# antoyang/FrozenBiLM

Hardware: AMD Instinct MI355X
Metric: video-text samples/sec (MLM fwd+bwd) DeBERTa-XL+adapters (higher is better)
Workload: dtype bf16; 1 GPU; DeBERTa-v2-XLarge(24L)+adapters ds8/8, B=32/GPU, T=10x1024, L=256 (S=266), MLM fwd+bwd+allreduce+clip+Adam, dropout 0.1 live, seeded random weights; global_batch=32, seq_len=266, parallelism=dp1, dead_layer23_encoder_pass=skipped (output unused, SURVEY fact 6); FLOPs still counted

## Files before the change

### frozenbilm_amd/build.py

```python
from __future__ import annotations

import concurrent.futures as cf
import os
import shutil
import subprocess
import sys

HERE = os.path.dirname(os.path.abspath(__file__))
CSRC = os.path.join(HERE, "csrc")
DEBUG = os.environ.get("FBL_DEBUG_BUILD", "0") == "1"
OBJ = os.path.join(HERE, "csrc", "build_dbg" if DEBUG else "build")
LIB = os.path.join(HERE, "libfbl_dbg.so" if DEBUG else "libfbl.so")
ARCH = "gfx950"
FLAGS = ["--offload-arch=" + ARCH, "-O3", "-std=c++17", "-fPIC", "-fno-gpu-rdc", "-Wno-unused-result"]
if DEBUG:
    FLAGS.append("-DFBL_DEBUG_SWITCHES")
    FLAGS += os.environ.get("FBL_DEBUG_EXTRA_FLAGS", "").split()
    if os.environ.get("FBL_DEBUG_LIB_NAME"):
        LIB = os.path.join(HERE, os.environ["FBL_DEBUG_LIB_NAME"])
        OBJ = os.path.join(HERE, "csrc", "build_dbg_" + os.path.splitext(os.environ["FBL_DEBUG_LIB_NAME"])[0])


def _hipcc() -> str:
    for cand in (os.environ.get("HIPCC"), shutil.which("hipcc"), "/opt/rocm/bin/hipcc"):
        if cand and os.path.exists(cand):
            return cand
    raise RuntimeError("hipcc not found (need ROCm >= 7.0 with gfx950 support)")


def sources():
    return sorted(os.path.join(CSRC, f) for f in os.listdir(CSRC) if f.endswith(".hip"))


def _deps_mtime() -> float:
    hdrs = [os.path.join(CSRC, f) for f in os.listdir(CSRC) if f.endswith(".h")]
    hdrs += [os.path.join(os.path.dirname(HERE), "include", h) for h in ("fbl.h", "fbl_mha.h", "fbl_qrows.h", "fbl_live.h", "fbl_predict.h", "fbl_groups.h", "fbl_lora.h", "fbl_ema.h", "fbl_prompt.h", "fbl_rows.h", "fbl_prompt_layers.h")]
    return max(os.path.getmtime(h) for h in hdrs)


def _compile(src: str, force: bool) -> str:
    obj = os.path.join(OBJ, os.path.basename(src)[:-4] + ".o")
    if not force and os.path.exists(obj) and os.path.getmtime(obj) > max(os.path.getmtime(src), _deps_mtime()):
        return obj
    cmd = [_hipcc(), *FLAGS, "-Rpass-analysis=kernel-resource-usage", "-c", src, "-o", obj]
    r = subprocess.run(cmd, capture_output=True, text=True)
    if r.returncode != 0:
        raise RuntimeError(f"hipcc failed for {src}:\n{r.stdout}\n{r.stderr}")
    bad, name = [], "?"
    for line in r.stderr.splitlines():
        if "Function Name:" in line:
            name = line.split("Function Name:")[1].split("[")[0].strip()
        elif "ScratchSize [bytes/lane]:" in line:
            n = int(line.split("ScratchSize [bytes/lane]:")[1].split("[")[0])
            if n > 64:
                bad.append(f"{name}: {n} bytes/lane")
            elif n > 0:
                print(f"[frozenbilm_amd.build] note: {name} spills {n} bytes/lane")
    if bad and os.environ.get("FBL_ALLOW_SCRATCH", "0") != "1":
        os.remove(obj)
        raise RuntimeError(f"{os.path.basename(src)}: kernels using scratch memory (set FBL_ALLOW_SCRATCH=1 to build anyway):\n  "
                           + "\n  ".join(bad))
    return obj


def build_lib(force: bool = False, verbose: bool = True) -> str:
    os.makedirs(OBJ, exist_ok=True)
    srcs = sources()
    with cf.ThreadPoolExecutor(max_workers=min(8, len(srcs))) as ex:
        objs = list(ex.map(lambda s: _compile(s, force), srcs))
    if force or not os.path.exists(LIB) or any(os.path.getmtime(o) > os.path.getmtime(LIB) for o in objs):
        cmd = [_hipcc(), "--offload-arch=" + ARCH, "-shared", "-fPIC", "-o", LIB, *objs]
        r = subprocess.run(cmd, capture_output=True, text=True)
        if r.returncode != 0:
            raise RuntimeError(f"link failed:\n{r.stdout}\n{r.stderr}")
        if verbose:
            print(f"[frozenbilm_amd.build] linked {LIB} from {len(objs)} objects")
    elif verbose:
        print(f"[frozenbilm_amd.build] {LIB} up to date")
    return LIB


if __name__ == "__main__":
    build_lib(force="--force" in sys.argv)
```

### frozenbilm_amd/csrc/adapter_dw.hip

```cpp
#include "fbl_common.h"
#include "../../include/fbl.h"

namespace {

constexpr int ADW_MAX_OUT = FBL_ADW_MAX_ADAPTERS;
constexpr int ADW_MAX_SEG = FBL_ADW_MAX_SEGMENTS;

struct AdwSeg { const bf16* dy; const bf16* z; const bf16* dz; const bf16* x; };
struct AdwArgs {
  AdwSeg seg[ADW_MAX_SEG];
  float* dWu[ADW_MAX_OUT]; float* dWd[ADW_MAX_OUT]; float* dbd[ADW_MAX_OUT];
  int seg_first[ADW_MAX_OUT + 1];
  int ld_dy[ADW_MAX_OUT], ld_z[ADW_MAX_OUT], ld_dz[ADW_MAX_OUT], ld_x[ADW_MAX_OUT];
  int N, H, A, tiles_h, n_out;
};

constexpr int WI = 2;
constexpr int WT = WI * 32;
constexpr int ADW_LDW = WT + 16;

template <int NT, int WHICH>
__device__ __forceinline__ void adw_tile(const AdwArgs& g, bf16* sW, bf16* sS, const int th, const int o) {
  constexpr int AP = NT * 32;
  constexpr int LDS_ = AP + 16;
  constexpr int NCH = AP / 8;
  constexpr int SPT = (64 * NCH) / 256;
  constexpr int WCH = WT / 8, WPT = (64 * WCH) / 256;
  const int tid = threadIdx.x, lane = tid & 63;
  const int wave = __builtin_amdgcn_readfirstlane(tid >> 6);
  const int wm = wave >> 1, wn = wave & 1;
  const int h0 = th * WT;
  const long ldw = WHICH ? g.ld_x[o] : g.ld_dy[o], lds = WHICH ? g.ld_dz[o] : g.ld_z[o];
  const int nk = (g.N + 63) / 64;
  const int s0 = g.seg_first[o], s1 = g.seg_first[o + 1];
  const int total = (s1 - s0) * nk;
  const int frow = lane & 15, fg = lane >> 4;

  f32x4 acc[NT][WI];
#pragma unroll
  for (int j = 0; j < NT; ++j)
#pragma unroll
    for (int i = 0; i < WI; ++i) acc[j][i] = (f32x4){0.f, 0.f, 0.f, 0.f};

  bf16x8 rw[WPT], rs[SPT];
  int gW[WPT], lW[WPT], rW[WPT], gS[SPT], lS[SPT], rS[SPT];
#pragma unroll
  for (int t = 0; t < WPT; ++t) {
    const int id = tid + t * 256;
    const int r = id / WCH, ch = id % WCH;
    const int c = min(h0 + ch * 8, g.H - 8);
    rW[t] = r;
    gW[t] = (int)(r * ldw + c);
    lW[t] = r * ADW_LDW + ch * 8;
  }
#pragma unroll
  for (int t = 0; t < SPT; ++t) {
    const int id = tid + t * 256;
    const int r = id / NCH, ch = id % NCH;
    rS[t] = r;
    gS[t] = (int)(r * lds + ch * 8);
    lS[t] = r * LDS_ + ch * 8;
  }
  const bf16x8 zero8 = (bf16x8){0, 0, 0, 0, 0, 0, 0, 0};
  const bool ragged = (g.N & 63) != 0;
  int sg_n = s0, kt_n = 0;
  auto load_tile = [&]() {
    const bf16* W = (WHICH ? g.seg[sg_n].x : g.seg[sg_n].dy) + (long)kt_n * 64 * ldw;
    const bf16* S = (WHICH ? g.seg[sg_n].dz : g.seg[sg_n].z) + (long)kt_n * 64 * lds;
    if (ragged && kt_n == nk - 1) {
      const int left = g.N - kt_n * 64;
#pragma unroll
      for (int t = 0; t < WPT; ++t) rw[t] = *(const bf16x8*)(W + gW[t] - (long)max(rW[t] - (left - 1), 0) * ldw);
#pragma unroll
      for (int t = 0; t < SPT; ++t) rs[t] = rS[t] < left ? *(const bf16x8*)(S + gS[t]) : zero8;
    } else {
#pragma unroll
      for (int t = 0; t < WPT; ++t) rw[t] = *(const bf16x8*)(W + gW[t]);
#pragma unroll
      for (int t = 0; t < SPT; ++t) rs[t] = *(const bf16x8*)(S + gS[t]);
    }
    if (++kt_n == nk) { kt_n = 0; ++sg_n; }
  };
  const bool do_cs = WHICH == 1 && th == 0 && g.dbd[o] != nullptr;
  const bf16x2 ones2 = {(bf16)1.0f, (bf16)1.0f};
  float cs[NT];
#pragma unroll
  for (int j = 0; j < NT; ++j) cs[j] = 0.f;
  const bf16* fW = sW + (fg * 4 + (frow >> 2)) * ADW_LDW + (frow & 3) * 4 + wm * (WI * 16);
  const bf16* fS = sS + (fg * 4 + (frow >> 2)) * LDS_ + (frow & 3) * 4 + wn * (NT * 16);
  if (total > 0) load_tile();
  for (int it = 0; it < total; ++it) {
#pragma unroll
    for (int t = 0; t < WPT; ++t) *(bf16x8*)(sW + lW[t]) = rw[t];
#pragma unroll
    for (int t = 0; t < SPT; ++t) *(bf16x8*)(sS + lS[t]) = rs[t];
    __syncthreads();
    if (it + 1 < total) load_tile();
#pragma unroll
    for (int s = 0; s < 2; ++s) {
      bf16x8 wf[WI], sf[NT];
#pragma unroll
      for (int i = 0; i < WI; ++i) {
        const bf16* p = fW + s * 32 * ADW_LDW + i * 16;
        union { tr16x4 h[2]; bf16x8 v; } u;
        u.h[0] = lds_tr16(p);
        u.h[1] = lds_tr16(p + 16 * ADW_LDW);
        wf[i] = u.v;
      }
#pragma unroll
      for (int j = 0; j < NT; ++j) {
        const bf16* p = fS + s * 32 * LDS_ + j * 16;
        union { tr16x4 h[2]; bf16x8 v; } u;
        u.h[0] = lds_tr16(p);
        u.h[1] = lds_tr16(p + 16 * LDS_);
        sf[j] = u.v;
      }
      if (WHICH == 1 && do_cs && s == wm) {
#pragma unroll
        for (int j = 0; j < NT; ++j) {
          union { bf16x8 v; bf16x2 p[4]; } u;
          u.v = sf[j];
#pragma unroll
          for (int q = 0; q < 4; ++q) cs[j] = __builtin_amdgcn_fdot2_f32_bf16(u.p[q], ones2, cs[j], false);
        }
      }
#pragma unroll
      for (int j = 0; j < NT; ++j)
#pragma unroll
        for (int i = 0; i < WI; ++i) {
          if (WHICH == 0) acc[j][i] = __builtin_amdgcn_mfma_f32_16x16x32_bf16(sf[j], wf[i], acc[j][i], 0, 0, 0);
          else acc[j][i] = __builtin_amdgcn_mfma_f32_16x16x32_bf16(wf[i], sf[j], acc[j][i], 0, 0, 0);
        }
    }
    __syncthreads();
  }
  const int A = g.A;
  if (WHICH == 0) {
    float* out = g.dWu[o];
    if (!out) return;
#pragma unroll
    for (int i = 0; i < WI; ++i) {
      const int h = h0 + wm * (WI * 16) + i * 16 + frow;
      if (h >= g.H) continue;
#pragma unroll
      for (int j = 0; j < NT; ++j) {
        const int a4 = wn * (NT * 16) + j * 16 + fg * 4;
        float* p = out + (long)h * A + a4;
        if (a4 + 4 <= A && ((uintptr_t)p & 15) == 0) *(f32x4*)p += acc[j][i];
        else
          for (int r = 0; r < 4; ++r)
            if (a4 + r < A) p[r] += acc[j][i][r];
      }
    }
  } else {
    if (do_cs) {
      float* red = (float*)sS;
#pragma unroll
      for (int j = 0; j < NT; ++j) red[(wm * 4 + fg) * AP + wn * (NT * 16) + j * 16 + frow] = cs[j];
      __syncthreads();
      if (tid < A) {
        float t = 0.f;
#pragma unroll
        for (int k = 0; k < 8; ++k) t += red[k * AP + tid];
        g.dbd[o][tid] += t;
      }
    }
    float* out = g.dWd[o];
    if (!out) return;
#pragma unroll
    for (int j = 0; j < NT; ++j) {
      const int a = wn * (NT * 16) + j * 16 + frow;
      if (a >= A) continue;
#pragma unroll
      for (int i = 0; i < WI; ++i) {
        const int h4 = h0 + wm * (WI * 16) + i * 16 + fg * 4;
        float* p = out + (long)a * g.H + h4;
        if (h4 + 4 <= g.H && ((uintptr_t)p & 15) == 0) *(f32x4*)p += acc[j][i];
        else
          for (int r = 0; r < 4; ++r)
            if (h4 + r < g.H) p[r] += acc[j][i][r];
      }
    }
  }
}

template <int NT>
__global__ __launch_bounds__(256, 2) void adapter_dw_kernel(AdwArgs g) {
  __shared__ __attribute__((aligned(16))) bf16 sW[64 * ADW_LDW];
  __shared__ __attribute__((aligned(16))) bf16 sS[64 * (NT * 32 + 16)];
  const int lin = blockIdx.x, xcd = lin & 7, slot = lin >> 3;
  const int p = (slot / g.tiles_h) * 8 + xcd, th = slot % g.tiles_h;
  if (p >= 2 * g.n_out) return;
  const int o = p >> 1;
  if ((p & 1) == 0) adw_tile<NT, 0>(g, sW, sS, th, o);
  else adw_tile<NT, 1>(g, sW, sS, th, o);
}

}

extern "C" int fbl_adapter_bwd_dw(int n_adapters, const int32_t* seg_first, const void* const* dy_bf16, const void* const* z_bf16,
                                  const void* const* dz_bf16, const void* const* x_bf16, const int64_t* ld_dy,
                                  const int64_t* ld_z, const int64_t* ld_dz, const int64_t* ld_x, int N, int H, int A, int Ap,
                                  float* const* dWu, float* const* dWd, float* const* dbd, void* stream) {
  if (n_adapters <= 0 || N <= 0 || H <= 0 || A <= 0) return 0;
  if (n_adapters > ADW_MAX_OUT || !seg_first || seg_first[0] != 0) return FBL_ERR_ARG;
  const int nseg = seg_first[n_adapters];
  if (nseg <= 0 || nseg > ADW_MAX_SEG) return FBL_ERR_ARG;
  if (Ap < A || (Ap % 64) || Ap > 256 || (H % 8)) return FBL_ERR_SHAPE;
  if (!dy_bf16 || !z_bf16 || !dz_bf16 || !x_bf16 || !ld_dy || !ld_z || !ld_dz || !ld_x) return FBL_ERR_ARG;
  AdwArgs g{};
  for (int o = 0; o < n_adapters; ++o) {
    if (seg_first[o + 1] < seg_first[o]) return FBL_ERR_ARG;
    g.seg_first[o] = seg_first[o];
    g.dWu[o] = dWu ? dWu[o] : nullptr;
    g.dWd[o] = dWd ? dWd[o] : nullptr;
    g.dbd[o] = dbd ? dbd[o] : nullptr;
    if ((ld_dy[o] % 8) || (ld_z[o] % 8) || (ld_dz[o] % 8) || (ld_x[o] % 8)) return FBL_ERR_ALIGN;
    if (ld_dy[o] < H || ld_x[o] < H || ld_z[o] < Ap || ld_dz[o] < Ap) return FBL_ERR_ARG;
    if ((ld_dy[o] | ld_x[o] | ld_z[o] | ld_dz[o]) >> 24) return FBL_ERR_ARG;
    g.ld_dy[o] = (int)ld_dy[o]; g.ld_z[o] = (int)ld_z[o]; g.ld_dz[o] = (int)ld_dz[o]; g.ld_x[o] = (int)ld_x[o];
  }
  g.seg_first[n_adapters] = nseg;
  for (int s = 0; s < nseg; ++s) {
    if (!dy_bf16[s] || !z_bf16[s] || !dz_bf16[s] || !x_bf16[s]) return FBL_ERR_ARG;
    g.seg[s] = AdwSeg{(const bf16*)dy_bf16[s], (const bf16*)z_bf16[s], (const bf16*)dz_bf16[s], (const bf16*)x_bf16[s]};
  }
  g.N = N; g.H = H; g.A = A;
  g.tiles_h = (H + WT - 1) / WT;
  g.n_out = n_adapters;
  dim3 grid((unsigned)(((2 * n_adapters + 7) / 8) * 8 * g.tiles_h));
  switch (Ap / 64) {
    case 1: hipLaunchKernelGGL(adapter_dw_kernel<2>, grid, dim3(256), 0, (hipStream_t)stream, g); break;
    case 2: hipLaunchKernelGGL(adapter_dw_kernel<4>, grid, dim3(256), 0, (hipStream_t)stream, g); break;
    case 3: hipLaunchKernelGGL(adapter_dw_kernel<6>, grid, dim3(256), 0, (hipStream_t)stream, g); break;
    default: hipLaunchKernelGGL(adapter_dw_kernel<8>, grid, dim3(256), 0, (hipStream_t)stream, g); break;
  }
  FBL_CHECK_LAUNCH();
  return 0;
}
```

### frozenbilm_amd/csrc/rowops.hip

```cpp
#include "fbl_common.h"
#include "../../include/fbl.h"
#include "../../include/fbl_live.h"
#include "../../include/fbl_groups.h"
#include "../../include/fbl_ema.h"
#include "../../include/fbl_rows.h"

namespace {

template <int VEC>
struct VecF {};
template <>
struct VecF<4> {
  typedef f32x4 T;
};
template <>
struct VecF<2> {
  typedef f32x2 T;
};

template <int VEC>
__device__ __forceinline__ void ldf(const float* p, float* v) {
  if (VEC == 4) {
    f32x4 x = *(const f32x4*)p;
    v[0] = x[0]; v[1] = x[1]; v[2] = x[2]; v[3] = x[3];
  } else if (VEC == 2) {
    f32x2 x = *(const f32x2*)p;
    v[0] = x[0]; v[1] = x[1];
  } else {
    v[0] = p[0];
  }
}
template <int VEC>
__device__ __forceinline__ void stf(float* p, const float* v) {
  if (VEC == 4) *(f32x4*)p = (f32x4){v[0], v[1], v[2], v[3]};
  else if (VEC == 2) *(f32x2*)p = (f32x2){v[0], v[1]};
  else p[0] = v[0];
}
template <int VEC>
__device__ __forceinline__ void stb(bf16* p, const float* v) {
  if (VEC == 4) *(bf16x4*)p = (bf16x4){f2bf(v[0]), f2bf(v[1]), f2bf(v[2]), f2bf(v[3])};
  else if (VEC == 2) *(bf16x2*)p = (bf16x2){f2bf(v[0]), f2bf(v[1])};
  else p[0] = f2bf(v[0]);
}

struct LnFwdArgs {
  const float* y; long ldy; float p_drop; uint64_t seed; const uint64_t* seed_dev;
  const float* r_plain; const float* r_t; const float* r_stats; const float* r_gamma; const float* r_beta;
  const int32_t* r_rowmask;
  const float* gamma; const float* beta; float eps; const int32_t* rowmask;
  float* out_t; float* out_stats; bf16* out_bf16; float* out_f32;
  int N, H;
};

template <int EPL>
__global__ __launch_bounds__(256) void ln_fwd_kernel(LnFwdArgs a) {
  constexpr int VEC = (EPL % 4 == 0) ? 4 : ((EPL % 2 == 0) ? 2 : 1);
  constexpr int NIT = EPL / VEC;
  const int lane = threadIdx.x & 63;
  const int row = blockIdx.x * 4 + (threadIdx.x >> 6);
  if (row >= a.N) return;
  const int H = a.H;
  float v[EPL];
  const uint32_t thr = fbl_drop_thresh(a.p_drop);
  const float inv_keep = a.p_drop > 0.f ? 1.0f / (1.0f - a.p_drop) : 1.0f;
  const uint64_t seed = a.p_drop > 0.f ? fbl_seed(a.seed, a.seed_dev) : 0;
  float rmean = 0.f, rrstd = 0.f, rmask = 1.f;
  if (a.r_t) {
    rmean = a.r_stats[2 * (long)row];
    rrstd = a.r_stats[2 * (long)row + 1];
    if (a.r_rowmask) rmask = (float)a.r_rowmask[row];
  }
#pragma unroll
  for (int it = 0; it < NIT; ++it) {
    const int col = (it * 64 + lane) * VEC;
    float* vv = v + it * VEC;
    if (a.y) {
      ldf<VEC>(a.y + (long)row * a.ldy + col, vv);
      if (a.p_drop > 0.f) {
#pragma unroll
        for (int c = 0; c < VEC; ++c) vv[c] *= fbl_dropout_scale(seed, (uint64_t)row * H + col + c, thr, inv_keep);
      }
    } else {
#pragma unroll
      for (int c = 0; c < VEC; ++c) vv[c] = 0.f;
    }
    if (a.r_plain) {
      float r[VEC];
      ldf<VEC>(a.r_plain + (long)row * H + col, r);
#pragma unroll
      for (int c = 0; c < VEC; ++c) vv[c] += r[c];
    }
    if (a.r_t) {
      float r[VEC], gg[VEC], bb[VEC];
      ldf<VEC>(a.r_t + (long)row * H + col, r);
      ldf<VEC>(a.r_gamma + col, gg);
      ldf<VEC>(a.r_beta + col, bb);
#pragma unroll
      for (int c = 0; c < VEC; ++c) vv[c] += ((r[c] - rmean) * rrstd * gg[c] + bb[c]) * rmask;
    }
    if (a.out_t) stf<VEC>(a.out_t + (long)row * H + col, vv);
  }
  float s = 0.f;
#pragma unroll
  for (int e = 0; e < EPL; ++e) s += v[e];
  const float mean = wave_sum(s) / (float)H;
  float q = 0.f;
#pragma unroll
  for (int e = 0; e < EPL; ++e) {
    const float d = v[e] - mean;
    q += d * d;
  }
  const float var = wave_sum(q) / (float)H;
  const float rstd = rsqrtf(var + a.eps);
  if (lane == 0 && a.out_stats) {
    a.out_stats[2 * (long)row] = mean;
    a.out_stats[2 * (long)row + 1] = rstd;
  }
  const float om = a.rowmask ? (float)a.rowmask[row] : 1.0f;
#pragma unroll
  for (int it = 0; it < NIT; ++it) {
    const int col = (it * 64 + lane) * VEC;
    float gg[VEC], bb[VEC], o[VEC];
    ldf<VEC>(a.gamma + col, gg);
    ldf<VEC>(a.beta + col, bb);
#pragma unroll
    for (int c = 0; c < VEC; ++c) o[c] = ((v[it * VEC + c] - mean) * rstd * gg[c] + bb[c]) * om;
    if (a.out_bf16) stb<VEC>(a.out_bf16 + (long)row * H + col, o);
    if (a.out_f32) stf<VEC>(a.out_f32 + (long)row * H + col, o);
  }
}

struct LnMatArgs {
  const float* t; const float* stats; const float* gamma; const float* beta; const int32_t* rowmask;
  const float* add_bcast; int S; float* out_f32; bf16* out_bf16; int N, H;
};
template <int EPL>
__global__ __launch_bounds__(256) void ln_mat_kernel(LnMatArgs a) {
  constexpr int VEC = (EPL % 4 == 0) ? 4 : ((EPL % 2 == 0) ? 2 : 1);
  constexpr int NIT = EPL / VEC;
  const int lane = threadIdx.x & 63;
  const int row = blockIdx.x * 4 + (threadIdx.x >> 6);
  if (row >= a.N) return;
  const int H = a.H;
  const float mean = a.stats[2 * (long)row], rstd = a.stats[2 * (long)row + 1];
  const float om = a.rowmask ? (float)a.rowmask[row] : 1.0f;
#pragma unroll
  for (int it = 0; it < NIT; ++it) {
    const int col = (it * 64 + lane) * VEC;
    float x[VEC], gg[VEC], bb[VEC], o[VEC];
    ldf<VEC>(a.t + (long)row * H + col, x);
    ldf<VEC>(a.gamma + col, gg);
    ldf<VEC>(a.beta + col, bb);
#pragma unroll
    for (int c = 0; c < VEC; ++c) o[c] = ((x[c] - mean) * rstd * gg[c] + bb[c]) * om;
    if (a.add_bcast) {
      float p[VEC];
      ldf<VEC>(a.add_bcast + (long)(row % a.S) * H + col, p);
#pragma unroll
      for (int c = 0; c < VEC; ++c) o[c] += p[c];
    }
    if (a.out_f32) stf<VEC>(a.out_f32 + (long)row * H + col, o);
    if (a.out_bf16) stb<VEC>(a.out_bf16 + (long)row * H + col, o);
  }
}

constexpr int LNB_BLOCKS = 768;
struct LnBwdArgs {
  const float* dout; const int32_t* rowmask; const float* t; const float* stats; const float* gamma;
  float p_drop; uint64_t seed; const uint64_t* seed_dev; float* out_dt; bf16* out_dy_bf16; float* out_dy_f32; float* ws; int N, H;
  long ld_dyb;
  const int32_t* inv; bf16* out_dy_pad;
};
template <int EPL, bool ROWS = false>
__global__ __launch_bounds__(256) void ln_bwd_kernel(LnBwdArgs a) {
  constexpr int VEC = (EPL % 4 == 0) ? 4 : ((EPL % 2 == 0) ? 2 : 1);
  constexpr int NIT = EPL / VEC;
  __shared__ float red[4 * 64 * EPL];
  const int lane = threadIdx.x & 63, wave = threadIdx.x >> 6;
  const int H = a.H;
  float dg[EPL], db[EPL], dys[EPL], gam[EPL];
#pragma unroll
  for (int e = 0; e < EPL; ++e) dg[e] = db[e] = dys[e] = 0.f;
#pragma unroll
  for (int it = 0; it < NIT; ++it) ldf<VEC>(a.gamma + (it * 64 + lane) * VEC, gam + it * VEC);
  const uint32_t thr = fbl_drop_thresh(a.p_drop);
  const float inv_keep = a.p_drop > 0.f ? 1.0f / (1.0f - a.p_drop) : 1.0f;
  const uint64_t seed = a.p_drop > 0.f ? fbl_seed(a.seed, a.seed_dev) : 0;
  for (int row = blockIdx.x * 4 + wave; row < a.N; row += gridDim.x * 4) {
    long crow = row;
    if (ROWS) {
      const int cr = a.inv[row];
      if (cr < 0) {
        const float z[VEC] = {};
#pragma unroll
        for (int it = 0; it < NIT; ++it) stb<VEC>(a.out_dy_pad + (long)row * H + (it * 64 + lane) * VEC, z);
        continue;
      }
      crow = cr;
    }
    const float mean = a.stats[2 * (long)row], rstd = a.stats[2 * (long)row + 1];
    const float om = a.rowmask ? (float)a.rowmask[row] : 1.0f;
    float g[EPL], xh[EPL];
    float s1 = 0.f, s2 = 0.f;
#pragma unroll
    for (int it = 0; it < NIT; ++it) {
      const int col = (it * 64 + lane) * VEC;
      float d[VEC], x[VEC];
      ldf<VEC>(a.dout + crow * H + col, d);
      ldf<VEC>(a.t + (long)row * H + col, x);
#pragma unroll
      for (int c = 0; c < VEC; ++c) {
        const int e = it * VEC + c;
        const float dd = d[c] * om;
        xh[e] = (x[c] - mean) * rstd;
        dg[e] += dd * xh[e];
        db[e] += dd;
        g[e] = dd * gam[e];
        s1 += g[e];
        s2 += g[e] * xh[e];
      }
    }
    s1 = wave_sum(s1) / (float)H;
    s2 = wave_sum(s2) / (float)H;
#pragma unroll
    for (int it = 0; it < NIT; ++it) {
      const int col = (it * 64 + lane) * VEC;
      float dt[VEC], dy[VEC];
#pragma unroll
      for (int c = 0; c < VEC; ++c) {
        const int e = it * VEC + c;
        dt[c] = rstd * (g[e] - s1 - xh[e] * s2);
        dy[c] = dt[c];
        if (a.p_drop > 0.f) dy[c] *= fbl_dropout_scale(seed, (uint64_t)row * H + col + c, thr, inv_keep);
        dys[e] += dy[c];
      }
      if (a.out_dt) stf<VEC>(a.out_dt + crow * H + col, dt);
      if (a.out_dy_bf16) stb<VEC>(a.out_dy_bf16 + crow * a.ld_dyb + col, dy);
      if (a.out_dy_f32) stf<VEC>(a.out_dy_f32 + crow * H + col, dy);
      if (ROWS) stb<VEC>(a.out_dy_pad + (long)row * H + col, dy);
    }
  }
#pragma unroll
  for (int which = 0; which < 3; ++which) {
    const float* src = which == 0 ? dg : (which == 1 ? db : dys);
    if (which) __syncthreads();
#pragma unroll
    for (int it = 0; it < NIT; ++it) {
      const int col = (it * 64 + lane) * VEC;
#pragma unroll
      for (int c = 0; c < VEC; ++c) red[wave * H + col + c] = src[it * VEC + c];
    }
    __syncthreads();
    for (int i = threadIdx.x; i < H; i += 256) {
      float s_ = 0.f;
#pragma unroll
      for (int w = 0; w < 4; ++w) s_ += red[w * H + i];
      a.ws[(long)blockIdx.x * 3 * H + which * H + i] = s_;
    }
  }
}
template <int EPL, bool ROWS = false>
__global__ __launch_bounds__(256, 3) void ln_bwd2_kernel(LnBwdArgs a) {
  static_assert(EPL % 2 == 0, "two waves share a row");
  constexpr int EW = EPL / 2;
  constexpr int VEC = (EW % 4 == 0) ? 4 : ((EW % 2 == 0) ? 2 : 1);
  constexpr int NIT = EW / VEC;
  __shared__ float red[2 * 64 * EPL];
  __shared__ float xch[2][2][2][2];
  const int lane = threadIdx.x & 63, wave = threadIdx.x >> 6;
  const int slot = wave >> 1, half = wave & 1;
  const int H = a.H;
  const int c0 = half * (H / 2);
  float dg[EW], db[EW], dys[EW], gam[EW];
#pragma unroll
  for (int e = 0; e < EW; ++e) dg[e] = db[e] = dys[e] = 0.f;
#pragma unroll
  for (int it = 0; it < NIT; ++it) ldf<VEC>(a.gamma + c0 + (it * 64 + lane) * VEC, gam + it * VEC);
  const uint32_t thr = fbl_drop_thresh(a.p_drop);
  const float inv_keep = a.p_drop > 0.f ? 1.0f / (1.0f - a.p_drop) : 1.0f;
  const uint64_t seed = a.p_drop > 0.f ? fbl_seed(a.seed, a.seed_dev) : 0;
  int par = 0;
  for (int base = blockIdx.x * 2; base < a.N; base += gridDim.x * 2, par ^= 1) {
    const int row = base + slot;
    bool live = row < a.N;
    const int rr = live ? row : a.N - 1;
    long crow = row;
    bool pad_zero = false;
    if (ROWS) {
      const int cr = a.inv[rr];
      pad_zero = live && cr < 0;
      live = live && cr >= 0;
      crow = cr;
    }
    float g[EW], xh[EW];
    float s1 = 0.f, s2 = 0.f, rstd = 0.f;
    if (!ROWS || live) {
      const long lr = ROWS ? crow : (long)rr;
      const float mean = a.stats[2 * (long)rr];
      rstd = a.stats[2 * (long)rr + 1];
      const float om = live ? (a.rowmask ? (float)a.rowmask[rr] : 1.0f) : 0.f;
#pragma unroll
      for (int it = 0; it < NIT; ++it) {
        const int col = c0 + (it * 64 + lane) * VEC;
        float d[VEC], x[VEC];
        ldf<VEC>(a.dout + lr * H + col, d);
        ldf<VEC>(a.t + (long)rr * H + col, x);
#pragma unroll
        for (int c = 0; c < VEC; ++c) {
          const int e = it * VEC + c;
          const float dd = d[c] * om;
          xh[e] = (x[c] - mean) * rstd;
          dg[e] += dd * xh[e];
          db[e] += dd;
          g[e] = dd * gam[e];
          s1 += g[e];
          s2 += g[e] * xh[e];
        }
      }
      s1 = wave_sum(s1);
      s2 = wave_sum(s2);
    }
    if (lane == 0) {
      xch[par][slot][half][0] = s1;
      xch[par][slot][half][1] = s2;
    }
    __syncthreads();
    s1 = (xch[par][slot][0][0] + xch[par][slot][1][0]) / (float)H;
    s2 = (xch[par][slot][0][1] + xch[par][slot][1][1]) / (float)H;
    if (live) {
#pragma unroll
      for (int it = 0; it < NIT; ++it) {
        const int col = c0 + (it * 64 + lane) * VEC;
        float dt[VEC], dy[VEC];
#pragma unroll
        for (int c = 0; c < VEC; ++c) {
          const int e = it * VEC + c;
          dt[c] = rstd * (g[e] - s1 - xh[e] * s2);
          dy[c] = dt[c];
          if (a.p_drop > 0.f) dy[c] *= fbl_dropout_scale(seed, (uint64_t)row * H + col + c, thr, inv_keep);
          dys[e] += dy[c];
        }
        if (a.out_dt) stf<VEC>(a.out_dt + crow * H + col, dt);
        if (a.out_dy_bf16) stb<VEC>(a.out_dy_bf16 + crow * a.ld_dyb + col, dy);
        if (a.out_dy_f32) stf<VEC>(a.out_dy_f32 + crow * H + col, dy);
        if (ROWS) stb<VEC>(a.out_dy_pad + (long)row * H + col, dy);
      }
    } else if (ROWS && pad_zero) {
      const float z[VEC] = {};
#pragma unroll
      for (int it = 0; it < NIT; ++it) stb<VEC>(a.out_dy_pad + (long)row * H + c0 + (it * 64 + lane) * VEC, z);
    }
  }
#pragma unroll
  for (int which = 0; which < 3; ++which) {
    const float* src = which == 0 ? dg : (which == 1 ? db : dys);
    __syncthreads();
#pragma unroll
    for (int it = 0; it < NIT; ++it) {
      const int col = c0 + (it * 64 + lane) * VEC;
#pragma unroll
      for (int c = 0; c < VEC; ++c) red[slot * H + col + c] = src[it * VEC + c];
    }
    __syncthreads();
    for (int i = threadIdx.x; i < H; i += 256) a.ws[(long)blockIdx.x * 3 * H + which * H + i] = red[i] + red[H + i];
  }
}

__device__ __forceinline__ float fold16(const float* ws, int nblk, int ncols, int col) {
  __shared__ float red[16][17];
  const int tx = threadIdx.x & 15, ty = threadIdx.x >> 4;
  float s = 0.f;
  if (col < ncols)
    for (int b = ty; b < nblk; b += 16) s += ws[(long)b * ncols + col];
  red[ty][tx] = s;
  __syncthreads();
  if (ty == 0) {
#pragma unroll
    for (int k = 1; k < 16; ++k) s += red[k][tx];
  }
  return s;
}
__global__ __launch_bounds__(256) void ln_bwd_fold_kernel(const float* ws, int nblk, int H, float* dgamma, float* dbeta,
                                                          float* dysum) {
  __shared__ f32x4 red[4][8];
  const int tx = threadIdx.x & 7, ty = threadIdx.x >> 3;
  const int lane = threadIdx.x & 63, wave = threadIdx.x >> 6;
  const int col = blockIdx.x * 32 + tx * 4;
  const int ncols = 3 * H;
  f32x4 s = {0.f, 0.f, 0.f, 0.f};
  if (col < ncols) {
    const float* p = ws + col;
    int b = ty;
    for (; b + 224 < nblk; b += 256) {
      f32x4 v[8];
#pragma unroll
      for (int u = 0; u < 8; ++u) v[u] = *(const f32x4*)(p + (long)(b + 32 * u) * ncols);
      s += ((v[0] + v[1]) + (v[2] + v[3])) + ((v[4] + v[5]) + (v[6] + v[7]));
    }
    for (; b < nblk; b += 32) s += *(const f32x4*)(p + (long)b * ncols);
  }
#pragma unroll
  for (int o = 8; o < 64; o <<= 1) {
#pragma unroll
    for (int r = 0; r < 4; ++r) s[r] += __shfl_xor(s[r], o, 64);
  }
  if (lane < 8) red[wave][lane] = s;
  __syncthreads();
  if (threadIdx.x < 8 && col < ncols) {
    s = (red[0][tx] + red[1][tx]) + (red[2][tx] + red[3][tx]);
    float* dst = col < H ? dgamma : (col < 2 * H ? dbeta : dysum);
    if (dst) {
      float* q = dst + (col % H);
#pragma unroll
      for (int r = 0; r < 4; ++r) q[r] += s[r];
    }
  }
}

__global__ void embed_gather_kernel(const int64_t* ids, const float* E, const float* vproj, int B, int T, int L, int H,
                                    float* out) {
  const int S = T + L;
  const int row = blockIdx.x;
  const int b = row / S, s = row % S;
  const float* src = (s < T) ? vproj + ((long)b * T + s) * H : E + ids[(long)b * L + (s - T)] * (long)H;
  float* dst = out + (long)row * H;
  for (int c = threadIdx.x * 4; c < H; c += blockDim.x * 4) *(f32x4*)(dst + c) = *(const f32x4*)(src + c);
}

__global__ void video_stage_kernel(const _Float16* feats, const int64_t* row_off, const int32_t* n_rows, int T, int F,
                                   float* out, int64_t* video_len, int64_t* video_mask) {
  const int b = blockIdx.x / T, j = blockIdx.x % T;
  const int n = n_rows[b];
  const int len = n < T ? n : T;
  if (threadIdx.x == 0) {
    if (j == 0 && video_len) video_len[b] = len;
    if (video_mask) video_mask[(long)b * T + j] = j < len ? 1 : 0;
  }
  float* dst = out + ((long)b * T + j) * F;
  if (j >= len) {
    for (int c = threadIdx.x * 4; c < F; c += blockDim.x * 4) *(f32x4*)(dst + c) = (f32x4){0.f, 0.f, 0.f, 0.f};
    return;
  }
  const long r = n > T ? ((long)j * n) / T : j;
  const _Float16* src = feats + (row_off[b] + r) * (long)F;
  typedef __attribute__((ext_vector_type(8))) _Float16 f16x8;
  for (int c = threadIdx.x * 8; c < F; c += blockDim.x * 8) {
    const f16x8 h = *(const f16x8*)(src + c);
    *(f32x4*)(dst + c) = (f32x4){(float)h[0], (float)h[1], (float)h[2], (float)h[3]};
    *(f32x4*)(dst + c + 4) = (f32x4){(float)h[4], (float)h[5], (float)h[6], (float)h[7]};
  }
}

__global__ void mask_tokens_kernel(int64_t* ids, int64_t* labels, long n, const int64_t* special, int n_special, float p,
                                   int64_t mask_id, int64_t vocab, uint64_t seed) {
  const long i = (long)blockIdx.x * blockDim.x + threadIdx.x;
  if (i >= n) return;
  const int64_t id = ids[i];
  bool sp = false;
  for (int k = 0; k < n_special; ++k) sp |= (special[k] == id);
  const float inv = 1.0f / 4294967296.0f;
  const bool pick = !sp && (float)fbl_hash(seed, 4ull * i) * inv < p;
  labels[i] = pick ? id : -100;
  if (!pick) return;
  if ((float)fbl_hash(seed, 4ull * i + 1) * inv < 0.8f) ids[i] = mask_id;
  else if ((float)fbl_hash(seed, 4ull * i + 2) * inv < 0.5f) ids[i] = (int64_t)(fbl_hash(seed, 4ull * i + 3) % (uint64_t)vocab);
}

__global__ void im2col3_kernel(const bf16* x, bf16* out, int B, int S, int H) {
  const int row = blockIdx.x;
  const int s = row % S;
  const int chunks = 3 * H / 8;
  for (int i = threadIdx.x; i < chunks; i += blockDim.x) {
    const int k = (i * 8) / H, c = (i * 8) % H;
    const int ss = s + k - 1;
    bf16x8 v = {0, 0, 0, 0, 0, 0, 0, 0};
    if (ss >= 0 && ss < S) v = *(const bf16x8*)(x + ((long)row + k - 1) * H + c);
    *(bf16x8*)(out + (long)row * 3 * H + i * 8) = v;
  }
}
__global__ void col2im3_kernel(const float* dcol, float* dx, int B, int S, int H, int accumulate) {
  const int row = blockIdx.x;
  const int s = row % S;
  for (int c = threadIdx.x * 4; c < H; c += blockDim.x * 4) {
    f32x4 acc = accumulate ? *(const f32x4*)(dx + (long)row * H + c) : (f32x4){0.f, 0.f, 0.f, 0.f};
#pragma unroll
    for (int k = 0; k < 3; ++k) {
      const int ss = s - k + 1;
      if (ss >= 0 && ss < S) acc += *(const f32x4*)(dcol + ((long)row - k + 1) * 3 * H + k * H + c);
    }
    *(f32x4*)(dx + (long)row * H + c) = acc;
  }
}

__global__ void dropout_gelu_fwd_kernel(const float* c, float p, uint64_t seed0, const uint64_t* seed_dev, float* out, long n) {
  const uint64_t seed = p > 0.f ? fbl_seed(seed0, seed_dev) : 0;
  const uint32_t thr = fbl_drop_thresh(p);
  const float ik = p > 0.f ? 1.f / (1.f - p) : 1.f;
  for (long i = (long)blockIdx.x * blockDim.x + threadIdx.x; i < n; i += (long)gridDim.x * blockDim.x) {
// ... 539 lines not shown
    const int h = (int)(eh % nh);
    const long e = eh / nh;
    const f32x4 a = *(const f32x4*)(src + q * 64 + c8 * 8), b = *(const f32x4*)(src + q * 64 + c8 * 8 + 4);
    *(bf16x8*)(dst + (e * rows + r) * ld_dst + h * 64 + c8 * 8) =
        (bf16x8){f2bf(a[0]), f2bf(a[1]), f2bf(a[2]), f2bf(a[3]), f2bf(b[0]), f2bf(b[1]), f2bf(b[2]), f2bf(b[3])};
  }
}

inline int grid1d(long n, int block = 256, int cap = 256 * 16) {
  long b = (n + block - 1) / block;
  return (int)(b < 1 ? 1 : (b > cap ? cap : b));
}

}

#define FBL_EPL_DISPATCH(H, KERNEL, GRID, ARGS, STREAM)                                              \
  switch ((H) / 64) {                                                                                \
    case 1: hipLaunchKernelGGL(KERNEL<1>, GRID, dim3(256), 0, STREAM, ARGS); break;                  \
    case 2: hipLaunchKernelGGL(KERNEL<2>, GRID, dim3(256), 0, STREAM, ARGS); break;                  \
    case 4: hipLaunchKernelGGL(KERNEL<4>, GRID, dim3(256), 0, STREAM, ARGS); break;                  \
    case 8: hipLaunchKernelGGL(KERNEL<8>, GRID, dim3(256), 0, STREAM, ARGS); break;                  \
    case 12: hipLaunchKernelGGL(KERNEL<12>, GRID, dim3(256), 0, STREAM, ARGS); break;                \
    case 16: hipLaunchKernelGGL(KERNEL<16>, GRID, dim3(256), 0, STREAM, ARGS); break;                \
    case 24: hipLaunchKernelGGL(KERNEL<24>, GRID, dim3(256), 0, STREAM, ARGS); break;                \
    case 32: hipLaunchKernelGGL(KERNEL<32>, GRID, dim3(256), 0, STREAM, ARGS); break;                \
    default: return FBL_ERR_SHAPE;                                                                   \
  }

extern "C" int fbl_abi_version(void) { return 9; }

extern "C" int fbl_embed_gather(const int64_t* ids, const float* E, const float* vproj, int B, int T, int L, int H,
                                float* out_t, void* stream) {
  if (H % 4) return FBL_ERR_SHAPE;
  if (T > 0 && !vproj) return FBL_ERR_ARG;
  if (B * (T + L) <= 0) return 0;
  hipLaunchKernelGGL(embed_gather_kernel, dim3(B * (T + L)), dim3(128), 0, (hipStream_t)stream, ids, E, vproj, B, T, L,
                     H, out_t);
  FBL_CHECK_LAUNCH();
  return 0;
}

extern "C" int fbl_video_stage_f16(const void* feats_f16, const int64_t* row_off, const int32_t* n_rows, int B, int T, int F,
                                   float* out_f32, int64_t* video_len, int64_t* video_mask, void* stream) {
  if (F % 8 || ((uintptr_t)feats_f16 & 15) || ((uintptr_t)out_f32 & 15)) return FBL_ERR_ALIGN;
  if (B <= 0 || T <= 0) return 0;
  hipLaunchKernelGGL(video_stage_kernel, dim3(B * T), dim3(128), 0, (hipStream_t)stream, (const _Float16*)feats_f16, row_off,
                     n_rows, T, F, out_f32, video_len, video_mask);
  FBL_CHECK_LAUNCH();
  return 0;
}

extern "C" int fbl_mask_tokens(int64_t* ids, int64_t* labels, int64_t n, const int64_t* special_ids, int n_special,
                               float mlm_probability, int64_t mask_token_id, int64_t vocab_size, uint64_t seed,
                               void* stream) {
  if (n <= 0) return 0;
  if (vocab_size <= 0 || mlm_probability < 0.f || mlm_probability > 1.f || n_special < 0) return FBL_ERR_ARG;
  hipLaunchKernelGGL(mask_tokens_kernel, dim3((unsigned)((n + 255) / 256)), dim3(256), 0, (hipStream_t)stream, ids, labels,
                     (long)n, special_ids, n_special, mlm_probability, mask_token_id, vocab_size, seed);
  FBL_CHECK_LAUNCH();
  return 0;
}

extern "C" int fbl_ln_fwd(const float* y, int64_t ldy, float p_drop, uint64_t seed, const uint64_t* seed_dev, const float* r_plain,
                          const float* r_t, const float* r_stats, const float* r_gamma, const float* r_beta,
                          const int32_t* r_rowmask, const float* gamma, const float* beta, float eps,
                          const int32_t* rowmask, float* out_t, float* out_stats, void* out_bf16, float* out_f32, int N,
                          int H, void* stream) {
  if (H % 64 || H > 2048) return FBL_ERR_SHAPE;
  if (r_t && (!r_stats || !r_gamma || !r_beta)) return FBL_ERR_ARG;
  if (N <= 0) return 0;
  LnFwdArgs a{y, ldy, p_drop, seed, seed_dev, r_plain, r_t, r_stats, r_gamma, r_beta, r_rowmask, gamma, beta, eps, rowmask,
              out_t, out_stats, (bf16*)out_bf16, out_f32, N, H};
  dim3 grid((N + 3) / 4);
  FBL_EPL_DISPATCH(H, ln_fwd_kernel, grid, a, (hipStream_t)stream);
  FBL_CHECK_LAUNCH();
  return 0;
}

extern "C" int fbl_ln_materialize(const float* t, const float* stats, const float* gamma, const float* beta,
                                  const int32_t* rowmask, const float* add_bcast, int S, float* out_f32, void* out_bf16,
                                  int N, int H, void* stream) {
  if (H % 64 || H > 2048) return FBL_ERR_SHAPE;
  if (N <= 0) return 0;
  LnMatArgs a{t, stats, gamma, beta, rowmask, add_bcast, S > 0 ? S : 1, out_f32, (bf16*)out_bf16, N, H};
  dim3 grid((N + 3) / 4);
  FBL_EPL_DISPATCH(H, ln_mat_kernel, grid, a, (hipStream_t)stream);
  FBL_CHECK_LAUNCH();
  return 0;
}

extern "C" int64_t fbl_ln_bwd_ws_floats(int H) { return (int64_t)LNB_BLOCKS * 3 * H; }
template <bool ROWS>
static int ln_bwd_launch(const LnBwdArgs& a, float* dgamma, float* dbeta, float* dysum, hipStream_t stream) {
  const int N = a.N, H = a.H;
  int nblk;
  if ((H / 64) % 2 == 0) {
    nblk = (N + 1) / 2;
    if (nblk > LNB_BLOCKS) nblk = LNB_BLOCKS;
    dim3 grid(nblk);
    switch (H / 64) {
      case 2: hipLaunchKernelGGL((ln_bwd2_kernel<2, ROWS>), grid, dim3(256), 0, stream, a); break;
      case 4: hipLaunchKernelGGL((ln_bwd2_kernel<4, ROWS>), grid, dim3(256), 0, stream, a); break;
      case 8: hipLaunchKernelGGL((ln_bwd2_kernel<8, ROWS>), grid, dim3(256), 0, stream, a); break;
      case 12: hipLaunchKernelGGL((ln_bwd2_kernel<12, ROWS>), grid, dim3(256), 0, stream, a); break;
      case 16: hipLaunchKernelGGL((ln_bwd2_kernel<16, ROWS>), grid, dim3(256), 0, stream, a); break;
      case 24: hipLaunchKernelGGL((ln_bwd2_kernel<24, ROWS>), grid, dim3(256), 0, stream, a); break;
      case 32: hipLaunchKernelGGL((ln_bwd2_kernel<32, ROWS>), grid, dim3(256), 0, stream, a); break;
      default: return FBL_ERR_SHAPE;
    }
  } else {
    nblk = (N + 3) / 4;
    if (nblk > LNB_BLOCKS) nblk = LNB_BLOCKS;
    dim3 grid(nblk);
    switch (H / 64) {
      case 1: hipLaunchKernelGGL((ln_bwd_kernel<1, ROWS>), grid, dim3(256), 0, stream, a); break;
      default: return FBL_ERR_SHAPE;
    }
  }
  FBL_CHECK_LAUNCH();
  if (dgamma || dbeta || dysum) {
    hipLaunchKernelGGL(ln_bwd_fold_kernel, dim3((3 * H + 31) / 32), dim3(256), 0, stream, a.ws, nblk, H, dgamma, dbeta, dysum);
    FBL_CHECK_LAUNCH();
  }
  return 0;
}

extern "C" int fbl_ln_bwd(const float* dout, const int32_t* rowmask, const float* t, const float* stats,
                          const float* gamma, float p_drop, uint64_t seed, const uint64_t* seed_dev, float* out_dt, void* out_dy_bf16,
                          float* out_dy_f32, float* dgamma, float* dbeta, float* dysum, float* ws, int N, int H,
                          int64_t ld_dy_bf16, void* stream) {
  if (H % 64 || H > 2048) return FBL_ERR_SHAPE;
  if (N <= 0) return 0;
  if (ld_dy_bf16 == 0) ld_dy_bf16 = H;
  if (ld_dy_bf16 < H || (ld_dy_bf16 % 8)) return FBL_ERR_ALIGN;
  LnBwdArgs a{dout, rowmask, t, stats, gamma, p_drop, seed, seed_dev, out_dt, (bf16*)out_dy_bf16, out_dy_f32, ws, N, H, ld_dy_bf16,
              nullptr, nullptr};
  return ln_bwd_launch<false>(a, dgamma, dbeta, dysum, (hipStream_t)stream);
}

extern "C" int fbl_ln_bwd_rows(const float* dout, const int32_t* inv, const int32_t* rowmask, const float* t, const float* stats,
                               const float* gamma, float p_drop, uint64_t seed, const uint64_t* seed_dev, float* out_dt,
                               void* out_dy_bf16, int64_t ld_dy_bf16, void* out_dy_pad_bf16, float* dgamma, float* dbeta,
                               float* dysum, float* ws, int N_pad, int H, void* stream) {
  if (H % 64 || H > 2048) return FBL_ERR_SHAPE;
  if (!dout || !inv || !t || !stats || !gamma || !ws || !out_dy_pad_bf16) return FBL_ERR_ARG;
  if (N_pad <= 0) return 0;
  if (ld_dy_bf16 == 0) ld_dy_bf16 = H;
  if (ld_dy_bf16 < H || (ld_dy_bf16 % 8)) return FBL_ERR_ALIGN;
  LnBwdArgs a{dout, rowmask, t, stats, gamma, p_drop, seed, seed_dev, out_dt, (bf16*)out_dy_bf16, nullptr, ws, N_pad, H, ld_dy_bf16,
              inv, (bf16*)out_dy_pad_bf16};
  return ln_bwd_launch<true>(a, dgamma, dbeta, dysum, (hipStream_t)stream);
}

extern "C" int fbl_im2col3(const void* x_bf16, void* out_bf16, int B, int S, int H, void* stream) {
  if (H % 8) return FBL_ERR_SHAPE;
  if (B * S <= 0) return 0;
  hipLaunchKernelGGL(im2col3_kernel, dim3(B * S), dim3(256), 0, (hipStream_t)stream, (const bf16*)x_bf16,
                     (bf16*)out_bf16, B, S, H);
  FBL_CHECK_LAUNCH();
  return 0;
}
extern "C" int fbl_col2im3(const float* dcol, float* dx, int B, int S, int H, int accumulate, void* stream) {
  if (H % 4) return FBL_ERR_SHAPE;
  if (B * S <= 0) return 0;
  hipLaunchKernelGGL(col2im3_kernel, dim3(B * S), dim3(256), 0, (hipStream_t)stream, dcol, dx, B, S, H, accumulate);
  FBL_CHECK_LAUNCH();
  return 0;
}

extern "C" int fbl_dropout_gelu_fwd(const float* c, float p_drop, uint64_t seed, const uint64_t* seed_dev, float* out_f32,
                                    int64_t n, void* stream) {
  if (n <= 0) return 0;
  hipLaunchKernelGGL(dropout_gelu_fwd_kernel, dim3(grid1d(n)), dim3(256), 0, (hipStream_t)stream, c, p_drop, seed, seed_dev,
                     out_f32, (long)n);
  FBL_CHECK_LAUNCH();
  return 0;
}
extern "C" int fbl_dropout_gelu_bwd(const float* dy, const float* c, float p_drop, uint64_t seed, const uint64_t* seed_dev,
                                    void* out_bf16, float* out_f32, int64_t n, void* stream) {
  if (n <= 0) return 0;
  hipLaunchKernelGGL(dropout_gelu_bwd_kernel, dim3(grid1d(n)), dim3(256), 0, (hipStream_t)stream, dy, c, p_drop, seed, seed_dev,
                     (bf16*)out_bf16, out_f32, (long)n);
  FBL_CHECK_LAUNCH();
  return 0;
}

extern "C" int fbl_transpose_to_bf16(const void* in, int in_is_bf16, int64_t ld_in, int rows, int cols, void* out_bf16,
                                     int64_t rows_pad, void* stream) {
  if (rows_pad < rows) return FBL_ERR_ARG;
  if (rows_pad <= 0 || cols <= 0) return 0;
  dim3 grid((unsigned)((rows_pad + 63) / 64), (cols + 63) / 64);
  if (in_is_bf16)
    hipLaunchKernelGGL(transpose_kernel<true>, grid, dim3(256), 0, (hipStream_t)stream, in, (long)ld_in, rows, cols,
                       (bf16*)out_bf16, (long)rows_pad);
  else
    hipLaunchKernelGGL(transpose_kernel<false>, grid, dim3(256), 0, (hipStream_t)stream, in, (long)ld_in, rows, cols,
                       (bf16*)out_bf16, (long)rows_pad);
  FBL_CHECK_LAUNCH();
  return 0;
}

extern "C" int fbl_transpose_batched_bf16(const void* src_bf16, const int64_t* src_off, void* dst_bf16,
                                          const int64_t* dst_off, int count, int rows, int cols, void* stream) {
  if (count <= 0 || rows <= 0 || cols <= 0) return 0;
  hipLaunchKernelGGL(transpose_batched_kernel, dim3((rows + 63) / 64, (cols + 63) / 64, count), dim3(256), 0,
                     (hipStream_t)stream, (const bf16*)src_bf16, src_off, (bf16*)dst_bf16, dst_off, rows, cols);
  FBL_CHECK_LAUNCH();
  return 0;
}

extern "C" int64_t fbl_colsum_ws_floats(int cols) { return (int64_t)CS_BLOCKS * cols; }
extern "C" int fbl_colsum(const void* in, int in_is_bf16, int64_t ld_in, int rows, int cols, float* out, float* ws,
                          void* stream) {
  if (rows <= 0 || cols <= 0) return 0;
  int nblk = rows < CS_BLOCKS ? rows : CS_BLOCKS;
  dim3 grid(nblk, (cols + 255) / 256);
  if (in_is_bf16)
    hipLaunchKernelGGL(colsum_kernel<true>, grid, dim3(256), 0, (hipStream_t)stream, in, (long)ld_in, rows, cols, ws);
  else
    hipLaunchKernelGGL(colsum_kernel<false>, grid, dim3(256), 0, (hipStream_t)stream, in, (long)ld_in, rows, cols, ws);
  FBL_CHECK_LAUNCH();
  hipLaunchKernelGGL(colsum_fold_kernel, dim3((cols + 15) / 16), dim3(256), 0, (hipStream_t)stream, ws, nblk, cols,
                     out);
  FBL_CHECK_LAUNCH();
  return 0;
}

extern "C" int fbl_head_transpose(const void* v_bf16, int64_t ldv, void* vt_bf16, int B, int S, int Sp, int nh,
                                  int64_t out_sh, int64_t out_sb, int64_t out_sd, void* stream) {
  if (Sp < S || Sp % 64) return FBL_ERR_SHAPE;
  if (ldv % 8 || out_sh % 8 || out_sb % 8 || out_sd % 8 || ((uintptr_t)v_bf16 & 15) || ((uintptr_t)vt_bf16 & 15)) return FBL_ERR_ALIGN;
  if (B * S <= 0) return 0;
  hipLaunchKernelGGL(head_transpose_kernel, dim3(Sp / 64, nh, B), dim3(256), 0, (hipStream_t)stream,
                     (const bf16*)v_bf16, (long)ldv, (bf16*)vt_bf16, B, S, Sp, nh, (long)out_sh, (long)out_sb,
                     (long)out_sd);
  FBL_CHECK_LAUNCH();
  return 0;
}

extern "C" int fbl_ce_fwd(const float* logits, int64_t ldv, const int64_t* labels, int N, int V, float* row_lse,
                          float* loss_sum_cnt, void* stream) {
  if (N <= 0) return 0;
  hipLaunchKernelGGL(ce_fwd_kernel, dim3(N), dim3(256), 0, (hipStream_t)stream, logits, (long)ldv, labels, N, V,
                     row_lse, loss_sum_cnt);
  FBL_CHECK_LAUNCH();
  hipLaunchKernelGGL(ce_fold_kernel, dim3(1), dim3(256), 0, (hipStream_t)stream, logits, (long)ldv, labels, N, row_lse,
                     loss_sum_cnt);
  FBL_CHECK_LAUNCH();
  return 0;
}
extern "C" int fbl_ce_bwd_rows(const float* logits, int64_t ldv, const int64_t* labels, const int32_t* rows, int R,
                               int V, int Vp, const float* row_lse, const float* loss_sum_cnt, float gscale,
                               const float* gscale_dev, void* dlogits_bf16, void* stream) {
  if (R <= 0) return 0;
  if (Vp < V) return FBL_ERR_ARG;
  hipLaunchKernelGGL(ce_bwd_rows_kernel, dim3(R), dim3(256), 0, (hipStream_t)stream, logits, (long)ldv, labels, rows, V,
                     Vp, row_lse, loss_sum_cnt, gscale, gscale_dev, (bf16*)dlogits_bf16);
  FBL_CHECK_LAUNCH();
  return 0;
}

extern "C" int fbl_gather_rows_bf16(const void* in, int64_t ld, const int32_t* rows, int R, int cols, void* out,
                                    void* stream) {
  if (R <= 0) return 0;
  if (cols % 8 || ld % 8) return FBL_ERR_ALIGN;
  hipLaunchKernelGGL(gather_rows_bf16_kernel, dim3(R), dim3(128), 0, (hipStream_t)stream, (const bf16*)in, (long)ld,
                     rows, cols, (bf16*)out);
  FBL_CHECK_LAUNCH();
  return 0;
}
extern "C" int fbl_scatter_rows_f32(const float* in, const int32_t* rows, int R, int cols, float* out, int64_t ld,
                                    void* stream) {
  if (R <= 0) return 0;
  hipLaunchKernelGGL(scatter_rows_f32_kernel, dim3(R), dim3(256), 0, (hipStream_t)stream, in, rows, cols, out,
                     (long)ld);
  FBL_CHECK_LAUNCH();
  return 0;
}

extern "C" int64_t fbl_sumsq_ws_floats(void) { return SUMSQ_BLOCKS; }
extern "C" int fbl_sumsq(const float* x, int64_t n, float* out_sumsq, float* ws, void* stream) {
  if (n <= 0) return 0;
  if (!ws || !out_sumsq) return FBL_ERR_ARG;
  const int nblk = grid1d(n, 256, SUMSQ_BLOCKS);
  hipLaunchKernelGGL(sumsq_kernel, dim3(nblk), dim3(256), 0, (hipStream_t)stream, x, (long)n, ws);
  FBL_CHECK_LAUNCH();
  hipLaunchKernelGGL(sumsq_fold_kernel, dim3(1), dim3(256), 0, (hipStream_t)stream, (const float*)ws, nblk, out_sumsq);
  FBL_CHECK_LAUNCH();
  return 0;
}
extern "C" int fbl_adam_flat(float* p, const float* g, float* m, float* v, int64_t n, float lr, float beta1,
                             float beta2, float eps, float weight_decay, int step, const float* sumsq, float max_norm,
                             float grad_scale, void* stream) {
  if (n <= 0) return 0;
  const float bc1 = 1.0f - powf(beta1, (float)step);
  const float bc2 = 1.0f - powf(beta2, (float)step);
  hipLaunchKernelGGL(adam_flat_kernel, dim3(grid1d(n)), dim3(256), 0, (hipStream_t)stream, p, g, m, v, (long)n, lr,
                     beta1, beta2, eps, weight_decay, bc1, bc2, sumsq, max_norm, grad_scale);
  FBL_CHECK_LAUNCH();
  return 0;
}

static inline bool live_aligned(const void* a) { return ((uintptr_t)a & 15) == 0; }
extern "C" int fbl_sumsq_live(const float* x, int64_t n, const int64_t* ranges, float* out_sumsq, float* ws, void* stream) {
  if (n <= 0) return 0;
  if (!x || !ranges || !ws || !out_sumsq) return FBL_ERR_ARG;
// ... 138 lines not shown
```

### frozenbilm_amd/engine.py

```python
from __future__ import annotations

import dataclasses
from dataclasses import dataclass, field
from typing import Dict, List, Optional

import numpy as np
import torch

from . import lib as L
from .predict import check_topk, of_call as predictions_of_call
from .live_set import REL_LN, LiveSetMixin, flat_layout, stage_plan
from .attn_bwd import ATTN_SCALE, _relidx_range, disent_attn_bwd, pos_chain_buffers, pos_table_grads_batched
from .model.deberta import PROMPT_NAME, layer_prompt_name
from .model.relpos import rel_index_vector

BF16, F32 = torch.bfloat16, torch.float32


def _ru(x: int, m: int) -> int:
    return (x + m - 1) // m * m


def check_logit_rows(logit_rows: torch.Tensor, n_grid: int) -> None:
    r = logit_rows.reshape(-1)
    if r.numel() == 0:
        return
    s = torch.sort(r.long()).values
    dup = (s[1:] == s[:-1]).any() if s.numel() > 1 else torch.zeros((), dtype=torch.bool, device=s.device)
    lo, hi, dup = torch.stack([s[0], s[-1], dup.long()]).tolist()
    if lo < 0 or hi >= n_grid:
        raise ValueError(f"logit_rows must index the [B, S] token grid: 0 <= row < {n_grid} (got {lo} .. {hi})")
    if dup:
        raise ValueError("logit_rows holds an index more than once: with gradients every requested row must be distinct")


@dataclass
class NormRef:
    t: torch.Tensor
    stats: torch.Tensor
    gamma: torch.Tensor
    beta: torch.Tensor
    rowmask: Optional[torch.Tensor] = None

    def as_args(self):
        return (self.t, self.stats, self.gamma, self.beta, self.rowmask)


@dataclass
class Stream:
    bf16: torch.Tensor
    norm: Optional[NormRef] = None
    plain: Optional[torch.Tensor] = None
    full: Optional[torch.Tensor] = None


@dataclass
class Packing:
    row0: torch.Tensor
    sel: torch.Tensor
    inv: torch.Tensor
    pos: torch.Tensor
    n: int
    sel32: Optional[torch.Tensor] = None
    inv32: Optional[torch.Tensor] = None


@dataclass
class MergedPack:
    A: int
    WT: torch.Tensor
    WM: torch.Tensor
    bM: torch.Tensor
    b16: torch.Tensor
    WF: Optional[torch.Tensor]
    groups: list


@dataclass
class AdapterSite:
    name: str
    A: int
    Ap: int
    down: torch.Tensor
    up: torch.Tensor
    bd: torch.Tensor
    bu: torch.Tensor
    merged: bool
    grouped: bool
    WM: Optional[torch.Tensor] = None
    bM: Optional[torch.Tensor] = None
    WF: Optional[torch.Tensor] = None
    upT: Optional[torch.Tensor] = None
    downT: Optional[torch.Tensor] = None


@dataclass
class LoraSite:
    name: str
    li: int
    t: int
    idx: int


class Engine(LiveSetMixin):
    def __init__(self, model):
        self.m = model
        cfg = model.config
        self.cfg = cfg
        self.H, self.I, self.V = cfg.hidden_size, cfg.intermediate_size, cfg.vocab_size
        self.nh = cfg.num_attention_heads
        self.nL = cfg.num_hidden_layers
        self.span2 = 2 * cfg.att_span
        self.lin_span = min(cfg.position_buckets // 2, cfg.att_span) if cfg.position_buckets > 0 else 0
        self.F = model.features_dim
        self.Fp = _ru(self.F, 64) if self.F else 0
        self.A1 = self.H // model.ds_factor_attn if model.ds_factor_attn else 0
        self.A2 = self.H // model.ds_factor_ff if model.ds_factor_ff else 0
        self.Vp = _ru(self.V, 64)
        dev = model.device
        if dev.type != "cuda":
            raise RuntimeError("frozenbilm_amd runs on MI355X only: move the model to a cuda (HIP) device; "
                               "there is no CPU fallback")
        L.load()
        self.dev = dev
        o = dict(getattr(model, "engine_options", None) or {})
        unknown = set(o) - {"eager_logits", "dw_group", "attn_save_p"}
        if unknown:
            raise ValueError(f"unknown engine_options: {sorted(unknown)}")
        self.eager_logits = bool(o.get("eager_logits", False))
        self.attn_save_p = bool(o.get("attn_save_p", True))
        self.dw_group = max(1, min(L.ADW_MAX_ADAPTERS, int(o.get("dw_group", 16))))
        self.n_prompt = int(getattr(model, "n_prompt", 0))
        self.prompt_depth = int(getattr(model, "prompt_depth", 1))
        self._build_flat()
        self._pack_frozen()
        self._build_trainable_operands()
        self._build_lora()
        self._compose_ev = None
        self._relidx: Dict[int, torch.Tensor] = {}
        self._pos_cache: Dict[int, torch.Tensor] = {}
        self._no_pos_cache = False
        self.reducer = None
        self._dyz_pool: Dict[tuple, list] = {}
        self._dyz_shape = None
        self._dyz_compact = None
        self.params_version = 0
        self._ops_version = None
        self.skip_dead_layer = True
        self._ln_ws = L.ln_bwd_ws(self.H, dev)
        self._cs_ws = L.colsum_ws(max(self.H, self.I), dev)
        self.sk_ws = torch.empty(48 << 20, dtype=F32, device=dev)
        self.side = torch.cuda.Stream(device=dev)
        self.side_ws = torch.empty(8 << 20, dtype=F32, device=dev)
        self.side_cs_ws = L.colsum_ws(max(self.H, self.I), dev)
        if L._AUX.get(dev.index if dev.index is not None else torch.cuda.current_device()) is None:
            L.set_aux_stream(torch.cuda.Stream(device=dev), dev)
        L.exclude_from_aux(self.side)

    def _build_flat(self):
        from .model.deberta import flat_order

        m = self.m
        named = dict(m.named_parameters())
        train_names = m.trainable_names()
        order = flat_order(self.cfg, train_names)
        offs, total = flat_layout(order, {n: named[n].numel() for n in order})
        self.flat = torch.zeros(total, dtype=F32, device=self.dev)
        from .parallel import SCALAR_SLOT

        self.flat_grad_full = torch.zeros(SCALAR_SLOT + total, dtype=F32, device=self.dev)
        self.flat_grad = self.flat_grad_full[SCALAR_SLOT:]
        self.flat_bf16 = torch.zeros(total, dtype=BF16, device=self.dev)
        self.offsets, self.order = offs, order
        self._adT_offs = {}
        self.G: Dict[str, torch.Tensor] = {}
        self.Pb: Dict[str, torch.Tensor] = {}
        for n in order:
            p = named[n]
            o, k = offs[n], p.numel()
            view = self.flat[o:o + k].view(p.shape)
            view.copy_(p.data)
            p.data = view
            self.G[n] = self.flat_grad[o:o + k].view(p.shape)
            self.Pb[n] = self.flat_bf16[o:o + k].view(p.shape)
        self.P = {n: p.data for n, p in named.items()}
        self.named = named
        self.bucket_ends: Dict[str, int] = {}
        for n in order:
            key = self._bucket_key(n)
            self.bucket_ends[key] = offs[n] + _ru(named[n].numel(), 8)
        self._plans: Dict[tuple, object] = {}
        self._init_live()

    def plan(self, grad_in=()):
        key = (self.live_version, bool(grad_in))
        pl = self._plans.get(key)
        if pl is None:
            pl = self._plans[key] = stage_plan(self.nL, bool(self.cfg.conv_kernel_size), self.live_order, grad_in)
        return pl

    def _bucket_key(self, name: str) -> str:
        if name.startswith("lm_predictions."):
            return "head"
        if name.startswith("deberta.encoder.layer."):
            return "layer" + name.split(".")[3]
        if name.startswith("deberta.encoder.conv."):
            return "conv"
        if name.startswith("deberta.encoder.LayerNorm"):
            return "relln"
        return "emb"

    def attach_grads(self):
        fresh = all(self.named[n].grad is None for n in self.live_order)
        if fresh:
            L.zero_(self.flat_grad)
        for n in self.live_order:
            p = self.named[n]
# ... 27 lines not shown
                Wi=bf(P[p + ".intermediate.dense.weight"]), WiT=bf(P[p + ".intermediate.dense.weight"].t()),
                bi=P[p + ".intermediate.dense.bias"].float().contiguous(),
                Wd=bf(P[p + ".output.dense.weight"]), WdT=self.WdT_rev[j],
                bd=P[p + ".output.dense.bias"].float().contiguous(),
            )
            self.Lw.append(d)
        order = [nL - 1, nL - 1] + list(range(nL - 2, -1, -1)) + [nL - 1]
        self.WposT_exec = torch.empty(len(order), H, 2 * H, dtype=BF16, device=dev)
        for e, li in enumerate(order):
            self.WposT_exec[e].copy_(self.Lw[li]["WqkvT"][:, : 2 * H])
        if self.cfg.conv_kernel_size:
            w = P["deberta.encoder.conv.conv.weight"]
            W2 = w.permute(0, 2, 1).reshape(H, 3 * H)
            self.Wc, self.WcT = bf(W2), bf(W2.t())
            self.bc = P["deberta.encoder.conv.conv.bias"].float().contiguous()
        hd = "lm_predictions.lm_head."
        self.Wh, self.WhT = bf(P[hd + "dense.weight"]), bf(P[hd + "dense.weight"].t())
        self.bh = P[hd + "dense.bias"].float().contiguous()
        E = P["deberta.embeddings.word_embeddings.weight"]
        self.E32 = E.float().contiguous()
        self.Eb = bf(E)
        self.ETb = torch.zeros(H, self.Vp, dtype=BF16, device=self.dev)
        self.ETb[:, : self.V] = E.t().to(BF16)
        self.head_bias = P[hd + "bias"].float().contiguous()
        self.rel_emb = P["deberta.encoder.rel_embeddings.weight"].float().contiguous()
        self.pos_emb = P["deberta.embeddings.position_embeddings.weight"].float().contiguous()
        if self.m.n_ans:
            T = P["answer_embeddings.weight"]
            self.n_ans = T.shape[0]
            self.Ansb = bf(T)
            self.ans_bias = P["answer_bias"].float().contiguous()

    def _build_trainable_operands(self):
        H, nL, dev = self.H, self.nL, self.dev
        self.sites = [[None, None] for _ in range(nL)]
        self.packs: List[MergedPack] = []
        for k, (blk, A, K, WT, wkey, bkey) in enumerate(((".attention.output.adapter", self.A1, H, self.WoT_rev, "Wo", "bo"),
                                                         (".output.adapter", self.A2, self.I, self.WdT_rev, "Wd", "bd"))):
            if not A:
                continue
            Ap = _ru(A, 64)
            merged = A % 64 == 0 and H % 64 == 0
            names = [f"deberta.encoder.layer.{i}{blk}" for i in range(nL)]
            pack = None
            if merged:
                WF = torch.zeros(nL, H, _ru(H + A, 128), dtype=BF16, device=dev) if k == 0 else None
                ow = [self.offsets[n + ".down.weight"] for n in names]
                ob = [self.offsets[n + ".down.bias"] for n in names]
                if nL >= 3 and len({ow[i - 1] - ow[i] for i in range(2, nL)}) == 1 and \
                        len({ob[i - 1] - ob[i] for i in range(2, nL)}) == 1 and ow[nL - 2] - ow[nL - 1] == ob[nL - 2] - ob[nL - 1] > 0:
                    groups = [(nL - 1, 1, ow[0], ob[0], A * H), (0, nL - 1, ow[nL - 1], ob[nL - 1], ow[nL - 2] - ow[nL - 1])]
                else:
                    groups = [(nL - 1 - i, 1, ow[i], ob[i], A * H) for i in range(nL)]
                pack = MergedPack(A=A, WT=WT, WM=torch.zeros(nL, H + A, K, dtype=BF16, device=dev),
                                  bM=torch.zeros(nL, H + A, dtype=F32, device=dev),
                                  b16=torch.zeros(nL, 1, H, dtype=BF16, device=dev), WF=WF, groups=groups)
                self.packs.append(pack)
            for i, n in enumerate(names):
                j = nL - 1 - i
                up = self.Pb[n + ".up.weight"] if Ap == A else torch.zeros(H, Ap, dtype=BF16, device=dev)
                site = AdapterSite(name=n, A=A, Ap=Ap, down=self.Pb[n + ".down.weight"], up=up, bd=self.P[n + ".down.bias"],
                                   bu=self.P[n + ".up.bias"], merged=merged, grouped=Ap <= 256 and H % 8 == 0)
                if merged:
                    pack.WM[j, :H].copy_(self.Lw[i][wkey])
                    pack.bM[j, :H].copy_(self.Lw[i][bkey])
                    pack.b16[j, 0].copy_(self.Lw[i][bkey])
                    site.WM, site.bM = pack.WM[j], pack.bM[j]
                    if pack.WF is not None:
                        pack.WF[j, :, :H].copy_(WT[j])
                        site.WF = pack.WF[j]
                self.sites[i][k] = site
        self.all_sites = [a for pair in self.sites for a in pair if a is not None]
        if self.F:
            wv = self.Pb["deberta.embeddings.linear_video.weight"]
            self.Wv = wv if self.Fp == self.F else torch.zeros(H, self.Fp, dtype=BF16, device=dev)

    def _build_lora(self):
        from .model.deberta import LORA_TARGETS

        m, H = self.m, self.H
        self.lora_r = int(getattr(m, "lora_rank", 0) or 0)
        self.lora_sites: Dict[tuple, LoraSite] = {}
        self.lora_composes = 0
        self._lora_ops = None
        self._lora_idx = None
        self._lora_names = set()
        self._lora_pos = False
        if not self.lora_r:
            return
        self.lora_s = float(m.lora_scale)
        recs = []
        for i in range(self.nL):
            for tname in m.lora_targets:
                t = LORA_TARGETS.index(tname)
                nm = f"deberta.encoder.layer.{i}.attention.self.{tname}"
                self.lora_sites[(i, t)] = LoraSite(name=nm, li=i, t=t, idx=len(recs))
                recs.append(dict(W=self.P[nm + ".weight"], A=self.P[nm + ".lora_A.weight"], B=self.P[nm + ".lora_B.weight"],
                                 scale=self.lora_s, dst=self.Lw[i]["Wqkv"][t * H:(t + 1) * H],
                                 dstT=self.Lw[i]["WqkvT"][:, t * H:(t + 1) * H]))
        self._lora_recs = recs
        self._lora_table = L.LoraTable(recs, self.dev)
        self._lora_names = {s.name for s in self.lora_sites.values()}
        self._lora_pos = any(t < 2 for (_, t) in self.lora_sites)
        self._lora_Aop = torch.zeros(len(recs), 64, H, dtype=BF16, device=self.dev)
        self._lora_BTop = torch.zeros(len(recs), 64, H, dtype=BF16, device=self.dev)

    def _compose_lora(self):
        L.lora_compose(self._lora_table)
        self.lora_composes += 1
        if self._lora_pos:
            H, nL = self.H, self.nL
            for e, li in enumerate([nL - 1, nL - 1] + list(range(nL - 2, -1, -1)) + [nL - 1]):
                self.WposT_exec[e].copy_(self.Lw[li]["WqkvT"][:, : 2 * H])

    def merge_lora(self):
        L.lora_compose(L.LoraTable([dict(r, dst32=r["W"]) for r in self._lora_recs], self.dev))
        for r in self._lora_recs:
            r["B"].zero_()
        self.invalidate_operands()

    def _lora_bwd_operands(self):
        if self._lora_ops is None:
            r, H, dev = self.lora_r, self.H, self.dev
            if self._lora_idx is None:
                i64 = lambda v: torch.tensor(v, dtype=torch.int64, device=dev)
                sites = sorted(self.lora_sites.values(), key=lambda s: s.idx)
                oA = i64([self.offsets[s.name + ".lora_A.weight"] for s in sites])
                oB = i64([self.offsets[s.name + ".lora_B.weight"] for s in sites])
                rowmajor = torch.arange(r * H, device=dev)
                transposed = (torch.arange(H, device=dev)[None, :] * r + torch.arange(r, device=dev)[:, None]).reshape(-1)
                self._lora_idx = ((oA[:, None] + rowmajor[None]).reshape(-1), (oB[:, None] + transposed[None]).reshape(-1))
            ns = len(self.lora_sites)
            self._lora_Aop[:, :r].copy_(self.flat_bf16.index_select(0, self._lora_idx[0]).view(ns, r, H))
            self._lora_BTop[:, :r].copy_(self.flat_bf16.index_select(0, self._lora_idx[1]).view(ns, r, H))
            self._lora_ops = (self._lora_Aop, self._lora_BTop)
        return self._lora_ops

    def _lora_products(self, site: LoraSite, dy, x):
        Aop, BTop = self._lora_bwd_operands()
        n = dy.shape[0]
        u = torch.empty(n, 64, dtype=BF16, device=self.dev)
        v = torch.empty(n, 64, dtype=BF16, device=self.dev)
        L.gemm(x, Aop[site.idx], alpha=self.lora_s, out_bf16=u)
        L.gemm(dy, BTop[site.idx], alpha=self.lora_s, out_bf16=v)
        return (dy, u, v, x)

    def _lora_live(self, site: Optional[LoraSite]) -> bool:
        return site is not None and any((site.name + k) in self.Gl for k in (".lora_A.weight", ".lora_B.weight"))

    def _lora_bwd(self, run, li: int, t: int, dy, x):
        site = self.lora_sites.get((li, t))
        if not self._lora_live(site):
            return
        run.dw_pending.append((self.lora_r, site.name, self._lora_products(site, dy, x), run.dw_count, None))
        run.dw_count += 1

    def _dw_outputs(self, nm: str, Gl):
        if nm in getattr(self, "_lora_names", ()):
            return Gl.get(nm + ".lora_B.weight"), Gl.get(nm + ".lora_A.weight"), None
        return Gl.get(nm + ".up.weight"), Gl.get(nm + ".down.weight"), Gl.get(nm + ".down.bias")

    def _lora_pos_bwd(self, run, pc, dpb):
        H, nL = self.H, self.nL
        order = [nL - 1, nL - 1] + list(range(nL - 2, -1, -1)) + [nL - 1]
        segs: Dict[str, list] = {}
        for e in range(dpb.shape[0]):
            sites = [self.lora_sites.get((order[e], t)) for t in (0, 1)]
            if not any(self._lora_live(s) for s in sites):
                continue
            if run.p_hid > 0:
                xe = torch.empty(self.span2, H, dtype=BF16, device=self.dev)
                L.dropout_f32(run.R32, run.p_hid, pc.seeds[e], out_bf16=xe)
            else:
                xe = run.Rb
            x = xe[pc.rmin:pc.rmin + pc.rcnt]
            for t, site in enumerate(sites):
                if self._lora_live(site):
                    segs.setdefault(site.name, []).append(self._lora_products(site, dpb[e][:, t * H:(t + 1) * H], x))
        groups, nseg = [], 0
        for nm, sg in list(segs.items()) + [(None, None)]:
            if groups and (nm is None or len(groups) == L.ADW_MAX_ADAPTERS or nseg + len(sg) > L.ADW_MAX_SEGMENTS):
                L.adapter_bwd_dw(groups, A=self.lora_r)
                groups, nseg = [], 0
            if nm is not None:
                groups.append((sg, *self._dw_outputs(nm, self.Gl)))
                nseg += len(sg)

    def relidx(self, S: int) -> torch.Tensor:
        if S not in self._relidx:
            v = rel_index_vector(S, self.cfg.position_buckets, self.cfg.max_rel, self.cfg.att_span)
            self._relidx[S] = torch.from_numpy(np.ascontiguousarray(v)).to(self.dev)
        return self._relidx[S]

    def _refresh_if_stale(self, need_grad: bool):
        frozen = getattr(self.m, "_weights_frozen", 0) > 0
        ver = (self.params_version, tuple(self.named[n]._version for n in self.order)) if (frozen and not need_grad) else None
        if ver is None or ver != self._ops_version:
            self.refresh_trainable_operands()
            self._ops_version = ver

    def seed_word_value(self) -> int:
        return (self.m.dropout_seed_base() * 0x9E3779B1) & 0x7FFFFFFFFFFFFFFF

    def prepare_inference(self):
        self._refresh_if_stale(False)
        if self._compose_ev is not None:
            torch.cuda.current_stream().wait_event(self._compose_ev[1])
            self._compose_ev = None

    def invalidate_operands(self):
        self._ops_version = None
        self.params_version += 1

    def refresh_trainable_operands(self):
        self._pos_cache.clear()
        L.cast_bf16(self.flat, self.flat_bf16)
        for a in self.all_sites:
            if a.Ap != a.A:
                a.up[:, :a.A] = self.Pb[a.name + ".up.weight"]
            a.upT = a.downT = None
        if self.packs:
            self.side.wait_stream(torch.cuda.current_stream())
            with torch.cuda.stream(self.side):
                self._compose_ev = self._compose_adapter_down()
        if self.F and self.Fp != self.F:
            self.Wv[:, : self.F] = self.Pb["deberta.embeddings.linear_video.weight"]
        if self.lora_r:
            self._lora_ops = None
            self._compose_lora()

    def _compose_adapter_down(self):
        H = self.H

        def run_group(pk: MergedPack, grp):
            A, (j0, nb, o_w, o_b, st) = pk.A, grp
            wd3 = torch.as_strided(self.flat_bf16, (nb, A, H), (st, H, 1), o_w)
            L.gemm(wd3, pk.WT[j0:j0 + nb], out_bf16=pk.WM[j0:j0 + nb, H:H + A, :])
            if pk.WF is not None:
                L.gemm(pk.WT[j0:j0 + nb], wd3, out_bf16=pk.WF[j0:j0 + nb, :, H:H + A])
            bd3 = torch.as_strided(self.flat, (nb, A, 1), (st, 1, 1), o_b)
            bo3 = torch.as_strided(pk.bM, (nb, A, 1), (pk.bM.stride(0), 1, 1), pk.bM[j0, H:].storage_offset())
            L.gemm(wd3, pk.b16[j0:j0 + nb], aux=bd3, aux_kind=L.AUX_ADD_F32, out_f32=bo3)

        for pk in self.packs:
            run_group(pk, pk.groups[0])
        ev0 = torch.cuda.Event()
        ev0.record()
        for pk in self.packs:
            for grp in pk.groups[1:]:
                run_group(pk, grp)
        ev1 = torch.cuda.Event()
        ev1.record()
        return ev0, ev1

    def _adapter_bwd_operands(self, site: AdapterSite):
        if site.upT is None:
            H = self.H
            groups = {}
            for a in self.all_sites:
                groups.setdefault((a.A, a.Ap), []).append(a)
            for (A, Ap), sites in groups.items():
                upT_all = torch.empty(len(sites), A, H, dtype=BF16, device=self.dev)
                for i, a in enumerate(sites):
                    a.upT = upT_all[i]
                cache = self._adT_offs.get((A, Ap))
                if cache is None:
                    i64 = lambda v: torch.tensor(v, dtype=torch.int64, device=self.dev)
                    cache = dict(up_src=i64([self.offsets[a.name + ".up.weight"] for a in sites]),
                                 dn_src=i64([self.offsets[a.name + ".down.weight"] for a in sites]),
                                 dst=i64([i * A * H for i in range(len(sites))]))
                    self._adT_offs[(A, Ap)] = cache
                L.transpose_batched_bf16(self.flat_bf16, cache["up_src"], upT_all, cache["dst"], H, A)
                if Ap == A:
                    dnT_all = torch.empty(len(sites), H, A, dtype=BF16, device=self.dev)
                    L.transpose_batched_bf16(self.flat_bf16, cache["dn_src"], dnT_all, cache["dst"], A, H)
                    for i, a in enumerate(sites):
                        a.downT = dnT_all[i]
                else:
                    for a in sites:
                        a.downT = torch.zeros(H, Ap, dtype=BF16, device=self.dev)
                        a.downT[:, :A].copy_(a.down.t())
        return site.upT, site.downT

    def run(self, input_ids, attention_mask, video, video_mask, labels, mlm, want_hidden, logit_rows=None, want_attn=False,
            inputs_embeds=None):
        m = self.m
        train = m.training
        k_pred = check_topk(getattr(m, "predict_topk", 0))
        text = input_ids if inputs_embeds is None else inputs_embeds
        if text.device != self.dev:
            raise RuntimeError(f"inputs must be on {self.dev}")
        B, Lt = text.shape[:2]
        if attention_mask is None:
            attention_mask = (torch.ones_like(input_ids) if inputs_embeds is None
                              else torch.ones(B, Lt, dtype=torch.long, device=self.dev))
        use_video = bool(self.F) and video is not None
        grad_on = torch.is_grad_enabled()
        grad_in = []
        if grad_on and use_video and video.requires_grad:
            grad_in.append(("video", video))
        if grad_on and inputs_embeds is not None and inputs_embeds.requires_grad:
            grad_in.append(("embeds", inputs_embeds))
        need_grad = grad_on and (self.update_live() or bool(grad_in))
        T = video.shape[1] if use_video else 0
        Pn = self.n_prompt
        S = T + Pn + Lt
        if S > self.cfg.max_position_embeddings:
            raise RuntimeError(
                f"sequence of {S} positions (video {T} + " + (f"prompt {Pn} + " if Pn else "") + f"text {Lt}) exceeds "
                f"max_position_embeddings={self.cfg.max_position_embeddings} (the reference fails the same way, "
                "model/deberta.py:1020-1021,1392)")
        front = []
        if use_video:
            if video_mask is None:
                video_mask = torch.ones(video.shape[:2], device=self.dev, dtype=attention_mask.dtype)
            front.append(video_mask.to(attention_mask.dtype))
        if Pn:
            front.append(torch.ones(B, Pn, device=self.dev, dtype=attention_mask.dtype))
        mask = torch.cat([*front, attention_mask], 1) if front else attention_mask
        mask = mask.to(torch.int32).contiguous()
        full_labels = None
        if labels is not None:
            if T + Pn:
                full_labels = torch.cat([torch.full((B, T + Pn), -100, dtype=torch.long, device=self.dev), labels], 1)
            else:
                full_labels = labels
            full_labels = full_labels.contiguous().view(-1)
            rows_labelled = torch.nonzero(full_labels != -100).view(-1)
        bwd_rows = self._backward_rows(m, need_grad, tuple(k for k, _ in grad_in), mask, full_labels, logit_rows, want_hidden, want_attn,
                                        B, S, T)
        if logit_rows is not None:
            if full_labels is not None:
                raise RuntimeError("logit_rows cannot be combined with labels (the loss of a labelled call lives on its own rows)")
            if need_grad:
                check_logit_rows(logit_rows, B * S)
        pk = None
        if (getattr(m, "packed_rows", False) and not want_attn and (full_labels is not None or logit_rows is not None)
                and not torch.cuda.is_current_stream_capturing()):
            pk = self._make_packing(mask, full_labels, logit_rows, B, S, T)
        if train:
            m.step_seed += 1
        run = Run(B=B, S=S, T=T, P=Pn, Lt=Lt, train=train, save=need_grad, seed_base=self.seed_word_value() if train else 0,
                  p_hid=self.cfg.hidden_dropout_prob if train else 0.0,
                  p_att=self.cfg.attention_probs_dropout_prob if train else 0.0,
                  p_ad=m.adapter_dropout if train else 0.0, mask=mask.view(-1), pk=pk, N=pk.n if pk is not None else B * S,
                  want_attn=bool(want_attn), labels=full_labels, rows=rows_labelled if full_labels is not None else None,
                  bwd_rows=bwd_rows)
        if want_attn and train and run.p_att > 0:
            raise NotImplementedError("output_attentions=True is served in eval mode (the probabilities of a training forward "
                                      "carry the attention dropout mask, which the fused kernel regenerates instead of storing)")
        if (getattr(m, "decoder_rows", False) and not self.lora_r and not want_attn and not want_hidden and not self.eager_logits
                and (full_labels is not None or logit_rows is not None) and not torch.cuda.is_current_stream_capturing()):
            run.dec_grid = (rows_labelled if full_labels is not None else logit_rows.to(self.dev).long().view(-1))
        if pk is not None and full_labels is not None:
            run.label_rows = rows_labelled
            run.rows = pk.inv[rows_labelled]
        self._refresh_if_stale(need_grad)
        use_ans = bool(m.n_ans) and not mlm
        if logit_rows is not None:
            run.logit_rows = logit_rows.to(self.dev).to(torch.int32).contiguous().view(-1)
            if pk is not None:
                run.logit_rows = pk.inv[run.logit_rows.long()].to(torch.int32)
        run.embeds = inputs_embeds
        run.video_dtype = video.dtype if use_video else None
        run.grad_in = tuple(k for k, _ in grad_in)
        if need_grad:
            run.plan, run.live_version = self.plan(run.grad_in), self.live_version
        run.hid_grad = bool(want_hidden) and need_grad
        with L.seed_word(run.seed_word):
            logits, loss_t = self._forward(run, input_ids.contiguous() if inputs_embeds is None else None, video, use_ans,
                                           want_hidden or want_attn)
        Vout = self.n_ans if use_ans else self.V
        if logit_rows is not None:
            res = {"logits": logits[:, :Vout], "loss": None, "run": run}
        else:
            res = {"logits": logits.view(B, S, -1)[:, :, :Vout] if logits is not None else None, "loss": None, "run": run}
        if k_pred:
            res["predictions"] = predictions_of_call(run, logits, k_pred, rows_labelled if full_labels is not None else None,
                                                     logit_rows)
        if want_hidden:
            res["hidden_states"] = run.hidden_out
        if want_attn:
            res["attentions"] = tuple(run.attn_out)
        if need_grad and res["logits"] is not None:
            lt = loss_t if loss_t is not None else torch.zeros((), dtype=F32, device=self.dev)
            hid = res["hidden_states"] if run.hid_grad else ()
            outs = _StepFn.apply(self, run, lt, res["logits"], len(hid), *hid, *[t for _, t in grad_in],
                                 *[self.named[n] for n in self.order])
            loss_o, res["logits"] = outs[:2]
            res["loss"] = loss_o if full_labels is not None else None
            if hid:
                res["hidden_states"] = tuple(outs[2:])
        elif full_labels is not None:
            res["loss"] = loss_t
        return res

    COMPACT_BWD_MIN_DROPPED = 0.37

    def _backward_rows(self, m, need_grad, grad_in, mask, full_labels, logit_rows, want_hidden, want_attn, B, S, T) -> Optional[Packing]:
        force = getattr(m, "compact_backward", None)
        if (force is False or not need_grad or full_labels is None or logit_rows is not None or want_hidden or want_attn
                or torch.cuda.is_current_stream_capturing() or getattr(m, "packed_rows", False) or getattr(m, "decoder_rows", False)
                or self.lora_r or self.n_prompt or self.reducer is not None or not self.attn_save_p):
            return None
        plan = self.plan(grad_in)
        if plan is not None and plan.lowest != 0:
            return None
        pk = self._make_packing(mask, full_labels, None, B, S, T)
        if pk is None or (force is not True and 1.0 - pk.n / (B * S) < self.COMPACT_BWD_MIN_DROPPED):
            return None
        pk.sel32, pk.inv32 = pk.sel.to(torch.int32), pk.inv.to(torch.int32)
        return pk

    def _make_packing(self, mask, full_labels, logit_rows, B, S, T) -> Optional[Packing]:
        dev = self.dev
        keep = mask.view(B, S) != 0
        if full_labels is not None:
            keep = keep | (full_labels.view(B, S) != -100)
        if logit_rows is not None:
            want = torch.zeros(B * S, dtype=torch.bool, device=dev)
            want[logit_rows.to(dev).long().view(-1)] = True
            keep = keep | want.view(B, S)
        pos1 = torch.arange(1, S + 1, device=dev, dtype=torch.int32)
        plen_h = [max(int(v), T, 1) for v in (keep.to(torch.int32) * pos1).amax(1).tolist()]
        n = sum(plen_h)
        if n >= B * S:
            return None
        offs = [0]
        for v in plen_h:
            offs.append(offs[-1] + v)
        row0 = torch.tensor(offs, dtype=torch.int32, device=dev)
        b_of = torch.repeat_interleave(torch.arange(B, device=dev), torch.tensor(plen_h, device=dev), output_size=n)
        pos = torch.arange(n, device=dev) - row0[:-1].long()[b_of]
        sel = b_of * S + pos
        inv = torch.full((B * S,), -1, dtype=torch.int64, device=dev)
        inv[sel] = torch.arange(n, device=dev)
        return Packing(row0=row0, sel=sel, inv=inv, pos=pos, n=n)

    def _ln(self, run, name, *, y, resid: Optional[Stream], N, p_drop=0.0, rowmask=None, want_f32=False, tail=0):
        H = self.H
        g, b = self.P[name + ".weight"], self.P[name + ".bias"]
        t = torch.empty(N, H, dtype=F32, device=self.dev)
        stats = torch.empty(N, 2, dtype=F32, device=self.dev)
        full = torch.empty(N + tail, H, dtype=BF16, device=self.dev)
        ob = full[:N]
        of = torch.empty(N, H, dtype=F32, device=self.dev) if want_f32 else None
        seed = run.next_seed() if p_drop > 0 else 0
        r_norm = resid.norm.as_args() if resid is not None and resid.norm is not None else None
        r_plain = resid.plain if resid is not None and r_norm is None else None
        L.ln_fwd(y=y, p_drop=p_drop, seed=seed, r_plain=r_plain, r_norm=r_norm,
                 gamma=g, beta=b, eps=self.cfg.layer_norm_eps, rowmask=rowmask, out_t=t, out_stats=stats, out_bf16=ob,
                 out_f32=of, N=N, H=H)
        return Stream(bf16=ob, norm=NormRef(t, stats, g, b, rowmask), plain=of, full=full if tail else None), seed

    def _adapter_fwd(self, run, site: AdapterSite, x_f32, x_bf16, N):
        A, Ap = site.A, site.Ap
        z = torch.zeros(N, Ap, dtype=BF16, device=self.dev) if Ap != A else torch.empty(N, Ap, dtype=BF16, device=self.dev)
        seed = run.next_seed() if run.p_ad > 0 else 0
        L.adapter_down_fwd(x_bf16, site.down, site.bd, z, A=A, p_drop=run.p_ad, seed=seed)
        y = torch.empty(N, self.H, dtype=F32, device=self.dev)
        L.gemm(z, site.up, bias=site.bu, aux=x_f32, aux_kind=L.AUX_ADD_F32, out_f32=y)
        return y, z, seed

    def _dense_adapter_ln(self, run, li, x_bf16, W, bias, site: Optional[AdapterSite], N, ln_name, resid: Stream, tail=0):
        H, dev = self.H, self.dev
        ob = torch.empty(N, H, dtype=BF16, device=dev)
        if site is None or not site.merged:
            y = torch.empty(N, H, dtype=F32, device=dev)
            L.gemm(x_bf16, W, bias=bias, out_f32=y, out_bf16=ob)
            z, seed_ad = None, 0
            if site is not None:
                y, z, seed_ad = self._adapter_fwd(run, site, y, ob, N)
            out, seed_ln = self._ln(run, ln_name, y=y, resid=resid, N=N, p_drop=run.p_hid, tail=tail)
            return out, ob, z, seed_ad, seed_ln
        if self._compose_ev is not None:
            torch.cuda.current_stream().wait_event(self._compose_ev[0 if li == 0 else 1])
        A = site.A
        z = torch.empty(N, A, dtype=BF16, device=dev)
        seed_ad = run.next_seed() if run.p_ad > 0 else 0
        L.dense_adapter_down_fwd(x_bf16, site.WM, site.bM, H, z, y_bf16=ob, p_drop=run.p_ad, seed=seed_ad)
        g, b = self.P[ln_name + ".weight"], self.P[ln_name + ".bias"]
        t = torch.empty(N, H, dtype=F32, device=dev)
        stats = torch.empty(N, 2, dtype=F32, device=dev)
        full = torch.empty(N + tail, H, dtype=BF16, device=dev)
        seed_ln = run.next_seed() if run.p_hid > 0 else 0
        r_norm = resid.norm.as_args() if resid.norm is not None else None
        L.adapter_up_resid_fwd(z, site.up, site.bu, ob, t, A=A, p_drop=run.p_hid, seed=seed_ln,
                               r_plain=resid.plain if r_norm is None else None, r_norm=r_norm)
        L.ln_fwd(y=t, gamma=g, beta=b, eps=self.cfg.layer_norm_eps, out_stats=stats, out_bf16=full[:N], N=N, H=H)
        return (Stream(bf16=full[:N], norm=NormRef(t, stats, g, b, None), full=full if tail else None), ob, z, seed_ad,
                seed_ln)

    def _pos_proj_cached(self, li: int, W, Rb: torch.Tensor) -> torch.Tensor:
        c = self._pos_cache.get(li)
        if c is None:
            c = torch.empty(self.span2, 2 * self.H, dtype=BF16, device=self.dev)
            L.gemm(Rb, W["Wqkv"][: 2 * self.H], bias=W["bqkv"][: 2 * self.H], out_bf16=c)
            self._pos_cache[li] = c
        return c

    def _pos_cache_allowed(self, run) -> bool:
        return not run.save and run.p_hid == 0 and getattr(self.m, "_weights_frozen", 0) > 0 and not self._no_pos_cache

    def _layer_fwd(self, run, li: int, kv: Stream, q: Optional[Stream], Rb: torch.Tensor):
        W = self.Lw[li]
        B, S, H, nh = run.B, run.S, self.H, self.nh
        N = run.N
        Sp = _ru(S, 64)
        dev = self.dev
        sv = LayerSave(li=li, emd=q is not None)
        P_ = self.span2
        if run.p_hid > 0:
            sv.seed_pos = run.next_seed()

        def put_r(full):
            if run.p_hid > 0:
                L.dropout_f32(run.R32, run.p_hid, sv.seed_pos, out_bf16=full[N:])
            else:
                full[N:].copy_(Rb)

        infer = not run.save and run.p_hid == 0
        pqk_c = self._pos_proj_cached(li, W, Rb) if self._pos_cache_allowed(run) else None
        reuse = infer and q is not None and run.emd_qkv is not None
        if reuse:
            qkv = run.emd_qkv
            if pqk_c is None:
                put_r(q.full)
            L.gemm(q.full if pqk_c is None else q.bf16, W["Wqkv"][:H], bias=W["bqkv"][:H], out_bf16=qkv[:, :H])
        else:
            rows_in = N if pqk_c is not None else N + P_
            qkv = torch.empty(rows_in, 3 * H, dtype=BF16, device=dev)
            kin = kv.full[:rows_in]
            if pqk_c is None:
                put_r(kv.full)
            if q is None:
                L.gemm(kin, W["Wqkv"], bias=W["bqkv"], out_bf16=qkv)
            else:
                if pqk_c is None:
                    put_r(q.full)
                L.gemm(q.full[:rows_in], W["Wqkv"][:H], bias=W["bqkv"][:H], out_bf16=qkv[:, :H])
                L.gemm(kin, W["Wqkv"][H:], bias=W["bqkv"][H:], out_bf16=qkv[:, H:])
                if infer:
                    run.emd_qkv = qkv
        if pqk_c is not None:
            pq, pk = pqk_c[:, :H], pqk_c[:, H:]
        else:
            pq, pk = qkv[N:, :H], qkv[N:, H:2 * H]
        ctx = torch.empty(N, H, dtype=BF16, device=dev)
        lse = torch.empty(B, nh, S, dtype=F32, device=dev)
        sv.seed_att = run.next_seed() if run.p_att > 0 else 0
        psave = msave = None
        if run.save and self.attn_save_p:
            psave = torch.empty(B, nh, Sp, Sp, dtype=BF16, device=dev)
            msave = torch.empty(B, nh, Sp // 64, S, dtype=F32, device=dev)
        L.disent_attn_fwd(qkv[:N, :H], qkv[:N, H:2 * H], qkv[:N, 2 * H:], pk, pq, self.relidx(S), run.mask_i32,
                          ATTN_SCALE, ctx, lse, B, S, Sp, nh, self.span2, p_drop=run.p_att, seed=sv.seed_att, klen=run.klen,
                          border=run.border, lin=self.lin_span, row0=run.row0, psave=psave, msave=msave)
        sv.psave, sv.msave = psave, msave
        if run.want_attn and q is None:
            probs = torch.empty(B, nh, S, S, dtype=F32, device=dev)
            L.disent_attn_probs(qkv[:N, :H], qkv[:N, H:2 * H], pk, pq, self.relidx(S), run.mask_i32, lse,
                                ATTN_SCALE, probs, B, S, nh)
            run.attn_out.append(probs)
        if run.save:
            sv.qkv, sv.pqk, sv.ctx, sv.lse = qkv[:N], qkv[N:, : 2 * H], ctx, lse
            if self.lora_r:
                sv.xkv, sv.xq = kv.bf16, (q.bf16 if q is not None else None)
        return self._layer_tail(run, li, sv, ctx, q if q is not None else kv, N, tail=self.span2)

    def _layer_tail(self, run, li: int, sv: "LayerSave", ctx, resid: Stream, N: int, tail=0) -> Stream:
        W, (a1, a2) = self.Lw[li], self.sites[li]
        p = f"deberta.encoder.layer.{li}"
        a, ob, z1, sv.seed_ad1, sv.seed_ln1 = self._dense_adapter_ln(
            run, li, ctx, W["Wo"], W["bo"], a1, N, p + ".attention.output.LayerNorm", resid=resid)
        h = torch.empty(N, self.I, dtype=BF16, device=self.dev)
        hpre = torch.empty(N, self.I, dtype=BF16, device=self.dev) if run.save else None
        L.gemm(a.bf16, W["Wi"], bias=W["bi"], act=L.ACT_GELU_GRAD if run.save else L.ACT_GELU, out_bf16=h, out_pre=hpre)
        out, fb, z2, sv.seed_ad2, sv.seed_ln2 = self._dense_adapter_ln(
            run, li, h, W["Wd"], W["bd"], a2, N, p + ".output.LayerNorm", resid=Stream(bf16=a.bf16, norm=a.norm), tail=tail)
        if run.save:
            sv.ob, sv.z1, sv.ln1 = ob, z1, a.norm
            sv.hpre, sv.fb, sv.z2, sv.ln2 = hpre, fb, z2, out.norm
            run.layers.append(sv)
        return out

    @staticmethod
    def _stage_runs(run, stage: str) -> bool:
        return run.plan is None or run.plan.runs(stage)

    def _skip_tail_seeds(self, run, li: int):
# ... 157 lines not shown
            run.logits_c = lc
        run.logits = torch.empty(run.B * run.S, run.ldv, dtype=F32, device=self.dev)
        run.logits_pending = True
        return run.loss_acc[0] / run.loss_acc[1]

    def _decoder_rows_fwd(self, run, kv: Stream, Rb, use_ans):
        from .row_plan import plan_query_rows

        H, nh, dev = self.H, self.nh, self.dev
        B, S, N = run.B, run.S, run.N
        li = self.nL - 1
        W = self.Lw[li]
        pk = run.pk
        pl = plan_query_rows(run.dec_grid, B, S, inv=pk.inv if pk is not None else None)
        run.dec_plan = pl
        R = pl.R
        Sp = _ru(S, 64)
        q = None
        if R:
            n_ = kv.norm
            if n_ is not None:
                qc32 = torch.empty(R, H, dtype=F32, device=dev)
                rm = n_.rowmask.index_select(0, pl.krows) if n_.rowmask is not None else None
                L.ln_materialize(n_.t.index_select(0, pl.krows), n_.stats.index_select(0, pl.krows), n_.gamma, n_.beta, rowmask=rm,
                                 out_f32=qc32)
            else:
                qc32 = kv.plain.index_select(0, pl.krows)
            qc32.add_(self.pos_emb.index_select(0, pl.rpos.long()))
            q = Stream(bf16=qc32.to(BF16), plain=qc32)
            kvp = torch.empty(N, 2 * H, dtype=BF16, device=dev)
            L.gemm(kv.bf16, W["Wqkv"][H:], bias=W["bqkv"][H:], out_bf16=kvp)
        keep = run.save
        run.save = keep and self._stage_runs(run, "decoder")
        for _ in range(2):
            sv = LayerSave(li=li, emd=True)
            if run.p_hid > 0:
                sv.seed_pos = run.next_seed()
            sv.seed_att = run.next_seed() if run.p_att > 0 else 0
            if not R:
                self._skip_tail_seeds(run, li)
                continue
            if run.p_hid > 0:
                Rd = torch.empty(self.span2, H, dtype=BF16, device=dev)
                L.dropout_f32(run.R32, run.p_hid, sv.seed_pos, out_bf16=Rd)
            else:
                Rd = Rb
            if self._pos_cache_allowed(run):
                pqk = self._pos_proj_cached(li, W, Rb)
            else:
                pqk = torch.empty(self.span2, 2 * H, dtype=BF16, device=dev)
                L.gemm(Rd, W["Wqkv"][: 2 * H], bias=W["bqkv"][: 2 * H], out_bf16=pqk)
            qp = torch.empty(R, H, dtype=BF16, device=dev)
            L.gemm(q.bf16, W["Wqkv"][:H], bias=W["bqkv"][:H], out_bf16=qp)
            ctx = torch.empty(R, H, dtype=BF16, device=dev)
            lse = torch.empty(nh, R, dtype=F32, device=dev)
            L.disent_attn_fwd_qrows(qp, pl.rseg, pl.rpos, kvp[:, :H], kvp[:, H:], pqk[:, H:], pqk[:, :H], self.relidx(S), run.mask_i32,
                                    run.klen, ATTN_SCALE, ctx, lse, B, S, Sp, nh, self.span2, p_drop=run.p_att, seed=sv.seed_att,
                                    row0=run.row0)
            if run.save:
                sv.qc, sv.kvp, sv.pqk, sv.ctx, sv.lse = qp, kvp, pqk, ctx, lse
            q = self._layer_tail(run, li, sv, ctx, q, R)
        run.save = keep
        Vout, table, bias, ldv = self._head_tables(run, use_ans)
        hin = q.bf16 if R else torch.empty(0, H, dtype=BF16, device=dev)
        hp, hl = self._head_stage(run, hin, R)
        run.head_pre, run.head_norm, run.head_ln_bf16 = hp, hl.norm, hl.bf16
        lc = torch.empty(R, ldv, dtype=F32, device=dev)
        if R:
            L.gemm(hl.bf16, table, bias=bias, out_f32=lc, N=Vout)
        if run.labels is None:
            run.logits = lc.index_select(0, pl.back)
            return run.logits, None
        run.rows_i32 = run.rows.to(torch.int32)
        loss_t = self._labelled_loss(run, lc, run.labels[pl.grid]) if R else self._labelled_loss(run, None, None)
        return run.logits, loss_t

    def fill_logits(self, run):
        if run.logits_pending:
            run.logits_pending = False
            if run.dec_plan is not None:
                run.logits.zero_()
                if run.dec_plan.R:
                    run.logits.index_copy_(0, run.dec_plan.grid, run.logits_c)
                return
            hin_all = run.head_in_all
            if hin_all is not None:
                _, hl = self._head_stage(run, hin_all, hin_all.shape[0])
                run.head_ln_bf16, run.head_in_all = hl.bf16, None
            pk = run.pk
            if pk is None:
                L.gemm(run.head_ln_bf16, run.head_table, bias=run.head_bias, out_f32=run.logits, N=run.Vout)
            else:
                run.logits.zero_()
                for r0 in range(0, pk.n, 1024):
                    r1 = min(pk.n, r0 + 1024)
                    slab = torch.empty(r1 - r0, run.logits.shape[1], dtype=F32, device=self.dev)
                    L.gemm(run.head_ln_bf16[r0:r1], run.head_table, bias=run.head_bias, out_f32=slab, N=run.Vout)
                    run.logits.index_copy_(0, pk.sel[r0:r1], slab)

    def _head_stage(self, run, hin, N):
        hp = torch.empty(N, self.H, dtype=F32, device=self.dev)
        L.gemm(hin, self.Wh, bias=self.bh, out_f32=hp)
        hg = torch.empty(N, self.H, dtype=F32, device=self.dev)
        L.dropout_gelu_fwd(hp, 0.0, 0, hg)
        hl, _ = self._ln(run, "lm_predictions.lm_head.LayerNorm", y=hg, resid=None, N=N)
        return hp, hl

    def _materialize(self, s: Stream, add=None, S=1, out_f32=None, out_bf16=None):
        N, H = s.bf16.shape
        if s.plain is not None and add is None and out_bf16 is None:
            return s.plain
        if out_f32 is None:
            out_f32 = torch.empty(N, H, dtype=F32, device=self.dev)
        if s.norm is not None:
            n = s.norm
            L.ln_materialize(n.t, n.stats, n.gamma, n.beta, rowmask=n.rowmask, add_bcast=add, S=S, out_f32=out_f32,
                             out_bf16=out_bf16)
        else:
            v = s.plain if add is None else (s.plain.view(-1, S, H) + add[:S]).view(N, H)
            out_f32.copy_(v)
            if out_bf16 is not None:
                out_bf16.copy_(v)
        return out_f32

    def _prompt_overwrite(self, run, i: int, x: Stream) -> Stream:
        N, H = run.N, self.H
        f32 = torch.empty(N, H, dtype=F32, device=self.dev)
        full = torch.empty(N + self.span2, H, dtype=BF16, device=self.dev)
        self._materialize(x, out_f32=f32, out_bf16=full[:N])
        L.prompt_rows_write(self.P[layer_prompt_name(i)], run.row0, run.B, run.S, run.T, out_f32=f32, out_bf16=full[:N])
        return Stream(bf16=full[:N], plain=f32, full=full)

    def _conv_fwd(self, run, emb: Stream, l0: Stream) -> Stream:
        B, S, H, dev = run.B, run.S, self.H, self.dev
        N = run.N
        pk = run.pk
        if pk is None:
            col = torch.empty(N, 3 * H, dtype=BF16, device=dev)
            L.im2col3(emb.bf16, col, B, S, H)
        else:
            grid = torch.zeros(B * S, H, dtype=BF16, device=dev).index_copy_(0, pk.sel, emb.bf16)
            colg = torch.empty(B * S, 3 * H, dtype=BF16, device=dev)
            L.im2col3(grid, colg, B, S, H)
            col = colg.index_select(0, pk.sel)
        c = torch.empty(N, H, dtype=F32, device=dev)
        L.gemm(col, self.Wc, bias=self.bc, rowscale=run.mask_f, out_f32=c)
        y = torch.empty(N, H, dtype=F32, device=dev)
        run.seed_conv = run.next_seed() if run.p_hid > 0 else 0
        L.dropout_gelu_fwd(c, run.p_hid, run.seed_conv, y)
        out, _ = self._ln(run, "deberta.encoder.conv.LayerNorm", y=y, resid=l0, N=N, rowmask=run.rowmask, tail=self.span2)
        run.conv_c, run.conv_norm = c, out.norm
        return out

    def _ln_bwd(self, name, dout, norm: NormRef, p_drop, seed, want_dy_bf16=True, dysum=None, tail=0, dy_out=None, cb=None):
        N, H = dout.shape
        if cb is not None:
            dt = torch.empty(N, H, dtype=F32, device=self.dev)
            dyb = dy_out if dy_out is not None else torch.empty(N, H, dtype=BF16, device=self.dev)
            dy_pad = torch.empty(norm.t.shape[0], H, dtype=BF16, device=self.dev)
            L.ln_bwd_rows(dout, cb.inv32, norm.t, norm.stats, norm.gamma, rowmask=norm.rowmask, p_drop=p_drop, seed=seed, out_dt=dt,
                          out_dy_bf16=dyb, out_dy_pad=dy_pad, dgamma=self.Gl.get(name + ".weight"), dbeta=self.Gl.get(name + ".bias"),
                          dysum=dysum, ws=self._ln_ws)
            return dt, dyb, dy_pad
        dt_full = torch.empty(N + tail, H, dtype=F32, device=self.dev)
        dt = dt_full[:N]
        if tail:
            dt_full[N:].zero_()
        dyb = dy_out if dy_out is not None else (torch.empty(N, H, dtype=BF16, device=self.dev) if want_dy_bf16 else None)
        L.ln_bwd(dout, norm.t, norm.stats, norm.gamma, rowmask=norm.rowmask, p_drop=p_drop, seed=seed, out_dt=dt,
                 out_dy_bf16=dyb, dgamma=self.Gl.get(name + ".weight"), dbeta=self.Gl.get(name + ".bias"), dysum=dysum,
                 ws=self._ln_ws)
        if tail:
            return dt, dyb, dt_full
        return dt, dyb

    def _adapter_bwd(self, run, site: AdapterSite, dyb, z, xin_b, seed, dz_out=None, pooled=None, pad=None):
        N, H = dyb.shape
        A, Ap = site.A, site.Ap
        dev = self.dev
        upT, downT = self._adapter_bwd_operands(site)
        if dz_out is not None:
            dz = dz_out
        else:
            dz = torch.zeros(N, Ap, dtype=BF16, device=dev) if Ap != A else torch.empty(N, Ap, dtype=BF16, device=dev)
        inv_keep = 1.0 / (1.0 - run.p_ad) if run.p_ad > 0 else 1.0
        L.gemm(dyb, upT, alpha=inv_keep, aux=z, aux_kind=L.AUX_MUL_POS_BF16, out_bf16=dz, N=A)
        dx = None
        if dz_out is None:
            dx = torch.empty(N, H, dtype=BF16, device=dev)
            L.gemm(dz, downT, aux=dyb, aux_kind=L.AUX_ADD_BF16, out_bf16=dx)
        nm = site.name
        gwu, gwd, gbd = (self.Gl.get(nm + k) for k in (".up.weight", ".down.weight", ".down.bias"))
        if gwu is None and gwd is None and gbd is None:
            return dx
        if pad is not None:
            dz_c, (dyb, z) = dz, pad
            dz = torch.empty(dyb.shape[0], dz_c.shape[1], dtype=BF16, device=dev)
            L.scatter_rows_zero_bf16(dz_c, run.cb.inv32, dz)
        sk = max(2, min(16, dyb.shape[0] // 512))

        if site.grouped:
            run.dw_pending.append((A, nm, (dyb, z, dz, xin_b), run.dw_count, pooled))
            run.dw_count += 1
            return dx

        self.side.wait_stream(torch.cuda.current_stream())
        with torch.cuda.stream(self.side):
            if gwu is not None:
                L.gemm_tn_acc(dyb, z, gwu, self.side_ws, N=A, splitk=sk)
            if gwd is not None:
                L.gemm_tn_acc(dz, xin_b, gwd, self.side_ws, M=A, splitk=sk)
            if gbd is not None:
                L.colsum(dz, gbd, self.side_cs_ws, cols=A)
        if not torch.cuda.is_current_stream_capturing():
            for t in (dyb, z, dz, xin_b):
                t.record_stream(self.side)
        else:
            run._pos_keep.extend((dyb, z, dz, xin_b))
        run.side_used = True
        if self.reducer is not None:
            run.dw_event = torch.cuda.Event()
            run.dw_event.record(self.side)
        return dx

    def _dw_flush(self, run, red=None, force=False):
        pend = run.dw_pending
        while pend and (force or len({rec[1] for rec in pend}) >= self.dw_group):
            take, names, rest = {}, set(), []
            for rec in pend:
                A, nm, seg = rec[:3]
                if nm in names or len(names) >= min(self.dw_group, L.ADW_MAX_ADAPTERS):
                    rest.append(rec)
                else:
                    names.add(nm)
                    take.setdefault((A, getattr(seg[0], "shape", (None,))[0]), []).append((nm, seg))
            for (A, _rows), recs in take.items():
                Gl = getattr(self, "Gl", None)
                Gl = self.G if Gl is None else Gl
                L.adapter_bwd_dw([([seg], *Engine._dw_outputs(self, nm, Gl)) for nm, seg in recs], A=A)
            kept = {id(r) for r in rest}
            for rec in pend:
                if id(rec) not in kept and rec[4] is not None and tuple(rec[4].shape) == self._dyz_shape:
                    self._dyz_pool.setdefault(self._dyz_shape, []).append(rec[4])
            pend[:] = rest
        if red is not None:
            parked = {self._bucket_key(rec[1] + ".up.weight") for rec in pend}
            still = []
            for key in run.dw_ready_keys:
                if key in parked:
                    still.append(key)
                elif not (getattr(run, "lora_pos_wait", False) and key.startswith("layer")):
                    red.ready(key)
            run.dw_ready_keys[:] = still

    def _layer_bwd(self, run, sv: "LayerSave", dout: torch.Tensor):
        li = sv.li
        W, (a1, a2) = self.Lw[li], self.sites[li]
        H, I, dev = self.H, self.I, self.dev
        N = dout.shape[0]
        p = f"deberta.encoder.layer.{li}"
        cb = run.cb
        if cb is not None:
            return self._layer_bwd_compact(run, sv, dout, cb)
        dt2, dy2 = self._ln_bwd(p + ".output.LayerNorm", dout, sv.ln2, run.p_hid, sv.seed_ln2,
                                dysum=self.Gl.get(a2.name + ".up.bias") if a2 is not None else None)
        df = dy2
        if a2 is not None:
            df = self._adapter_bwd(run, a2, dy2, sv.z2, sv.fb, sv.seed_ad2)
        dh = torch.empty(N, I, dtype=BF16, device=dev)
        L.gemm(df, W["WdT"], aux=sv.hpre, aux_kind=L.AUX_MUL_BF16, out_bf16=dh)
        da = torch.empty(N, H, dtype=F32, device=dev)
        L.gemm(dh, W["WiT"], aux=dt2, aux_kind=L.AUX_ADD_F32, out_f32=da)
        del dh
        dctx = torch.empty(N, H, dtype=BF16, device=dev)
        if a1 is not None and a1.merged:
            A1, Kf = a1.A, a1.WF.shape[1]
            pooled = None
            can_pool = not torch.cuda.is_current_stream_capturing() and a1.grouped and sv.kvp is None
            if can_pool and self._dyz_shape != (N, Kf):
                self._dyz_pool.clear()
                self._dyz_shape = (N, Kf)
            free = self._dyz_pool.get((N, Kf)) if can_pool else None
            if free:
                dyz = pooled = free.pop()
            elif can_pool:
                dyz = pooled = torch.zeros(N, Kf, dtype=BF16, device=dev)
            else:
                dyz = torch.empty(N, Kf, dtype=BF16, device=dev)
                if Kf > H + A1:
                    dyz[:, H + A1:].zero_()
            dt1, dy1 = self._ln_bwd(p + ".attention.output.LayerNorm", da, sv.ln1, run.p_hid, sv.seed_ln1,
                                    dysum=self.Gl.get(a1.name + ".up.bias"), dy_out=dyz[:, :H])
            self._adapter_bwd(run, a1, dy1, sv.z1, sv.ob, sv.seed_ad1, dz_out=dyz[:, H:H + A1], pooled=pooled)
            L.gemm(dyz, a1.WF, out_bf16=dctx)
            if pooled is not None and not any((a1.name + k) in self.Gl for k in (".up.weight", ".down.weight", ".down.bias")):
                self._dyz_pool.setdefault(self._dyz_shape, []).append(pooled)
        else:
            dt1, dy1 = self._ln_bwd(p + ".attention.output.LayerNorm", da, sv.ln1, run.p_hid, sv.seed_ln1,
                                    dysum=self.Gl.get(a1.name + ".up.bias") if a1 is not None else None)
            do = dy1
            if a1 is not None:
                do = self._adapter_bwd(run, a1, dy1, sv.z1, sv.ob, sv.seed_ad1)
            L.gemm(do, W["WoT"], out_bf16=dctx)
        if self.reducer is not None:
            self.reducer.window()
        if not sv.emd:
            dqkv = self._attn_bwd(run, sv, dctx)
            for t in range(3 if self.lora_r else 0):
                self._lora_bwd(run, li, t, dqkv[:, t * H:(t + 1) * H], sv.xkv)
            dx = torch.empty(N, H, dtype=F32, device=dev)
            L.gemm(dqkv, W["WqkvT"], aux=dt1, aux_kind=L.AUX_ADD_F32, out_f32=dx)
            return dx, None
        if sv.kvp is not None:
            dq_op, dkv_op = self._attn_bwd_qrows(run, sv, dctx)
        else:
            dqkv = self._attn_bwd(run, sv, dctx)
            dq_op, dkv_op = dqkv[:, :H], dqkv[:, H:]
            for t in range(3 if self.lora_r else 0):
                self._lora_bwd(run, li, t, dqkv[:, t * H:(t + 1) * H], sv.xq if t == 0 else sv.xkv)
        dq = torch.empty(N, H, dtype=F32, device=dev)
        L.gemm(dq_op, W["WqkvT"][:, :H], aux=dt1, aux_kind=L.AUX_ADD_F32, out_f32=dq)
        return dq, dkv_op

    def _layer_bwd_compact(self, run, sv: "LayerSave", dout: torch.Tensor, cb: Packing):
        li = sv.li
        W, (a1, a2) = self.Lw[li], self.sites[li]
        H, I, dev = self.H, self.I, self.dev
        Np = dout.shape[0]
        p = f"deberta.encoder.layer.{li}"
        pairs = [(t, torch.empty(Np, t.shape[1], dtype=t.dtype, device=dev))
                 for t in (sv.qkv, sv.ctx, sv.hpre, sv.z1 if a1 is not None else None, sv.z2 if a2 is not None else None) if t is not None]
        L.gather_rows_multi(pairs, cb.sel32)
        got = {id(src): dst for src, dst in pairs}
        qkv, ctx, hpre = got[id(sv.qkv)], got[id(sv.ctx)], got[id(sv.hpre)]
        dt2, dy2, dy2p = self._ln_bwd(p + ".output.LayerNorm", dout, sv.ln2, run.p_hid, sv.seed_ln2,
                                      dysum=self.Gl.get(a2.name + ".up.bias") if a2 is not None else None, cb=cb)
        df = dy2
        if a2 is not None:
            df = self._adapter_bwd(run, a2, dy2, got[id(sv.z2)], sv.fb, sv.seed_ad2, pad=(dy2p, sv.z2))
        del dy2p
        dh = torch.empty(Np, I, dtype=BF16, device=dev)
        L.gemm(df, W["WdT"], aux=hpre, aux_kind=L.AUX_MUL_BF16, out_bf16=dh)
        da = torch.empty(Np, H, dtype=F32, device=dev)
        L.gemm(dh, W["WiT"], aux=dt2, aux_kind=L.AUX_ADD_F32, out_f32=da)
        del dh, hpre
        dctx = torch.empty(Np, H, dtype=BF16, device=dev)
        if a1 is not None and a1.merged:
            A1, Kf = a1.A, a1.WF.shape[1]
            dyz = self._dyz_compact
            if dyz is None or tuple(dyz.shape) != (Np, Kf):
                dyz = self._dyz_compact = torch.zeros(Np, Kf, dtype=BF16, device=dev)
            dt1, dy1, dy1p = self._ln_bwd(p + ".attention.output.LayerNorm", da, sv.ln1, run.p_hid, sv.seed_ln1,
                                          dysum=self.Gl.get(a1.name + ".up.bias"), dy_out=dyz[:, :H], cb=cb)
            self._adapter_bwd(run, a1, dy1, got[id(sv.z1)], sv.ob, sv.seed_ad1, dz_out=dyz[:, H:H + A1], pad=(dy1p, sv.z1))
            L.gemm(dyz, a1.WF, out_bf16=dctx)
        else:
            dt1, dy1, dy1p = self._ln_bwd(p + ".attention.output.LayerNorm", da, sv.ln1, run.p_hid, sv.seed_ln1,
                                          dysum=self.Gl.get(a1.name + ".up.bias") if a1 is not None else None, cb=cb)
            do = dy1
            if a1 is not None:
                do = self._adapter_bwd(run, a1, dy1, got[id(sv.z1)], sv.ob, sv.seed_ad1, pad=(dy1p, sv.z1))
            L.gemm(do, W["WoT"], out_bf16=dctx)
        del dy1p
        svc = dataclasses.replace(sv, qkv=qkv, ctx=ctx)
        dqkv = self._attn_bwd(run, svc, dctx)
        sv.psave = sv.msave = None
        if not sv.emd:
            dx = torch.empty(Np, H, dtype=F32, device=dev)
            L.gemm(dqkv, W["WqkvT"], aux=dt1, aux_kind=L.AUX_ADD_F32, out_f32=dx)
            return dx, None
        dq = torch.empty(Np, H, dtype=F32, device=dev)
        L.gemm(dqkv[:, :H], W["WqkvT"][:, :H], aux=dt1, aux_kind=L.AUX_ADD_F32, out_f32=dq)
        return dq, dqkv[:, H:]

    def _attn_bwd(self, run, sv, dctx):
        dqkv = torch.empty(dctx.shape[0], 3 * self.H, dtype=BF16, device=self.dev)
        st = disent_attn_bwd(self, run, sv, dctx, dqkv, None, defer_pos=True)
        if run.pos_chain is not None and sv.extra:
            run.pos_extra = (st, sv.seed_pos)
        elif run.pos_chain is not None:
            run.pos_chain.add(st, sv.seed_pos)
        return dqkv

    def _attn_bwd_qrows(self, run, sv, dctx):
        B, S, H, nh, dev = run.B, run.S, self.H, self.nh, self.dev
        pl = run.dec_plan
        R, Sp = pl.R, _ru(S, 64)
        rmin, rcnt = _relidx_range(S, self.cfg)
        dqc = torch.empty(R, H, dtype=BF16, device=dev)
        dkv = torch.empty(run.N, 2 * H, dtype=BF16, device=dev)
        dpk, dpq = run.pos_chain.formed_slot() if run.pos_chain is not None else (None, None)
        ws = torch.empty(L.disent_attn_bwd_qrows_ws_bytes(R, Sp, nh), dtype=torch.uint8, device=dev)
        kvp, pqk = sv.kvp, sv.pqk
        L.disent_attn_bwd_qrows(sv.qc, pl.rseg, pl.rpos, kvp[:, :H], kvp[:, H:], pqk[:, H:], pqk[:, :H], self.relidx(S), run.mask_i32,
                                run.klen, dctx, sv.ctx, sv.lse, ATTN_SCALE, dqc, dkv[:, :H], dkv[:, H:], dpk, dpq,
                                rmin, rcnt, ws, B, S, Sp, nh, self.span2, p_drop=run.p_att, seed=sv.seed_att, row0=run.row0)
        if run.pos_chain is not None:
            run.pos_chain.add_formed(sv.seed_pos)
        return dqc, dkv

    def _dlog_operand(self, g):
        rows, Vout = g.shape
        Vp = _ru(Vout, 64)
        dlog = torch.zeros(rows, Vp, dtype=BF16, device=self.dev) if Vp != Vout else torch.empty(rows, Vp, dtype=BF16, device=self.dev)
        dlog[:, :Vout].copy_(g)
        return dlog

    def _head_bwd(self, run, rows, dlog, dq, all_rows=False, compact=False, to_rows=None):
        H, dev = self.H, self.dev
        R, Vp = dlog.shape
        Vout = run.Vout
        if Vout == self.V:
            tableT = self.ETb
        else:
            tableT = torch.zeros(H, Vp, dtype=BF16, device=dev)
            tableT[:, :Vout] = self.Ansb.t()
        dhl = L.zeros(R, H, dtype=F32, device=dev)
        if R >= 2048:
            L.gemm(dlog, tableT, out_f32=dhl)
        else:
            L.gemm(dlog, tableT, out_f32=dhl, splitk=max(2, min(16, Vp // 8192)), ws=self.sk_ws)
        hn = run.head_norm
        if compact:
            sub, pre = hn, run.head_pre
        else:
            rl = rows.long()
            sub, pre = NormRef(hn.t[rl].contiguous(), hn.stats[rl].contiguous(), hn.gamma, hn.beta), run.head_pre[rl].contiguous()
        dt, _ = self._ln_bwd("lm_predictions.lm_head.LayerNorm", dhl, sub, 0.0, 0, want_dy_bf16=False)
        dpre = torch.empty(R, H, dtype=BF16, device=dev)
        L.dropout_gelu_bwd(dt, pre, 0.0, 0, out_bf16=dpre)
        dqr = torch.empty(R, H, dtype=F32, device=dev)
        L.gemm(dpre, self.WhT, out_f32=dqr)
        if all_rows:
            dq.add_(dqr)
        else:
            L.scatter_rows_f32(dqr, rows if to_rows is None else to_rows, dq)

    def backward(self, run, gloss: Optional[torch.Tensor], glogits: Optional[torch.Tensor] = None, attach: bool = True,
                 ghid=None):
        if not run.save:
            raise RuntimeError("forward was run without gradient bookkeeping")
        with L.seed_word(run.seed_word):
            return self._backward(run, gloss, glogits, attach, ghid)

    def _hid_grad(self, run, ghid, i):
        g = ghid[i] if ghid is not None and i < len(ghid) else None
        if g is None:
            return None
        g = g.reshape(run.B * run.S, self.H).to(F32)
        return g.index_select(0, run.pk.sel) if run.pk is not None else g.contiguous()

    def _backward(self, run, gloss, glogits, attach, ghid=None):
        cfg, H, dev = self.cfg, self.H, self.dev
        B, S, T = run.B, run.S, run.T
        N = run.N
        pk = run.pk
        if run.plan is not None and run.live_version != self.live_version:
            raise RuntimeError("requires_grad of a trainable parameter changed between this step's forward and its backward: "
                               "the forward saved what the live set of ITS time needs; change the flags between steps")
        if attach:
            self.attach_grads()
        reducer = self.reducer
        runs = lambda stage: self._stage_runs(run, stage)
        if ghid is not None and all(g is None for g in ghid):
            ghid = None
        if run.logit_rows is not None and run.logit_rows.numel() == 0 and reducer is None and ghid is None:
            return

        red = _Ready(self, run, reducer) if reducer is not None else None
        run.dw_pending, run.dw_ready_keys, run.dw_count = [], [], 0
        dec = run.dec_plan
        cb = run.cb = run.bwd_rows if (glogits is None and ghid is None and gloss is not None and dec is None and pk is None) else None
        run.bwd_compact = cb is not None
        dq = L.zeros(dec.R if dec is not None else (cb.n if cb is not None else N), H, dtype=F32, device=dev)
        Vout = run.Vout
        Vp = _ru(Vout, 64)
        if gloss is not None and run.labels is not None:
            rows = run.rows_i32
            R = rows.numel()
            if R > 0:
                dlog = torch.empty(R, Vp, dtype=BF16, device=dev)
                gs = gloss.detach().to(F32) if (isinstance(gloss, torch.Tensor) and gloss.is_cuda) else float(gloss)
                ar = torch.arange(R, dtype=torch.int32, device=dev)
                L.ce_bwd_rows(run.logits_c, run.labels_c, ar, Vout, Vp, run.row_lse, run.loss_acc, gs, dlog)
                if dec is not None:
                    self._head_bwd(run, None, dlog, dq, all_rows=True, compact=True)
                else:
                    self._head_bwd(run, rows, dlog, dq, to_rows=cb.inv32[rows.long()] if cb is not None else None)
                del dlog
        if glogits is not None and run.logit_rows is not None:
            rows = run.logit_rows
            R = rows.numel()
            if R > 0:
                gl = glogits.reshape(R, Vout)
                if dec is not None:
                    self._head_bwd(run, None, self._dlog_operand(gl.index_select(0, dec.order)), dq, all_rows=True, compact=True)
                else:
                    self._head_bwd(run, rows, self._dlog_operand(gl), dq, compact=True)
        elif glogits is not None and dec is not None:
            if dec.R:
                gl = glogits.reshape(B * S, Vout).index_select(0, dec.grid)
                self._head_bwd(run, None, self._dlog_operand(gl), dq, all_rows=True, compact=True)
        elif glogits is not None:
            gl = glogits.reshape(B * S, Vout)
            if pk is not None:
                gl = gl.index_select(0, pk.sel)
            self._head_bwd(run, torch.arange(N, dtype=torch.int32, device=dev), self._dlog_operand(gl), dq, all_rows=True)

        def stage_done(key):
            run.dw_ready_keys.append(key)
            self._dw_flush(run, red)

        D = self.prompt_depth

# ... 345 lines not shown
```

### frozenbilm_amd/lib.py

```python
from __future__ import annotations

import ctypes as C
import os
import re
from typing import Optional

import torch

HERE = os.path.dirname(os.path.abspath(__file__))
LIB_PATH = os.environ.get("FBL_LIB") or os.path.join(HERE, "libfbl.so")

ACT_NONE, ACT_GELU, ACT_RELU, ACT_GELU_GRAD = 0, 1, 2, 3
AUX_NONE, AUX_ADD_F32, AUX_ADD_BF16, AUX_MUL_DGELU_BF16, AUX_MUL_POS_BF16, AUX_MUL_BF16 = 0, 1, 2, 3, 4, 5
ABI_VERSION = 9

_CTYPES = {"int": C.c_int, "int64_t": C.c_int64, "float": C.c_float, "uint64_t": C.c_uint64}
_DECL = re.compile(r"(?:^|[;{}])\s*([\w\s*]+?)\s*\b(fbl_\w+)\s*\(([^;()]*)\)\s*(?=;)")


def _ctype(text: str, decl: str):
    if "*" in text:
        return C.c_void_p
    words = [w for w in text.split() if w != "const"]
    if not 1 <= len(words) <= 2 or words[0] not in _CTYPES or not words[-1].isidentifier():
        raise ValueError(f"{decl}: no ctypes mapping for '{text.strip()}'")
    return _CTYPES[words[0]]


def parse_signatures(src: str) -> dict:
    src = re.sub(r"/\*.*?\*/|//[^\n]*", "", src, flags=re.S)
    src = re.sub(r"^[ \t]*#.*$", "", src, flags=re.M)
    out = {}
    for ret, name, params in _DECL.findall(src):
        params = [] if params.strip() in ("", "void") else params.split(",")
        out[name] = (_ctype(ret, name), [_ctype(p, name) for p in params])
    unparsed = set(re.findall(r"\b(fbl_\w+)\s*\(", src)) - set(out)
    if unparsed:
        raise ValueError(f"{', '.join(sorted(unparsed))}: declaration not understood")
    return out


def _header_signatures(header: str) -> dict:
    p = os.path.join(os.path.dirname(HERE), "include", header)
    if not os.path.exists(p):
        raise RuntimeError(f"{p} not found: the binding of libfbl.so takes its argument types from the C headers")
    with open(p) as f:
        return parse_signatures(f.read())


SIGNATURES = _header_signatures("fbl.h")
MHA_SIGNATURES = _header_signatures("fbl_mha.h")
QROWS_SIGNATURES = _header_signatures("fbl_qrows.h")
LIVE_SIGNATURES = _header_signatures("fbl_live.h")
PREDICT_SIGNATURES = _header_signatures("fbl_predict.h")
GROUP_SIGNATURES = _header_signatures("fbl_groups.h")
LORA_SIGNATURES = _header_signatures("fbl_lora.h")
EMA_SIGNATURES = _header_signatures("fbl_ema.h")
PROMPT_SIGNATURES = _header_signatures("fbl_prompt.h")

ROWS_SIGNATURES = _header_signatures("fbl_rows.h")
PROMPT_LAYERS_SIGNATURES = _header_signatures("fbl_prompt_layers.h")

_LIB = None


def load(path: Optional[str] = None):
    global _LIB
    if _LIB is not None and path is None:
        return _LIB
    p = path or LIB_PATH
    if not os.path.exists(p):
        raise RuntimeError(
            f"{p} not found: the FrozenBiLM MI355X path needs its HIP library (python -m frozenbilm_amd.build); "
            "there is no CPU/eager fallback")
    lib = C.CDLL(p)
    for name, (res, args) in (*SIGNATURES.items(), *MHA_SIGNATURES.items(), *QROWS_SIGNATURES.items(),
                              *LIVE_SIGNATURES.items(), *PREDICT_SIGNATURES.items(), *GROUP_SIGNATURES.items(),
                              *LORA_SIGNATURES.items(), *EMA_SIGNATURES.items(), *PROMPT_SIGNATURES.items(),
                              *ROWS_SIGNATURES.items(), *PROMPT_LAYERS_SIGNATURES.items()):
        fn = getattr(lib, name)
        fn.restype = res
        fn.argtypes = args
    ver = lib.fbl_abi_version()
    if ver != ABI_VERSION:
        raise RuntimeError(f"{p} has ABI version {ver}, this binding needs {ABI_VERSION}: rebuild it "
                           "(python -m frozenbilm_amd.build --force)")
    if path is None:
        _LIB = lib
    return lib


def _p(t: Optional[torch.Tensor]):
    return None if t is None else t.data_ptr()


def _stream():
    return torch.cuda.current_stream().cuda_stream


_AUX = {}
_NO_AUX = set()


def exclude_from_aux(stream: "torch.cuda.Stream"):
    _NO_AUX.add(stream.cuda_stream)



def set_aux_stream(stream: Optional["torch.cuda.Stream"], device=None):
    dev = torch.device("cuda", torch.cuda.current_device()) if device is None else torch.device(device)
    idx = dev.index if dev.index is not None else torch.cuda.current_device()
    if stream is None:
        _AUX.pop(idx, None)
    else:
        _AUX[idx] = stream


def _aux_stream():
    st = _AUX.get(torch.cuda.current_device())
    if st is None:
        return None
    h = st.cuda_stream
    cur = torch.cuda.current_stream().cuda_stream
    return None if (h == cur or cur in _NO_AUX) else h


_SEED_WORD = None


class seed_word:

    def __init__(self, t: Optional[torch.Tensor]):
        self.t, self.prev = t, None

    def __enter__(self):
        global _SEED_WORD
        if self.t is not None:
            assert self.t.dtype == torch.int64 and self.t.is_cuda and self.t.numel() >= 1
        self.prev, _SEED_WORD = _SEED_WORD, self.t
        return self

    def __exit__(self, *exc):
        global _SEED_WORD
        _SEED_WORD = self.prev
        return False


def _seed_dev():
    return None if _SEED_WORD is None else _SEED_WORD.data_ptr()


def _chk(code: int, name: str):
    if code != 0:
        raise RuntimeError(f"{name} failed with code {code}")


def _req(t: torch.Tensor, dtype, name: str):
    if t.dtype != dtype:
        raise TypeError(f"{name}: expected {dtype}, got {t.dtype}")
    if not t.is_cuda:
        raise RuntimeError(f"{name}: tensor must live in HBM (cuda device), got {t.device}")


def _rows2d(t: torch.Tensor, name: str):
    if t.dim() != 2 or t.stride(1) != 1:
        raise ValueError(f"{name}: need a 2-D row-major view (stride(1)==1), got shape {tuple(t.shape)} strides {t.stride()}")
    return t.stride(0)


def gemm_plan(M, N, K, batch=1, splitk=1):
    return load().fbl_gemm_plan(int(M), int(N), int(K), int(batch), int(splitk))


GK_NAMES = ("G8_256", "G8_224", "G8_128", "G8_SPLITK", "T2_256", "T2_224", "T2_128", "T2_64_RING", "T2_128_SPLITK")
ENTRY_PLAIN, ENTRY_ADAPTER_DOWN, ENTRY_DENSE_ADAPTER_DOWN, ENTRY_ADAPTER_TAIL = 0, 1, 2, 3
GPQ = dict(out_f32=1, out_bf16=2, out_pre=4, bias=8, rowscale=16, aux=32, dropout=64, ws=128, aux_stream=256, r_norm=512)


def gemm_plan_launches(entry, M, N, K, *, lda=None, ldb=None, ldc=None, ld_aux=0, seg_n=0, act=ACT_NONE, aux_kind=AUX_NONE,
                       opts=(), batch=1, splitk=1, ws_floats=0, n_cu=256):
    flags = 0
    for o in opts:
        flags |= GPQ[o]
    out = (C.c_int32 * 13)()
    code = load().fbl_gemm_plan_launches(int(entry), int(M), int(N), int(K), int(K if lda is None else lda),
                                         int(K if ldb is None else ldb), int(N if ldc is None else ldc), int(ld_aux),
                                         int(seg_n), int(act), int(aux_kind), flags, int(batch), int(splitk), int(ws_floats),
                                         int(n_cu), out)
    if code:
        return code, None
    launches = [(GK_NAMES[out[5 + 4 * i]], out[6 + 4 * i], out[7 + 4 * i], bool(out[8 + 4 * i])) for i in range(out[0])]
    return 0, dict(launches=launches, splitk=out[1], k8_per=out[2], fold=bool(out[3]), big8=bool(out[4]))


def gemm(A, B, *, bias=None, rowscale=None, alpha=1.0, act=ACT_NONE, aux=None, aux_kind=AUX_NONE, out_f32=None,
         out_bf16=None, out_pre=None, splitk=1, M=None, N=None, ws=None):
    _req(A, torch.bfloat16, "A")
    _req(B, torch.bfloat16, "B")
    batch = 1
    sA = sB = sC = sX = 0
    if A.dim() == 3:
        batch = A.shape[0]
        sA, sB = A.stride(0), (B.stride(0) if B.dim() == 3 else 0)
        A2, B2 = A[0], (B[0] if B.dim() == 3 else B)
    else:
        A2, B2 = A, B
    lda, ldb = _rows2d(A2, "A"), _rows2d(B2, "B")
    Mv, K = A2.shape
    Nv = B2.shape[0]
    assert B2.shape[1] == K, (A2.shape, B2.shape)
    M = Mv if M is None else M
    N = Nv if N is None else N
    ldc = None
    for o, dt in ((out_f32, torch.float32), (out_bf16, torch.bfloat16), (out_pre, torch.bfloat16)):
        if o is None:
            continue
        _req(o, dt, "out")
        o2 = o[0] if o.dim() == 3 else o
        l = _rows2d(o2, "out")
        assert o2.shape[0] >= M and o2.shape[1] >= N, (o2.shape, M, N)
        if ldc is None:
            ldc = l
            sC = o.stride(0) if o.dim() == 3 else 0
        assert ldc == l, "all outputs of one GEMM must share the row stride"
    ld_aux = 0
    if aux is not None:
        a2 = aux[0] if aux.dim() == 3 else aux
        ld_aux = _rows2d(a2, "aux")
        sX = aux.stride(0) if aux.dim() == 3 else 0
        _req(aux, torch.float32 if aux_kind == AUX_ADD_F32 else torch.bfloat16, "aux")
    sBias = 0
    if bias is not None:
        _req(bias, torch.float32, "bias")
        if bias.dim() == 2:
            sBias = bias.stride(0)
    if rowscale is not None:
        _req(rowscale, torch.float32, "rowscale")
    code = load().fbl_gemm_bf16_nt(_p(A), lda, _p(B), ldb, M, N, K, _p(bias), _p(rowscale), float(alpha), act, aux_kind,
                                   _p(aux), ld_aux, _p(out_f32), _p(out_bf16), _p(out_pre), ldc or 0, batch, sA, sB, sC,
                                   sX, sBias, splitk, _p(ws), (ws.numel() if ws is not None else 0), _stream(), _aux_stream())
    _chk(code, "fbl_gemm_bf16_nt")


def adapter_down_fwd(x, wd, bias, z, *, A=None, p_drop=0.0, seed=0):
    _req(x, torch.bfloat16, "x"); _req(wd, torch.bfloat16, "wd"); _req(z, torch.bfloat16, "z")
    _req(bias, torch.float32, "bias")
    ldx, ldw, ldz = _rows2d(x, "x"), _rows2d(wd, "wd"), _rows2d(z, "z")
    M, K = x.shape
    A = wd.shape[0] if A is None else A
    assert wd.shape[1] == K and z.shape[0] >= M and z.shape[1] >= A
    _chk(load().fbl_adapter_down_fwd(_p(x), ldx, _p(wd), ldw, M, A, K, _p(bias), float(p_drop), int(seed), _seed_dev(), _p(z), ldz,
                                     _stream()), "fbl_adapter_down_fwd")


def dense_adapter_down_fwd(x, wm, bias_m, N1, z, *, y_f32=None, y_bf16=None, p_drop=0.0, seed=0):
    _req(x, torch.bfloat16, "x"); _req(wm, torch.bfloat16, "wm"); _req(z, torch.bfloat16, "z"); _req(bias_m, torch.float32, "bias")
    ldx, ldw, ldz = _rows2d(x, "x"), _rows2d(wm, "wm"), _rows2d(z, "z")
    M, K = x.shape
    A = wm.shape[0] - N1
    assert wm.shape[1] == K and A > 0 and z.shape[0] >= M and z.shape[1] >= A and bias_m.numel() >= N1 + A
    ldy = None
    for o, dt in ((y_f32, torch.float32), (y_bf16, torch.bfloat16)):
        if o is not None:
            _req(o, dt, "y")
            l = _rows2d(o, "y")
            assert ldy is None or ldy == l
            ldy = l
    _chk(load().fbl_dense_adapter_down_fwd(_p(x), ldx, _p(wm), ldw, M, N1, A, K, _p(bias_m), _p(y_f32), _p(y_bf16), ldy or 0,
                                           float(p_drop), int(seed), _seed_dev(), _p(z), ldz, _stream(), _aux_stream()),
         "fbl_dense_adapter_down_fwd")


def adapter_up_resid_fwd(z, wu, bias_u, x, out_t, *, A=None, p_drop=0.0, seed=0, r_plain=None, r_norm=None):
    _req(z, torch.bfloat16, "z"); _req(wu, torch.bfloat16, "wu"); _req(x, torch.bfloat16, "x"); _req(out_t, torch.float32, "out_t")
    ldz, ldw, ldx, ldt = _rows2d(z, "z"), _rows2d(wu, "wu"), _rows2d(x, "x"), _rows2d(out_t, "out_t")
    M, H = x.shape
    A = wu.shape[1] if A is None else A
    assert wu.shape[0] == H and z.shape[0] >= M and z.shape[1] >= A and out_t.shape[0] >= M and out_t.shape[1] >= H
    if bias_u is not None:
        _req(bias_u, torch.float32, "bias_u")
    if (r_plain is None) == (r_norm is None):
        raise ValueError("exactly one of r_plain / r_norm")
    rs = rg = rb = rm = None
    if r_norm is not None:
        rt, rs, rg, rb, rm = r_norm
        for t in (rt, rs, rg, rb):
            _req(t, torch.float32, "r_norm")
        assert rs.is_contiguous() and rs.numel() >= 2 * M
        if rm is not None:
            _req(rm, torch.int32, "rowmask")
    else:
        rt = r_plain
        _req(rt, torch.float32, "r_plain")
    ld_r = _rows2d(rt, "residual")
    assert rt.shape[0] >= M and rt.shape[1] >= H
    _chk(load().fbl_adapter_up_resid_fwd(_p(z), ldz, _p(wu), ldw, M, H, int(A), _p(bias_u), _p(x), ldx, float(p_drop),
                                         int(seed), _seed_dev(), _p(rt), ld_r, _p(rs), _p(rg), _p(rb), _p(rm), _p(out_t), ldt,
                                         _stream()), "fbl_adapter_up_resid_fwd")


def gemm_tn_acc(A, B, out_f32, ws, *, M=None, N=None, K=None, splitk=8):
    _req(A, torch.bfloat16, "A"); _req(B, torch.bfloat16, "B"); _req(out_f32, torch.float32, "out")
    lda, ldb, ldc = _rows2d(A, "A"), _rows2d(B, "B"), _rows2d(out_f32, "out")
    K = min(A.shape[0], B.shape[0]) if K is None else K
    M = A.shape[1] if M is None else M
    N = B.shape[1] if N is None else N
    assert out_f32.shape[0] >= M and out_f32.shape[1] >= N
    _chk(load().fbl_gemm_bf16_tn_acc(_p(A), lda, _p(B), ldb, M, N, K, _p(out_f32), ldc, splitk, _p(ws), ws.numel(),
                                     _stream()), "fbl_gemm_bf16_tn_acc")


ADW_MAX_ADAPTERS, ADW_MAX_SEGMENTS = 16, 24


def adapter_bwd_dw(groups, *, A):
    segs = [sg for g in groups for sg in g[0]]
    assert 0 < len(groups) <= ADW_MAX_ADAPTERS and 0 < len(segs) <= ADW_MAX_SEGMENTS
    N, H = segs[0][0].shape
    Ap = segs[0][1].shape[1]
    strides = []
    for g in groups:
        lds = None
        for dy, z, dz, x in g[0]:
            for t, n in ((dy, "dy"), (z, "z"), (dz, "dz"), (x, "x")):
                _req(t, torch.bfloat16, n)
            assert dy.shape == (N, H) and x.shape == (N, H) and z.shape == (N, Ap) and dz.shape == (N, Ap) and Ap >= A
            l = (_rows2d(dy, "dy"), _rows2d(z, "z"), _rows2d(dz, "dz"), _rows2d(x, "x"))
            assert lds is None or l == lds, "the segments of an adapter share their row strides"
            lds = l
        strides.append(lds)
    for _, dWu, dWd, dbd in groups:
        for o, shp in ((dWu, (H, A)), (dWd, (A, H)), (dbd, (A,))):
            if o is not None:
                _req(o, torch.float32, "out")
                assert tuple(o.shape) == shp and o.is_contiguous(), (tuple(o.shape), shp)
    first = [0]
    for g in groups:
        first.append(first[-1] + len(g[0]))
    seg_first = (C.c_int32 * len(first))(*first)
    tab = lambda ts: (C.c_void_p * len(ts))(*[_p(t) for t in ts])
    ldt = lambda k: (C.c_int64 * len(strides))(*[st[k] for st in strides])
    _chk(load().fbl_adapter_bwd_dw(len(groups), seg_first, tab([s[0] for s in segs]), tab([s[1] for s in segs]),
                                   tab([s[2] for s in segs]), tab([s[3] for s in segs]), ldt(0), ldt(1), ldt(2), ldt(3),
                                   N, H, int(A), Ap, tab([g[1] for g in groups]), tab([g[2] for g in groups]),
                                   tab([g[3] for g in groups]), _stream()), "fbl_adapter_bwd_dw")


def embed_gather(ids, E, vproj, T, out_t):
    B, L = ids.shape
    H = E.shape[1]
    _req(ids, torch.int64, "ids"); _req(E, torch.float32, "E"); _req(out_t, torch.float32, "out_t")
    assert ids.is_contiguous() and E.is_contiguous() and out_t.is_contiguous()
    if vproj is not None:
        _req(vproj, torch.float32, "vproj")
        assert vproj.is_contiguous()
    _chk(load().fbl_embed_gather(_p(ids), _p(E), _p(vproj), B, T, L, H, _p(out_t), _stream()), "fbl_embed_gather")


PROMPT_MAX = 128


def embed_assemble(ids, E, vproj, prompt, T, L, out_t):
    P, H = prompt.shape
    B = out_t.shape[0]
    _req(prompt, torch.float32, "prompt"); _req(out_t, torch.float32, "out_t")
    assert prompt.is_contiguous() and out_t.is_contiguous() and tuple(out_t.shape) == (B, T + P + L, H), (out_t.shape, T, P, L, H)
    if ids is not None:
        _req(ids, torch.int64, "ids"); _req(E, torch.float32, "E")
        assert ids.is_contiguous() and E.is_contiguous() and tuple(ids.shape) == (B, L) and E.shape[1] == H
    if vproj is not None:
        _req(vproj, torch.float32, "vproj")
        assert vproj.is_contiguous() and vproj.numel() == B * T * H
    _chk(load().fbl_embed_assemble(_p(ids), _p(E) if ids is not None else None, _p(vproj), _p(prompt), B, T, P, L, H, _p(out_t),
                                   _stream()), "fbl_embed_assemble")


def prompt_grad(dt, row0, B, S, T, g):
    P, H = g.shape
    _req(dt, torch.float32, "dt"); _req(g, torch.float32, "g")
    assert dt.is_contiguous() and g.is_contiguous() and dt.dim() == 2 and dt.shape[1] == H
    if row0 is not None:
        _req(row0, torch.int32, "row0")
        assert row0.is_contiguous() and row0.numel() >= B
    else:
        assert dt.shape[0] >= B * S
    _chk(load().fbl_prompt_grad(_p(dt), _p(row0), B, S, T, P, H, _p(g), _stream()), "fbl_prompt_grad")


def _prompt_rows_checks(t, row0, B, S, T, P, H, what):
    assert t.is_contiguous() and t.dim() == 2 and t.shape[1] == H, (what, tuple(t.shape), H)
    if row0 is not None:
        _req(row0, torch.int32, "row0")
        assert row0.is_contiguous() and row0.numel() >= B
    else:
        assert S >= T + P and t.shape[0] >= B * S, (what, tuple(t.shape), B, S, T, P)


def prompt_rows_write(prompt, row0, B, S, T, out_f32=None, out_bf16=None):
    P, H = prompt.shape
    _req(prompt, torch.float32, "prompt")
    assert prompt.is_contiguous() and (out_f32 is not None or out_bf16 is not None)
    if out_f32 is not None:
        _req(out_f32, torch.float32, "out_f32")
        _prompt_rows_checks(out_f32, row0, B, S, T, P, H, "out_f32")
    if out_bf16 is not None:
        _req(out_bf16, torch.bfloat16, "out_bf16")
        _prompt_rows_checks(out_bf16, row0, B, S, T, P, H, "out_bf16")
    _chk(load().fbl_prompt_rows_write(_p(prompt), _p(row0), B, S, T, P, H, _p(out_f32), _p(out_bf16), _stream()),
         "fbl_prompt_rows_write")


def prompt_rows_grad(dx, row0, B, S, T, P, g):
    H = dx.shape[1]
    _req(dx, torch.float32, "dx")
    _prompt_rows_checks(dx, row0, B, S, T, P, H, "dx")
    if g is not None:
        _req(g, torch.float32, "g")
        assert g.is_contiguous() and tuple(g.shape) == (P, H), (tuple(g.shape), P, H)
    _chk(load().fbl_prompt_rows_grad(_p(dx), _p(row0), B, S, T, P, H, _p(g), _stream()), "fbl_prompt_rows_grad")


def ln_fwd(*, y=None, p_drop=0.0, seed=0, r_plain=None, r_norm=None, gamma, beta, eps, rowmask=None, out_t=None,
           out_stats=None, out_bf16=None, out_f32=None, N, H):
    ldy = 0
    if y is not None:
        _req(y, torch.float32, "y")
        ldy = _rows2d(y, "y")
    rt = rs = rg = rb = rm = None
    if r_norm is not None:
        rt, rs, rg, rb, rm = r_norm
    for t in (r_plain, rt, out_t, out_bf16, out_f32):
        if t is not None:
            assert t.is_contiguous()
    _chk(load().fbl_ln_fwd(_p(y), ldy, float(p_drop), int(seed), _seed_dev(), _p(r_plain), _p(rt), _p(rs), _p(rg), _p(rb), _p(rm),
                           _p(gamma), _p(beta), float(eps), _p(rowmask), _p(out_t), _p(out_stats), _p(out_bf16),
                           _p(out_f32), N, H, _stream()), "fbl_ln_fwd")


def ln_materialize(t, stats, gamma, beta, rowmask=None, add_bcast=None, S=1, out_f32=None, out_bf16=None):
    N, H = t.shape
    _chk(load().fbl_ln_materialize(_p(t), _p(stats), _p(gamma), _p(beta), _p(rowmask), _p(add_bcast), S, _p(out_f32),
                                   _p(out_bf16), N, H, _stream()), "fbl_ln_materialize")


def ln_bwd_ws(H, device):
    return torch.empty(load().fbl_ln_bwd_ws_floats(H), dtype=torch.float32, device=device)


def ln_bwd(dout, t, stats, gamma, *, rowmask=None, p_drop=0.0, seed=0, out_dt=None, out_dy_bf16=None, out_dy_f32=None,
           dgamma=None, dbeta=None, dysum=None, ws=None):
    N, H = t.shape
    assert dout.is_contiguous() and t.is_contiguous()
    ld_dyb = _rows2d(out_dy_bf16, "out_dy_bf16") if out_dy_bf16 is not None else 0
    _chk(load().fbl_ln_bwd(_p(dout), _p(rowmask), _p(t), _p(stats), _p(gamma), float(p_drop), int(seed), _seed_dev(), _p(out_dt),
                           _p(out_dy_bf16), _p(out_dy_f32), _p(dgamma), _p(dbeta), _p(dysum), _p(ws), N, H, ld_dyb,
                           _stream()), "fbl_ln_bwd")


def im2col3(x_bf16, out_bf16, B, S, H):
    _chk(load().fbl_im2col3(_p(x_bf16), _p(out_bf16), B, S, H, _stream()), "fbl_im2col3")


def col2im3(dcol, dx, B, S, H, accumulate):
    _chk(load().fbl_col2im3(_p(dcol), _p(dx), B, S, H, int(accumulate), _stream()), "fbl_col2im3")


def dropout_gelu_fwd(c, p_drop, seed, out_f32):
    _chk(load().fbl_dropout_gelu_fwd(_p(c), float(p_drop), int(seed), _seed_dev(), _p(out_f32), c.numel(), _stream()),
         "fbl_dropout_gelu_fwd")


def dropout_gelu_bwd(dy, c, p_drop, seed, out_bf16=None, out_f32=None):
    _chk(load().fbl_dropout_gelu_bwd(_p(dy), _p(c), float(p_drop), int(seed), _seed_dev(), _p(out_bf16), _p(out_f32), c.numel(),
                                     _stream()), "fbl_dropout_gelu_bwd")


def video_stage_f16(feats, row_off, n_rows, T):
    assert feats.dtype == torch.float16 and feats.is_contiguous() and row_off.dtype == torch.int64 and n_rows.dtype == torch.int32
    B, F_ = n_rows.numel(), feats.shape[1]
    video = torch.empty(B, T, F_, dtype=torch.float32, device=feats.device)
    vlen = torch.empty(B, dtype=torch.int64, device=feats.device)
    vmask = torch.empty(B, T, dtype=torch.int64, device=feats.device)
    _chk(load().fbl_video_stage_f16(_p(feats), _p(row_off), _p(n_rows), B, T, F_, _p(video), _p(vlen), _p(vmask), _stream()),
         "fbl_video_stage_f16")
    return video, vlen, vmask


def mask_tokens(ids, labels, special_ids, p, mask_token_id, vocab_size, seed):
    assert ids.dtype == torch.int64 and labels.dtype == torch.int64 and ids.is_contiguous() and labels.is_contiguous()
    assert special_ids.dtype == torch.int64
    _chk(load().fbl_mask_tokens(_p(ids), _p(labels), ids.numel(), _p(special_ids), special_ids.numel(), float(p),
                                int(mask_token_id), int(vocab_size), int(seed), _stream()), "fbl_mask_tokens")


def transpose_batched_bf16(src, src_off, dst, dst_off, rows, cols):
    assert src.dtype == torch.bfloat16 and dst.dtype == torch.bfloat16
    assert src_off.dtype == torch.int64 and dst_off.dtype == torch.int64 and src_off.numel() == dst_off.numel()
    _chk(load().fbl_transpose_batched_bf16(_p(src), _p(src_off), _p(dst), _p(dst_off), src_off.numel(), rows, cols,
# ... 146 lines not shown
                                  _p(PQX), _p(PKX), B, S, Sp, nh, span2, _row0(row0, B, True), _stream()),
         "fbl_attn_bwd_prep")


def attn_rowdot(dO, O, out, B, S, nh):
    ld = _rows2d(dO, "dO")
    assert _rows2d(O, "O") == ld
    _chk(load().fbl_attn_rowdot(_p(dO), _p(O), ld, _p(out), B, S, nh, _stream()), "fbl_attn_rowdot")


def disent_attn_bwd_ds(q, k, v, dO, pk, pq, relidx, mask, lse, Dv, scale, dV, dS, dST, B, S, Sp, nh, span2,
                       p_drop=0.0, seed=0, klen=None, border=None, lin=0, row0=None):
    ldq = _rows2d(q, "q")
    assert _rows2d(k, "k") == ldq and _rows2d(v, "v") == ldq
    ldo, ldp, lddv = _rows2d(dO, "dO"), _rows2d(pk, "pk"), _rows2d(dV, "dV")
    assert _rows2d(pq, "pq") == ldp
    _chk(load().fbl_disent_attn_bwd_ds(_p(q), _p(k), _p(v), ldq, _p(dO), ldo, _p(pk), _p(pq), ldp,
                                       _p(relidx), _p(mask), _p(klen), _p(border), _p(lse), _p(Dv), float(scale), float(p_drop), int(seed), _seed_dev(),
                                       _p(dV), lddv, _p(dS), _p(dST), B, S, Sp, nh, span2, int(lin), _row0(row0, B, klen), _stream()),
         "fbl_disent_attn_bwd_ds")


def disent_attn_bwd_dspk(psave, msave, q, v, dO, pqx, lse, Dv, scale, dK, dV, dS, dST, B, S, Sp, nh, p_drop=0.0, seed=0, klen=None,
                         border=None, row0=None):
    _req(psave, torch.bfloat16, "psave"); _req(msave, torch.float32, "msave"); _req(pqx, torch.bfloat16, "pqx")
    assert psave.is_contiguous() and msave.is_contiguous() and pqx.is_contiguous()
    assert psave.numel() == B * nh * Sp * Sp and msave.numel() == B * nh * (Sp // 64) * S and pqx.numel() == nh * 64 * 2 * Sp
    ldq, ldv, ldo, lddk, lddv = _rows2d(q, "q"), _rows2d(v, "v"), _rows2d(dO, "dO"), _rows2d(dK, "dK"), _rows2d(dV, "dV")
    _chk(load().fbl_disent_attn_bwd_dspk(_p(psave), _p(msave), _p(q), ldq, _p(v), ldv, _p(dO), ldo, _p(pqx), _p(klen), _p(border),
                                         _p(lse), _p(Dv), float(scale), float(p_drop), int(seed), _seed_dev(), _p(dK), lddk,
                                         _p(dV), lddv, _p(dS), _p(dST), B, S, Sp, nh, _row0(row0, B, klen), _stream()),
         "fbl_disent_attn_bwd_dspk")


def disent_attn_bwd_dq(dS, k, pkx, dQ, B, S, Sp, nh, klen=None, border=None, row0=None):
    _req(dS, torch.bfloat16, "dS"); _req(pkx, torch.bfloat16, "pkx")
    assert dS.is_contiguous() and pkx.is_contiguous() and dS.numel() == B * nh * Sp * Sp and pkx.numel() == nh * 2 * Sp * 64
    ldk, lddq = _rows2d(k, "k"), _rows2d(dQ, "dQ")
    _chk(load().fbl_disent_attn_bwd_dq(_p(dS), _p(k), ldk, _p(pkx), _p(klen), _p(border), _p(dQ), lddq, B, S, Sp, nh,
                                       _row0(row0, B, klen), _stream()), "fbl_disent_attn_bwd_dq")


def attn_pos_grad(neg, Xs, Ys, dlo, dcnt, dcnt_max, out, B, S, Sp, nh, rcnt, klen=None, row0=None):
    E = len(Xs)
    assert E == len(Ys) and E > 0
    ldy = _rows2d(Ys[0], "Y")
    for x, y in zip(Xs, Ys):
        _req(x, torch.bfloat16, "X"); _req(y, torch.bfloat16, "Y")
        assert x.is_contiguous() and x.numel() == B * nh * Sp * Sp and _rows2d(y, "Y") == ldy
    _req(dlo, torch.int16, "dlo"); _req(dcnt, torch.int16, "dcnt"); _req(out, torch.float32, "out")
    assert dlo.numel() == rcnt and dcnt.numel() == rcnt and out.is_contiguous() and out.numel() == E * nh * rcnt * 64
    xp = (C.c_void_p * E)(*[x.data_ptr() for x in Xs])
    yp = (C.c_void_p * E)(*[y.data_ptr() for y in Ys])
    _chk(load().fbl_attn_pos_grad(int(neg), xp, yp, ldy, _p(dlo), _p(dcnt), int(dcnt_max), _p(klen), _row0(row0, B, klen), _p(out),
                                  E, B, S, Sp, nh, int(rcnt), _stream()), "fbl_attn_pos_grad")


def disent_attn_bwd_shear(dST, QT, PQT, relidx, dK, B, S, Sp, nh, span2, klen=None, lin=0, border=None, row0=None):
    lddk = _rows2d(dK, "dK")
    sh, sb, sd = head_strides(B, Sp, nh, True)
    _chk(load().fbl_disent_attn_bwd_shear(_p(dST), _p(QT), sh, sb, sd, _p(PQT), _p(relidx), _p(klen), _p(border), _p(dK), lddk,
                                          int(lin), B, S, Sp, nh, span2, _row0(row0, B, klen), _stream()),
         "fbl_disent_attn_bwd_shear")


def ce_fwd(logits, labels, V, row_lse, loss_sum_cnt):
    ldv = _rows2d(logits, "logits")
    _req(logits, torch.float32, "logits"); _req(labels, torch.int64, "labels")
    _chk(load().fbl_ce_fwd(_p(logits), ldv, _p(labels), logits.shape[0], V, _p(row_lse), _p(loss_sum_cnt), _stream()),
         "fbl_ce_fwd")


def ce_bwd_rows(logits, labels, rows, V, Vp, row_lse, loss_sum_cnt, gscale, dlogits):
    ldv = _rows2d(logits, "logits")
    _req(rows, torch.int32, "rows")
    gdev = None
    if isinstance(gscale, torch.Tensor):
        gdev = gscale.reshape(1)
        _req(gdev, torch.float32, "gscale")
        gscale = 1.0
    _chk(load().fbl_ce_bwd_rows(_p(logits), ldv, _p(labels), _p(rows), rows.numel(), V, Vp, _p(row_lse),
                                _p(loss_sum_cnt), float(gscale), _p(gdev), _p(dlogits), _stream()), "fbl_ce_bwd_rows")


PREDICT_MAX_K = 16


def row_predict(logits, V, k, labels=None, row_lse=None):
    ldv = _rows2d(logits, "logits")
    _req(logits, torch.float32, "logits")
    R, dev = logits.shape[0], logits.device
    if not 1 <= int(k) <= PREDICT_MAX_K:
        raise ValueError(f"k = {k}: fbl_row_predict takes 1..{PREDICT_MAX_K}")
    if labels is not None:
        _req(labels, torch.int64, "labels")
        assert labels.is_contiguous() and labels.numel() == R
    if row_lse is not None:
        _req(row_lse, torch.float32, "row_lse")
        assert row_lse.is_contiguous() and row_lse.numel() == R
    ids = torch.empty(R, k, dtype=torch.int32, device=dev)
    lp = torch.empty(R, k, dtype=torch.float32, device=dev)
    rank = torch.empty(R, dtype=torch.int32, device=dev) if labels is not None else None
    nll = torch.empty(R, dtype=torch.float32, device=dev) if labels is not None else None
    h = load()
    nbytes = h.fbl_row_predict_ws_bytes(R, int(V), int(k))
    if nbytes < 0:
        _chk(nbytes, "fbl_row_predict_ws_bytes")
    ws = torch.empty(max(nbytes, 8) // 8, dtype=torch.int64, device=dev)
    _chk(h.fbl_row_predict(_p(logits), ldv, R, int(V), int(k), _p(labels), _p(row_lse), _p(ids), _p(lp), _p(rank), _p(nll),
                           _p(ws), nbytes, _stream()), "fbl_row_predict")
    return ids, lp, rank, nll


def gather_rows_bf16(x, rows, out):
    ld = _rows2d(x, "x")
    _chk(load().fbl_gather_rows_bf16(_p(x), ld, _p(rows), rows.numel(), x.shape[1], _p(out), _stream()),
         "fbl_gather_rows_bf16")


def scatter_rows_f32(x, rows, out):
    ld = _rows2d(out, "out")
    _chk(load().fbl_scatter_rows_f32(_p(x), _p(rows), rows.numel(), x.shape[1], _p(out), ld, _stream()),
         "fbl_scatter_rows_f32")


GATHER_MAX_TENSORS = 8


def gather_rows_multi(pairs, sel):
    _req(sel, torch.int32, "sel")
    Np, n = sel.numel(), len(pairs)
    assert sel.is_contiguous() and 1 <= n <= GATHER_MAX_TENSORS
    rb, sl, dl = [], [], []
    for src, dst in pairs:
        assert src.dtype == dst.dtype and src.is_cuda and dst.is_cuda and src.shape[1] == dst.shape[1] and dst.shape[0] == Np
        es = src.element_size()
        rb.append(src.shape[1] * es); sl.append(_rows2d(src, "src") * es); dl.append(_rows2d(dst, "dst") * es)
    tab = lambda ts: (C.c_void_p * n)(*[_p(t) for t in ts])
    arr = lambda v: (C.c_int64 * n)(*v)
    _chk(load().fbl_gather_rows_multi(n, tab([s for s, _ in pairs]), tab([d for _, d in pairs]), arr(rb), arr(sl), arr(dl), _p(sel),
                                      Np, _stream()), "fbl_gather_rows_multi")


def scatter_rows_zero_bf16(src, inv, out):
    _req(src, torch.bfloat16, "src"); _req(out, torch.bfloat16, "out"); _req(inv, torch.int32, "inv")
    assert inv.is_contiguous() and inv.numel() == out.shape[0] and src.shape[1] == out.shape[1]
    _chk(load().fbl_scatter_rows_zero_bf16(_p(src), _rows2d(src, "src"), _p(inv), out.shape[0], out.shape[1], _p(out),
                                           _rows2d(out, "out"), _stream()), "fbl_scatter_rows_zero_bf16")


def ln_bwd_rows(dout, inv, t, stats, gamma, *, rowmask=None, p_drop=0.0, seed=0, out_dt=None, out_dy_bf16=None, out_dy_pad,
                dgamma=None, dbeta=None, dysum=None, ws=None):
    N, H = t.shape
    _req(inv, torch.int32, "inv"); _req(out_dy_pad, torch.bfloat16, "out_dy_pad")
    assert dout.is_contiguous() and t.is_contiguous() and inv.is_contiguous() and inv.numel() == N
    assert out_dy_pad.is_contiguous() and tuple(out_dy_pad.shape) == (N, H) and dout.shape[1] == H
    assert out_dt is None or (out_dt.is_contiguous() and out_dt.shape == dout.shape)
    ld_dyb = _rows2d(out_dy_bf16, "out_dy_bf16") if out_dy_bf16 is not None else 0
    _chk(load().fbl_ln_bwd_rows(_p(dout), _p(inv), _p(rowmask), _p(t), _p(stats), _p(gamma), float(p_drop), int(seed), _seed_dev(),
                                _p(out_dt), _p(out_dy_bf16), ld_dyb, _p(out_dy_pad), _p(dgamma), _p(dbeta), _p(dysum), _p(ws), N, H,
                                _stream()), "fbl_ln_bwd_rows")


_SUMSQ_WS = {}


def sumsq(x, out, ws=None):
    if ws is None:
        ws = _SUMSQ_WS.get(x.device)
        if ws is None:
            ws = _SUMSQ_WS[x.device] = torch.empty(load().fbl_sumsq_ws_floats(), dtype=torch.float32, device=x.device)
    _chk(load().fbl_sumsq(_p(x), x.numel(), _p(out), _p(ws), _stream()), "fbl_sumsq")


def adam_flat(p, g, m, v, lr, beta1, beta2, eps, weight_decay, step, sumsq_t=None, max_norm=0.0, grad_scale=1.0):
    _chk(load().fbl_adam_flat(_p(p), _p(g), _p(m), _p(v), p.numel(), float(lr), float(beta1), float(beta2), float(eps),
                              float(weight_decay), int(step), _p(sumsq_t), float(max_norm), float(grad_scale),
                              _stream()), "fbl_adam_flat")


LIVE_MAX_RANGES = 1024


def live_table(ranges, n: int, device) -> torch.Tensor:
    if len(ranges) > LIVE_MAX_RANGES:
        raise ValueError(f"{len(ranges)} live ranges: the kernels take {LIVE_MAX_RANGES}")
    tab, cum, last = [len(ranges), 0], 0, 0
    for b, e in ranges:
        if b < last or e <= b or e > n or b % 8 or e % 8:
            raise ValueError(f"live range [{b}, {e}) of {n}: ranges must be sorted, disjoint, non-empty and 8-aligned")
        tab += [b, cum]
        cum += e - b
        last = e
    tab[1] = cum
    return torch.tensor(tab, dtype=torch.int64, device=device)


def sumsq_live(x, table, out, ws):
    _req(x, torch.float32, "x"); _req(table, torch.int64, "table")
    _chk(load().fbl_sumsq_live(_p(x), x.numel(), _p(table), _p(out), _p(ws), _stream()), "fbl_sumsq_live")


def adam_flat_live(p, g, m, v, table, lr, beta1, beta2, eps, weight_decay, step, sumsq_t=None, max_norm=0.0, grad_scale=1.0):
    _req(table, torch.int64, "table")
    _chk(load().fbl_adam_flat_live(_p(p), _p(g), _p(m), _p(v), p.numel(), _p(table), float(lr), float(beta1), float(beta2),
                                   float(eps), float(weight_decay), int(step), _p(sumsq_t), float(max_norm), float(grad_scale),
                                   _stream()), "fbl_adam_flat_live")


ADAM_MAX_GROUPS = 64
ADAM_GROUP_FLOATS = 6


def group_table(segments, n: int, device, n_groups: int = ADAM_MAX_GROUPS) -> torch.Tensor:
    if len(segments) > LIVE_MAX_RANGES:
        raise ValueError(f"{len(segments)} segments: the kernel takes {LIVE_MAX_RANGES}")
    if not 1 <= n_groups <= ADAM_MAX_GROUPS:
        raise ValueError(f"{n_groups} parameter groups: the kernel takes 1 .. {ADAM_MAX_GROUPS}")
    tab, cum, last = [len(segments), 0], 0, 0
    for b, e, k in segments:
        if b < last or e <= b or e > n or b % 8 or e % 8:
            raise ValueError(f"segment [{b}, {e}) of {n}: segments must be sorted, disjoint, non-empty and 8-aligned")
        if not 0 <= k < n_groups:
            raise ValueError(f"segment [{b}, {e}): group {k} outside [0, {n_groups})")
        tab += [b, cum, k]
        cum += e - b
        last = e
    tab[1] = cum
    return torch.tensor(tab, dtype=torch.int64, device=device)


def adam_hyper(groups):
    if not 1 <= len(groups) <= ADAM_MAX_GROUPS:
        raise ValueError(f"{len(groups)} parameter groups: the kernel takes 1 .. {ADAM_MAX_GROUPS}")
    flat = []
    for lr, b1, b2, eps, wd, dec in groups:
        flat += [float(lr), float(b1), float(b2), float(eps), float(wd), 1.0 if dec else 0.0]
    return (C.c_float * len(flat))(*flat)


def adam_flat_groups(p, g, m, v, table, groups, step, sumsq_t=None, max_norm=0.0, grad_scale=1.0):
    _req(table, torch.int64, "table")
    hyper = groups if isinstance(groups, C.Array) else adam_hyper(groups)
    _chk(load().fbl_adam_flat_groups(_p(p), _p(g), _p(m), _p(v), p.numel(), _p(table), len(hyper) // ADAM_GROUP_FLOATS, hyper,
                                     int(step), _p(sumsq_t), float(max_norm), float(grad_scale), _stream()),
         "fbl_adam_flat_groups")


def _flat32(t, n, name):
    _req(t, torch.float32, name)
    if t.numel() != n or not t.is_contiguous():
        raise ValueError(f"{name}: a contiguous buffer of {n} elements is needed, got {tuple(t.shape)}")
    if n % 8 or t.data_ptr() % 16:
        raise ValueError(f"{name}: {n} elements at {t.data_ptr():#x}: a multiple of 8 elements on a 16-byte boundary is needed")


def adam_flat_groups_ema(p, g, m, v, ema, table, groups, step, ema_w, sumsq_t=None, max_norm=0.0, grad_scale=1.0):
    _req(table, torch.int64, "table")
    for t, name in ((p, "p"), (g, "g"), (m, "m"), (v, "v"), (ema, "ema")):
        _flat32(t, p.numel(), name)
    if ema.device != p.device:
        raise ValueError(f"ema lives on {ema.device}, the parameters on {p.device}")
    if not 0.0 < float(ema_w) <= 1.0:
        raise ValueError(f"ema_w = {ema_w}: the weight of the new parameter lies in (0, 1]")
    hyper = groups if isinstance(groups, C.Array) else adam_hyper(groups)
    _chk(load().fbl_adam_flat_groups_ema(_p(p), _p(g), _p(m), _p(v), _p(ema), p.numel(), _p(table),
                                         len(hyper) // ADAM_GROUP_FLOATS, hyper, int(step), _p(sumsq_t), float(max_norm),
                                         float(grad_scale), float(ema_w), _stream()), "fbl_adam_flat_groups_ema")


def swap_(a, b):
    _flat32(a, a.numel(), "a"); _flat32(b, a.numel(), "b")
    if a.device != b.device:
        raise ValueError(f"a lives on {a.device}, b on {b.device}")
    lo, hi = sorted((a.data_ptr(), b.data_ptr()))
    if a.numel() and lo + 4 * a.numel() > hi:
        raise ValueError("swap_: the two buffers overlap")
    _chk(load().fbl_swap_f32(_p(a), _p(b), a.numel(), _stream()), "fbl_swap_f32")


LORA_MAX_RANK, LORA_SITE_WORDS = 64, 16


class LoraTable:

    def __init__(self, sites, device):
        import struct

        words, self.keep = [], []
        for s in sites:
            W, A, B, dst, dstT, d32 = s["W"], s["A"], s["B"], s["dst"], s["dstT"], s.get("dst32")
            _req(W, torch.float32, "W"); _req(A, torch.float32, "A"); _req(B, torch.float32, "B")
            _req(dst, torch.bfloat16, "dst"); _req(dstT, torch.bfloat16, "dstT")
            O, I = W.shape
            r = A.shape[0]
            assert A.shape == (r, I) and B.shape == (O, r) and A.is_contiguous() and B.is_contiguous(), (W.shape, A.shape, B.shape)
            assert tuple(dst.shape) == (O, I) and tuple(dstT.shape) == (I, O)
            ld32 = 0
            if d32 is not None:
                _req(d32, torch.float32, "dst32")
                assert tuple(d32.shape) == (O, I)
                ld32 = _rows2d(d32, "dst32")
            bits = struct.unpack("<I", struct.pack("<f", float(s["scale"])))[0]
            words += [W.data_ptr(), _rows2d(W, "W"), A.data_ptr(), B.data_ptr(), dst.data_ptr(), _rows2d(dst, "dst"),
                      dstT.data_ptr(), _rows2d(dstT, "dstT"), _p(d32) or 0, ld32, O, I, r, bits, 0, 0]
            self.keep.append((W, A, B, dst, dstT, d32))
        self.n = len(sites)
        self.host = (C.c_int64 * max(len(words), 1))(*words)
        self.dev = torch.tensor(words or [0], dtype=torch.int64, device=device)


# ... 108 lines not shown
```

Measured before the change: 853.0 samples/s.

## Gather compact rows inside adapter dW kernel instead of materializing padded gradients

Adds a rows variant of the adapter weight-gradient kernel. It reads compacted dy/z/dz rows through the inverse row map and visits only the 64-row tiles that contain live tokens. LayerNorm backward can then skip writing the zero-padded full-length bf16 gradient buffer. This removes a large padded write and read per adapter in the compacted backward path, at the cost of indirect gathered loads, extra map staging in LDS and a more complex pipeline.

Result: no change. 852.9 samples/s (-0.0%).

```diff
diff --git a/frozenbilm_amd/build.py b/frozenbilm_amd/build.py
--- a/frozenbilm_amd/build.py
+++ b/frozenbilm_amd/build.py
@@ -34,7 +34,7 @@
 
 def _deps_mtime() -> float:
     hdrs = [os.path.join(CSRC, f) for f in os.listdir(CSRC) if f.endswith(".h")]
-    hdrs += [os.path.join(os.path.dirname(HERE), "include", h) for h in ("fbl.h", "fbl_mha.h", "fbl_qrows.h", "fbl_live.h", "fbl_predict.h", "fbl_groups.h", "fbl_lora.h", "fbl_ema.h", "fbl_prompt.h", "fbl_rows.h", "fbl_prompt_layers.h")]
+    hdrs += [os.path.join(os.path.dirname(HERE), "include", h) for h in ("fbl.h", "fbl_mha.h", "fbl_qrows.h", "fbl_live.h", "fbl_predict.h", "fbl_groups.h", "fbl_lora.h", "fbl_ema.h", "fbl_prompt.h", "fbl_rows.h", "fbl_prompt_layers.h", "fbl_adw_rows.h")]
     return max(os.path.getmtime(h) for h in hdrs)
 
 
diff --git a/frozenbilm_amd/csrc/adapter_dw.hip b/frozenbilm_amd/csrc/adapter_dw.hip
--- a/frozenbilm_amd/csrc/adapter_dw.hip
+++ b/frozenbilm_amd/csrc/adapter_dw.hip
@@ -1,5 +1,6 @@
 #include "fbl_common.h"
 #include "../../include/fbl.h"
+#include "../../include/fbl_adw_rows.h"
 
 namespace {
 
@@ -14,13 +15,19 @@
   int ld_dy[ADW_MAX_OUT], ld_z[ADW_MAX_OUT], ld_dz[ADW_MAX_OUT], ld_x[ADW_MAX_OUT];
   int N, H, A, tiles_h, n_out;
 };
+struct AdwRowsArgs : AdwArgs {
+  const int32_t* inv;
+  const int32_t* tiles;
+  int n_tiles, Np;
+};
+typedef __attribute__((ext_vector_type(4))) int adw_i32x4;
 
 constexpr int WI = 2;
 constexpr int WT = WI * 32;
 constexpr int ADW_LDW = WT + 16;
 
-template <int NT, int WHICH>
-__device__ __forceinline__ void adw_tile(const AdwArgs& g, bf16* sW, bf16* sS, const int th, const int o) {
+template <int NT, int WHICH, bool ROWS = false, class Args = AdwArgs>
+__device__ __forceinline__ void adw_tile(const Args& g, bf16* sW, bf16* sS, const int th, const int o, int* sM = nullptr) {
   constexpr int AP = NT * 32;
   constexpr int LDS_ = AP + 16;
   constexpr int NCH = AP / 8;
@@ -31,7 +38,8 @@
   const int wm = wave >> 1, wn = wave & 1;
   const int h0 = th * WT;
   const long ldw = WHICH ? g.ld_x[o] : g.ld_dy[o], lds = WHICH ? g.ld_dz[o] : g.ld_z[o];
-  const int nk = (g.N + 63) / 64;
+  int nk = (g.N + 63) / 64;
+  if constexpr (ROWS) nk = g.n_tiles;
   const int s0 = g.seg_first[o], s1 = g.seg_first[o + 1];
   const int total = (s1 - s0) * nk;
   const int frow = lane & 15, fg = lane >> 4;
@@ -81,6 +89,66 @@
     }
     if (++kt_n == nk) { kt_n = 0; ++sg_n; }
   };
+  [[maybe_unused]] int pkS[SPT];
+  [[maybe_unused]] unsigned live = 0;
+  [[maybe_unused]] int mreg = -1;
+  [[maybe_unused]] int ktA = 0, ktB = 0, ktC = 0, jC = 0;
+  if constexpr (ROWS) {
+#pragma unroll
+    for (int t = 0; t < SPT; ++t) pkS[t] = (rS[t] << 2) | ((gS[t] - rS[t] * (int)lds) << 16);
+  }
+  auto tile_at = [&](int j) {
+    if constexpr (ROWS) return min(max(g.tiles[j], 0), (g.N - 1) >> 6);
+    else return 0;
+  };
+  auto tile_step = [&]() {
+    if constexpr (ROWS) {
+      ktA = ktB; ktB = ktC;
+      if (++jC == g.n_tiles) jC = 0;
+      ktC = tile_at(jC);
+    }
+  };
+  auto fetch_map = [&](int kt) {
+    if constexpr (ROWS) {
+      const int r = kt * 64 + lane;
+      const int m = g.inv[min(r, g.N - 1)];
+      mreg = r < g.N ? m : -1;
+    }
+  };
+  auto load_tile_rows = [&](const int* mp) {
+    if constexpr (ROWS) {
+      const bf16* S = WHICH ? g.seg[sg_n].dz : g.seg[sg_n].z;
+      const int np1 = g.Np - 1;
+      if constexpr (WHICH == 0) {
+        const bf16* W = g.seg[sg_n].dy;
+        const int cW = gW[0] - rW[0] * (int)ldw;
+#pragma unroll
+        for (int t = 0; t < WPT; ++t) {
+          const int m = mp[rW[0] + t * (256 / WCH)];
+          rw[t] = *(const bf16x8*)(W + (unsigned)(min(max(m, 0), np1) * (int)ldw + cW));
+        }
+      } else {
+        const bf16* W = g.seg[sg_n].x + (long)ktA * 64 * ldw;
+        const int left = g.N - ktA * 64;
+        if (left < 64) {
+#pragma unroll
+          for (int t = 0; t < WPT; ++t) rw[t] = *(const bf16x8*)(W + gW[t] - (long)max(rW[t] - (left - 1), 0) * ldw);
+        } else {
+#pragma unroll
+          for (int t = 0; t < WPT; ++t) rw[t] = *(const bf16x8*)(W + gW[t]);
+        }
+      }
+      unsigned lv = 0;
+#pragma unroll
+      for (int t = 0; t < SPT; ++t) {
+        const int m = *(const int*)((const char*)mp + (pkS[t] & 0xffff));
+        rs[t] = *(const bf16x8*)(S + (unsigned)(min(max(m, 0), np1) * (int)lds + (pkS[t] >> 16)));
+        lv |= ((unsigned)~m >> 31) << t;
+      }
+      live = lv;
+      if (++kt_n == nk) { kt_n = 0; ++sg_n; }
+    }
+  };
   const bool do_cs = WHICH == 1 && th == 0 && g.dbd[o] != nullptr;
   const bf16x2 ones2 = {(bf16)1.0f, (bf16)1.0f};
   float cs[NT];
@@ -88,14 +156,50 @@
   for (int j = 0; j < NT; ++j) cs[j] = 0.f;
   const bf16* fW = sW + (fg * 4 + (frow >> 2)) * ADW_LDW + (frow & 3) * 4 + wm * (WI * 16);
   const bf16* fS = sS + (fg * 4 + (frow >> 2)) * LDS_ + (frow & 3) * 4 + wn * (NT * 16);
-  if (total > 0) load_tile();
+  if constexpr (ROWS) {
+    if (total > 0) {
+      ktA = tile_at(0);
+      jC = g.n_tiles > 1 ? 1 : 0;
+      ktB = tile_at(jC);
+      if (++jC == g.n_tiles) jC = 0;
+      ktC = tile_at(jC);
+      if (wave == 0) {
+        fetch_map(ktA);
+        sM[lane] = mreg;
+        fetch_map(ktB);
+      }
+      __syncthreads();
+      load_tile_rows(sM);
+    }
+  } else {
+    if (total > 0) load_tile();
+  }
   for (int it = 0; it < total; ++it) {
 #pragma unroll
     for (int t = 0; t < WPT; ++t) *(bf16x8*)(sW + lW[t]) = rw[t];
-#pragma unroll
-    for (int t = 0; t < SPT; ++t) *(bf16x8*)(sS + lS[t]) = rs[t];
+    if constexpr (ROWS) {
+#pragma unroll
+      for (int t = 0; t < SPT; ++t) {
+        union { bf16x8 v; adw_i32x4 i; } u;
+        u.v = rs[t];
+        u.i &= __builtin_amdgcn_sbfe(live, t, 1);
+        *(bf16x8*)(sS + lS[t]) = u.v;
+      }
+      if (wave == 0) sM[((it + 1) & 1) * 64 + lane] = mreg;
+    } else {
+#pragma unroll
+      for (int t = 0; t < SPT; ++t) *(bf16x8*)(sS + lS[t]) = rs[t];
+    }
     __syncthreads();
-    if (it + 1 < total) load_tile();
+    if constexpr (ROWS) {
+      if (it + 1 < total) {
+        tile_step();
+        if (wave == 0) fetch_map(ktB);
+        load_tile_rows(sM + ((it + 1) & 1) * 64);
+      }
+    } else {
+      if (it + 1 < total) load_tile();
+    }
 #pragma unroll
     for (int s = 0; s < 2; ++s) {
       bf16x8 wf[WI], sf[NT];
@@ -196,19 +300,30 @@
   else adw_tile<NT, 1>(g, sW, sS, th, o);
 }
 
-}
-
-extern "C" int fbl_adapter_bwd_dw(int n_adapters, const int32_t* seg_first, const void* const* dy_bf16, const void* const* z_bf16,
-                                  const void* const* dz_bf16, const void* const* x_bf16, const int64_t* ld_dy,
-                                  const int64_t* ld_z, const int64_t* ld_dz, const int64_t* ld_x, int N, int H, int A, int Ap,
-                                  float* const* dWu, float* const* dWd, float* const* dbd, void* stream) {
-  if (n_adapters <= 0 || N <= 0 || H <= 0 || A <= 0) return 0;
+template <int NT>
+__global__ __launch_bounds__(256, 2) void adapter_dw_rows_kernel(AdwRowsArgs g) {
+  __shared__ __attribute__((aligned(16))) bf16 sW[64 * ADW_LDW];
+  __shared__ __attribute__((aligned(16))) bf16 sS[64 * (NT * 32 + 16)];
+  __shared__ int sM[2 * 64];
+  const int lin = blockIdx.x, xcd = lin & 7, slot = lin >> 3;
+  const int p = (slot / g.tiles_h) * 8 + xcd, th = slot % g.tiles_h;
+  if (p >= 2 * g.n_out) return;
+  const int o = p >> 1;
+  if ((p & 1) == 0) adw_tile<NT, 0, true>(g, sW, sS, th, o, sM);
+  else adw_tile<NT, 1, true>(g, sW, sS, th, o, sM);
+}
+
+}
+
+static int adw_fill(AdwArgs& g, int n_adapters, const int32_t* seg_first, const void* const* dy_bf16, const void* const* z_bf16,
+                    const void* const* dz_bf16, const void* const* x_bf16, const int64_t* ld_dy, const int64_t* ld_z,
+                    const int64_t* ld_dz, const int64_t* ld_x, int N, int H, int A, int Ap, float* const* dWu, float* const* dWd,
+                    float* const* dbd, int64_t Np) {
   if (n_adapters > ADW_MAX_OUT || !seg_first || seg_first[0] != 0) return FBL_ERR_ARG;
   const int nseg = seg_first[n_adapters];
   if (nseg <= 0 || nseg > ADW_MAX_SEG) return FBL_ERR_ARG;
   if (Ap < A || (Ap % 64) || Ap > 256 || (H % 8)) return FBL_ERR_SHAPE;
   if (!dy_bf16 || !z_bf16 || !dz_bf16 || !x_bf16 || !ld_dy || !ld_z || !ld_dz || !ld_x) return FBL_ERR_ARG;
-  AdwArgs g{};
   for (int o = 0; o < n_adapters; ++o) {
     if (seg_first[o + 1] < seg_first[o]) return FBL_ERR_ARG;
     g.seg_first[o] = seg_first[o];
@@ -218,6 +333,7 @@
     if ((ld_dy[o] % 8) || (ld_z[o] % 8) || (ld_dz[o] % 8) || (ld_x[o] % 8)) return FBL_ERR_ALIGN;
     if (ld_dy[o] < H || ld_x[o] < H || ld_z[o] < Ap || ld_dz[o] < Ap) return FBL_ERR_ARG;
     if ((ld_dy[o] | ld_x[o] | ld_z[o] | ld_dz[o]) >> 24) return FBL_ERR_ARG;
+    if (Np > 0 && ((Np * ld_dy[o]) >> 31 || (Np * ld_z[o]) >> 31 || (Np * ld_dz[o]) >> 31)) return FBL_ERR_ARG;
     g.ld_dy[o] = (int)ld_dy[o]; g.ld_z[o] = (int)ld_z[o]; g.ld_dz[o] = (int)ld_dz[o]; g.ld_x[o] = (int)ld_x[o];
   }
   g.seg_first[n_adapters] = nseg;
@@ -228,6 +344,42 @@
   g.N = N; g.H = H; g.A = A;
   g.tiles_h = (H + WT - 1) / WT;
   g.n_out = n_adapters;
+  return 0;
+}
+
+extern "C" int fbl_adapter_bwd_dw_rows(int n_adapters, const int32_t* seg_first, const void* const* dy_bf16,
+                                       const void* const* z_bf16, const void* const* dz_bf16, const void* const* x_bf16,
+                                       const int64_t* ld_dy, const int64_t* ld_z, const int64_t* ld_dz, const int64_t* ld_x,
+                                       int N_pad, int H, int A, int Ap, float* const* dWu, float* const* dWd, float* const* dbd,
+                                       const int32_t* inv, const int32_t* tiles, int n_tiles, int Np, void* stream) {
+  if (n_adapters <= 0 || N_pad <= 0 || H <= 0 || A <= 0) return 0;
+  AdwRowsArgs g{};
+  const int rc = adw_fill(g, n_adapters, seg_first, dy_bf16, z_bf16, dz_bf16, x_bf16, ld_dy, ld_z, ld_dz, ld_x, N_pad, H, A, Ap,
+                          dWu, dWd, dbd, Np > 0 ? Np : 1);
+  if (rc) return rc;
+  if (!inv || !tiles || n_tiles < 0 || n_tiles > (N_pad + 63) / 64 || Np > N_pad) return FBL_ERR_ARG;
+  if (Np <= 0 || n_tiles == 0) return 0;
+  g.inv = inv; g.tiles = tiles; g.n_tiles = n_tiles; g.Np = Np;
+  dim3 grid((unsigned)(((2 * n_adapters + 7) / 8) * 8 * g.tiles_h));
+  switch (Ap / 64) {
+    case 1: hipLaunchKernelGGL(adapter_dw_rows_kernel<2>, grid, dim3(256), 0, (hipStream_t)stream, g); break;
+    case 2: hipLaunchKernelGGL(adapter_dw_rows_kernel<4>, grid, dim3(256), 0, (hipStream_t)stream, g); break;
+    case 3: hipLaunchKernelGGL(adapter_dw_rows_kernel<6>, grid, dim3(256), 0, (hipStream_t)stream, g); break;
+    default: hipLaunchKernelGGL(adapter_dw_rows_kernel<8>, grid, dim3(256), 0, (hipStream_t)stream, g); break;
+  }
+  FBL_CHECK_LAUNCH();
+  return 0;
+}
+
+extern "C" int fbl_adapter_bwd_dw(int n_adapters, const int32_t* seg_first, const void* const* dy_bf16, const void* const* z_bf16,
+                                  const void* const* dz_bf16, const void* const* x_bf16, const int64_t* ld_dy,
+                                  const int64_t* ld_z, const int64_t* ld_dz, const int64_t* ld_x, int N, int H, int A, int Ap,
+                                  float* const* dWu, float* const* dWd, float* const* dbd, void* stream) {
+  if (n_adapters <= 0 || N <= 0 || H <= 0 || A <= 0) return 0;
+  AdwArgs g{};
+  const int rc = adw_fill(g, n_adapters, seg_first, dy_bf16, z_bf16, dz_bf16, x_bf16, ld_dy, ld_z, ld_dz, ld_x, N, H, A, Ap, dWu,
+                          dWd, dbd, 0);
+  if (rc) return rc;
   dim3 grid((unsigned)(((2 * n_adapters + 7) / 8) * 8 * g.tiles_h));
   switch (Ap / 64) {
     case 1: hipLaunchKernelGGL(adapter_dw_kernel<2>, grid, dim3(256), 0, (hipStream_t)stream, g); break;
diff --git a/frozenbilm_amd/csrc/rowops.hip b/frozenbilm_amd/csrc/rowops.hip
--- a/frozenbilm_amd/csrc/rowops.hip
+++ b/frozenbilm_amd/csrc/rowops.hip
@@ -4,6 +4,7 @@
 #include "../../include/fbl_groups.h"
 #include "../../include/fbl_ema.h"
 #include "../../include/fbl_rows.h"
+#include "../../include/fbl_adw_rows.h"
 
 namespace {
 
@@ -192,8 +193,10 @@
       const int cr = a.inv[row];
       if (cr < 0) {
         const float z[VEC] = {};
-#pragma unroll
-        for (int it = 0; it < NIT; ++it) stb<VEC>(a.out_dy_pad + (long)row * H + (it * 64 + lane) * VEC, z);
+        if (a.out_dy_pad) {
+#pragma unroll
+          for (int it = 0; it < NIT; ++it) stb<VEC>(a.out_dy_pad + (long)row * H + (it * 64 + lane) * VEC, z);
+        }
         continue;
       }
       crow = cr;
@@ -237,7 +240,7 @@
       if (a.out_dt) stf<VEC>(a.out_dt + crow * H + col, dt);
       if (a.out_dy_bf16) stb<VEC>(a.out_dy_bf16 + crow * a.ld_dyb + col, dy);
       if (a.out_dy_f32) stf<VEC>(a.out_dy_f32 + crow * H + col, dy);
-      if (ROWS) stb<VEC>(a.out_dy_pad + (long)row * H + col, dy);
+      if (ROWS && a.out_dy_pad) stb<VEC>(a.out_dy_pad + (long)row * H + col, dy);
     }
   }
 #pragma unroll
@@ -288,7 +291,7 @@
     bool pad_zero = false;
     if (ROWS) {
       const int cr = a.inv[rr];
-      pad_zero = live && cr < 0;
+      pad_zero = live && cr < 0 && a.out_dy_pad;
       live = live && cr >= 0;
       crow = cr;
     }
@@ -343,7 +346,7 @@
         if (a.out_dt) stf<VEC>(a.out_dt + crow * H + col, dt);
         if (a.out_dy_bf16) stb<VEC>(a.out_dy_bf16 + crow * a.ld_dyb + col, dy);
         if (a.out_dy_f32) stf<VEC>(a.out_dy_f32 + crow * H + col, dy);
-        if (ROWS) stb<VEC>(a.out_dy_pad + (long)row * H + col, dy);
+        if (ROWS && a.out_dy_pad) stb<VEC>(a.out_dy_pad + (long)row * H + col, dy);
       }
     } else if (ROWS && pad_zero) {
       const float z[VEC] = {};
@@ -1189,6 +1192,20 @@
   return ln_bwd_launch<true>(a, dgamma, dbeta, dysum, (hipStream_t)stream);
 }
 
+extern "C" int fbl_ln_bwd_rows_nopad(const float* dout, const int32_t* inv, const int32_t* rowmask, const float* t,
+                                     const float* stats, const float* gamma, float p_drop, uint64_t seed, const uint64_t* seed_dev,
+                                     float* out_dt, void* out_dy_bf16, int64_t ld_dy_bf16, float* dgamma, float* dbeta,
+                                     float* dysum, float* ws, int N_pad, int H, void* stream) {
+  if (H % 64 || H > 2048) return FBL_ERR_SHAPE;
+  if (!dout || !inv || !t || !stats || !gamma || !ws) return FBL_ERR_ARG;
+  if (N_pad <= 0) return 0;
+  if (ld_dy_bf16 == 0) ld_dy_bf16 = H;
+  if (ld_dy_bf16 < H || (ld_dy_bf16 % 8)) return FBL_ERR_ALIGN;
+  LnBwdArgs a{dout, rowmask, t, stats, gamma, p_drop, seed, seed_dev, out_dt, (bf16*)out_dy_bf16, nullptr, ws, N_pad, H, ld_dy_bf16,
+              inv, nullptr};
+  return ln_bwd_launch<true>(a, dgamma, dbeta, dysum, (hipStream_t)stream);
+}
+
 extern "C" int fbl_im2col3(const void* x_bf16, void* out_bf16, int B, int S, int H, void* stream) {
   if (H % 8) return FBL_ERR_SHAPE;
   if (B * S <= 0) return 0;
diff --git a/frozenbilm_amd/engine.py b/frozenbilm_amd/engine.py
--- a/frozenbilm_amd/engine.py
+++ b/frozenbilm_amd/engine.py
@@ -63,6 +63,8 @@
     n: int
     sel32: Optional[torch.Tensor] = None
     inv32: Optional[torch.Tensor] = None
+    plen: Optional[list] = None
+    tiles32: Optional[torch.Tensor] = None
 
 
 @dataclass
@@ -396,7 +398,7 @@
         site = self.lora_sites.get((li, t))
         if not self._lora_live(site):
             return
-        run.dw_pending.append((self.lora_r, site.name, self._lora_products(site, dy, x), run.dw_count, None))
+        run.dw_pending.append((self.lora_r, site.name, self._lora_products(site, dy, x), run.dw_count, None, None))
         run.dw_count += 1
 
     def _dw_outputs(self, nm: str, Gl):
@@ -654,6 +656,7 @@
         if pk is None or (force is not True and 1.0 - pk.n / (B * S) < self.COMPACT_BWD_MIN_DROPPED):
             return None
         pk.sel32, pk.inv32 = pk.sel.to(torch.int32), pk.inv.to(torch.int32)
+        pk.tiles32 = L.live_tiles(pk.plen, S, self.dev)
         return pk
 
     def _make_packing(self, mask, full_labels, logit_rows, B, S, T) -> Optional[Packing]:
@@ -679,7 +682,7 @@
         sel = b_of * S + pos
         inv = torch.full((B * S,), -1, dtype=torch.int64, device=dev)
         inv[sel] = torch.arange(n, device=dev)
-        return Packing(row0=row0, sel=sel, inv=inv, pos=pos, n=n)
+        return Packing(row0=row0, sel=sel, inv=inv, pos=pos, n=n, plen=plen_h)
 
     def _ln(self, run, name, *, y, resid: Optional[Stream], N, p_drop=0.0, rowmask=None, want_f32=False, tail=0):
         H = self.H
@@ -1143,12 +1146,13 @@
         run.conv_c, run.conv_norm = c, out.norm
         return out
 
-    def _ln_bwd(self, name, dout, norm: NormRef, p_drop, seed, want_dy_bf16=True, dysum=None, tail=0, dy_out=None, cb=None):
+    def _ln_bwd(self, name, dout, norm: NormRef, p_drop, seed, want_dy_bf16=True, dysum=None, tail=0, dy_out=None, cb=None,
+                want_pad=True):
         N, H = dout.shape
         if cb is not None:
             dt = torch.empty(N, H, dtype=F32, device=self.dev)
             dyb = dy_out if dy_out is not None else torch.empty(N, H, dtype=BF16, device=self.dev)
-            dy_pad = torch.empty(norm.t.shape[0], H, dtype=BF16, device=self.dev)
+            dy_pad = torch.empty(norm.t.shape[0], H, dtype=BF16, device=self.dev) if want_pad else None
             L.ln_bwd_rows(dout, cb.inv32, norm.t, norm.stats, norm.gamma, rowmask=norm.rowmask, p_drop=p_drop, seed=seed, out_dt=dt,
                           out_dy_bf16=dyb, out_dy_pad=dy_pad, dgamma=self.Gl.get(name + ".weight"), dbeta=self.Gl.get(name + ".bias"),
                           dysum=dysum, ws=self._ln_ws)
@@ -1165,7 +1169,7 @@
             return dt, dyb, dt_full
         return dt, dyb
 
-    def _adapter_bwd(self, run, site: AdapterSite, dyb, z, xin_b, seed, dz_out=None, pooled=None, pad=None):
+    def _adapter_bwd(self, run, site: AdapterSite, dyb, z, xin_b, seed, dz_out=None, pooled=None, pad=None, rows=None):
         N, H = dyb.shape
         A, Ap = site.A, site.Ap
         dev = self.dev
@@ -1191,7 +1195,7 @@
         sk = max(2, min(16, dyb.shape[0] // 512))
 
         if site.grouped:
-            run.dw_pending.append((A, nm, (dyb, z, dz, xin_b), run.dw_count, pooled))
+            run.dw_pending.append((A, nm, (dyb, z, dz, xin_b), run.dw_count, pooled, rows if pad is None else None))
             run.dw_count += 1
             return dx
 
@@ -1220,15 +1224,20 @@
             take, names, rest = {}, set(), []
             for rec in pend:
                 A, nm, seg = rec[:3]
+                rows = rec[5] if len(rec) > 5 else None
                 if nm in names or len(names) >= min(self.dw_group, L.ADW_MAX_ADAPTERS):
                     rest.append(rec)
                 else:
                     names.add(nm)
-                    take.setdefault((A, getattr(seg[0], "shape", (None,))[0]), []).append((nm, seg))
-            for (A, _rows), recs in take.items():
+                    take.setdefault((A, getattr(seg[0], "shape", (None,))[0], id(rows)), (rows, []))[1].append((nm, seg))
+            for (A, _rows, _), (cb, recs) in take.items():
                 Gl = getattr(self, "Gl", None)
                 Gl = self.G if Gl is None else Gl
-                L.adapter_bwd_dw([([seg], *Engine._dw_outputs(self, nm, Gl)) for nm, seg in recs], A=A)
+                groups = [([seg], *Engine._dw_outputs(self, nm, Gl)) for nm, seg in recs]
+                if cb is not None:
+                    L.adapter_bwd_dw_rows(groups, cb.inv32, cb.tiles32, cb.n, A=A)
+                else:
+                    L.adapter_bwd_dw(groups, A=A)
             kept = {id(r) for r in rest}
             for rec in pend:
                 if id(rec) not in kept and rec[4] is not None and tuple(rec[4].shape) == self._dyz_shape:
@@ -1324,11 +1333,12 @@
         L.gather_rows_multi(pairs, cb.sel32)
         got = {id(src): dst for src, dst in pairs}
         qkv, ctx, hpre = got[id(sv.qkv)], got[id(sv.ctx)], got[id(sv.hpre)]
+        pad1, pad2 = (a is not None and not a.grouped for a in (a1, a2))
         dt2, dy2, dy2p = self._ln_bwd(p + ".output.LayerNorm", dout, sv.ln2, run.p_hid, sv.seed_ln2,
-                                      dysum=self.Gl.get(a2.name + ".up.bias") if a2 is not None else None, cb=cb)
+                                      dysum=self.Gl.get(a2.name + ".up.bias") if a2 is not None else None, cb=cb, want_pad=pad2)
         df = dy2
         if a2 is not None:
-            df = self._adapter_bwd(run, a2, dy2, got[id(sv.z2)], sv.fb, sv.seed_ad2, pad=(dy2p, sv.z2))
+            df = self._adapter_bwd(run, a2, dy2, got[id(sv.z2)], sv.fb, sv.seed_ad2, pad=(dy2p, sv.z2) if pad2 else None, rows=cb)
         del dy2p
         dh = torch.empty(Np, I, dtype=BF16, device=dev)
         L.gemm(df, W["WdT"], aux=hpre, aux_kind=L.AUX_MUL_BF16, out_bf16=dh)
@@ -1338,19 +1348,31 @@
         dctx = torch.empty(Np, H, dtype=BF16, device=dev)
         if a1 is not None and a1.merged:
             A1, Kf = a1.A, a1.WF.shape[1]
-            dyz = self._dyz_compact
-            if dyz is None or tuple(dyz.shape) != (Np, Kf):
-                dyz = self._dyz_compact = torch.zeros(Np, Kf, dtype=BF16, device=dev)
+            pooled = None
+            if not pad1:
+                if self._dyz_shape != (Np, Kf):
+                    self._dyz_pool.clear()
+                    self._dyz_shape = (Np, Kf)
+                free = self._dyz_pool.get((Np, Kf))
+                dyz = pooled = free.pop() if free else torch.zeros(Np, Kf, dtype=BF16, device=dev)
+            else:
+                dyz = self._dyz_compact
+                if dyz is None or tuple(dyz.shape) != (Np, Kf):
+                    dyz = self._dyz_compact = torch.zeros(Np, Kf, dtype=BF16, device=dev)
             dt1, dy1, dy1p = self._ln_bwd(p + ".attention.output.LayerNorm", da, sv.ln1, run.p_hid, sv.seed_ln1,
-                                          dysum=self.Gl.get(a1.name + ".up.bias"), dy_out=dyz[:, :H], cb=cb)
-            self._adapter_bwd(run, a1, dy1, got[id(sv.z1)], sv.ob, sv.seed_ad1, dz_out=dyz[:, H:H + A1], pad=(dy1p, sv.z1))
+                                          dysum=self.Gl.get(a1.name + ".up.bias"), dy_out=dyz[:, :H], cb=cb, want_pad=pad1)
+            self._adapter_bwd(run, a1, dy1, got[id(sv.z1)], sv.ob, sv.seed_ad1, dz_out=dyz[:, H:H + A1], pooled=pooled,
+                              pad=(dy1p, sv.z1) if pad1 else None, rows=cb)
             L.gemm(dyz, a1.WF, out_bf16=dctx)
+            if pooled is not None and not any((a1.name + k) in self.Gl for k in (".up.weight", ".down.weight", ".down.bias")):
+                self._dyz_pool.setdefault(self._dyz_shape, []).append(pooled)
         else:
             dt1, dy1, dy1p = self._ln_bwd(p + ".attention.output.LayerNorm", da, sv.ln1, run.p_hid, sv.seed_ln1,
-                                          dysum=self.Gl.get(a1.name + ".up.bias") if a1 is not None else None, cb=cb)
+                                          dysum=self.Gl.get(a1.name + ".up.bias") if a1 is not None else None, cb=cb, want_pad=pad1)
             do = dy1
             if a1 is not None:
-                do = self._adapter_bwd(run, a1, dy1, got[id(sv.z1)], sv.ob, sv.seed_ad1, pad=(dy1p, sv.z1))
+                do = self._adapter_bwd(run, a1, dy1, got[id(sv.z1)], sv.ob, sv.seed_ad1, pad=(dy1p, sv.z1) if pad1 else None,
+                                       rows=cb)
             L.gemm(do, W["WoT"], out_bf16=dctx)
         del dy1p
         svc = dataclasses.replace(sv, qkv=qkv, ctx=ctx)
diff --git a/frozenbilm_amd/lib.py b/frozenbilm_amd/lib.py
--- a/frozenbilm_amd/lib.py
+++ b/frozenbilm_amd/lib.py
@@ -60,6 +60,7 @@
 
 ROWS_SIGNATURES = _header_signatures("fbl_rows.h")
 PROMPT_LAYERS_SIGNATURES = _header_signatures("fbl_prompt_layers.h")
+ADW_ROWS_SIGNATURES = _header_signatures("fbl_adw_rows.h")
 
 _LIB = None
 
@@ -77,7 +78,8 @@
     for name, (res, args) in (*SIGNATURES.items(), *MHA_SIGNATURES.items(), *QROWS_SIGNATURES.items(),
                               *LIVE_SIGNATURES.items(), *PREDICT_SIGNATURES.items(), *GROUP_SIGNATURES.items(),
                               *LORA_SIGNATURES.items(), *EMA_SIGNATURES.items(), *PROMPT_SIGNATURES.items(),
-                              *ROWS_SIGNATURES.items(), *PROMPT_LAYERS_SIGNATURES.items()):
+                              *ROWS_SIGNATURES.items(), *PROMPT_LAYERS_SIGNATURES.items(),
+                              *ADW_ROWS_SIGNATURES.items()):
         fn = getattr(lib, name)
         fn.restype = res
         fn.argtypes = args
@@ -313,10 +315,11 @@
 ADW_MAX_ADAPTERS, ADW_MAX_SEGMENTS = 16, 24
 
 
-def adapter_bwd_dw(groups, *, A):
+def _adw_tables(groups, A, Np=None):
     segs = [sg for g in groups for sg in g[0]]
     assert 0 < len(groups) <= ADW_MAX_ADAPTERS and 0 < len(segs) <= ADW_MAX_SEGMENTS
-    N, H = segs[0][0].shape
+    N, H = segs[0][3].shape
+    Nc = N if Np is None else Np
     Ap = segs[0][1].shape[1]
     strides = []
     for g in groups:
@@ -324,7 +327,8 @@
         for dy, z, dz, x in g[0]:
             for t, n in ((dy, "dy"), (z, "z"), (dz, "dz"), (x, "x")):
                 _req(t, torch.bfloat16, n)
-            assert dy.shape == (N, H) and x.shape == (N, H) and z.shape == (N, Ap) and dz.shape == (N, Ap) and Ap >= A
+            assert dy.shape[1] == H and x.shape == (N, H) and z.shape[1] == Ap and dz.shape[1] == Ap and Ap >= A
+            assert all(t.shape[0] >= Nc if Np is not None else t.shape[0] == N for t in (dy, z, dz))
             l = (_rows2d(dy, "dy"), _rows2d(z, "z"), _rows2d(dz, "dz"), _rows2d(x, "x"))
             assert lds is None or l == lds, "the segments of an adapter share their row strides"
             lds = l
@@ -340,10 +344,30 @@
     seg_first = (C.c_int32 * len(first))(*first)
     tab = lambda ts: (C.c_void_p * len(ts))(*[_p(t) for t in ts])
     ldt = lambda k: (C.c_int64 * len(strides))(*[st[k] for st in strides])
-    _chk(load().fbl_adapter_bwd_dw(len(groups), seg_first, tab([s[0] for s in segs]), tab([s[1] for s in segs]),
-                                   tab([s[2] for s in segs]), tab([s[3] for s in segs]), ldt(0), ldt(1), ldt(2), ldt(3),
-                                   N, H, int(A), Ap, tab([g[1] for g in groups]), tab([g[2] for g in groups]),
-                                   tab([g[3] for g in groups]), _stream()), "fbl_adapter_bwd_dw")
+    lead = (len(groups), seg_first, tab([s[0] for s in segs]), tab([s[1] for s in segs]), tab([s[2] for s in segs]),
+            tab([s[3] for s in segs]), ldt(0), ldt(1), ldt(2), ldt(3))
+    return lead, N, H, Ap, (tab([g[1] for g in groups]), tab([g[2] for g in groups]), tab([g[3] for g in groups]))
+
+
+def adapter_bwd_dw(groups, *, A):
+    lead, N, H, Ap, outs = _adw_tables(groups, A)
+    _chk(load().fbl_adapter_bwd_dw(*lead, N, H, int(A), Ap, *outs, _stream()), "fbl_adapter_bwd_dw")
+
+
+def live_tiles(plen, S: int, device) -> torch.Tensor:
+    live = set()
+    for b, n in enumerate(plen):
+        if n > 0:
+            live.update(range((b * S) // 64, (b * S + n - 1) // 64 + 1))
+    return torch.tensor(sorted(live), dtype=torch.int32, device=device)
+
+
+def adapter_bwd_dw_rows(groups, inv, tiles, Np, *, A):
+    _req(inv, torch.int32, "inv"); _req(tiles, torch.int32, "tiles")
+    lead, N, H, Ap, outs = _adw_tables(groups, A, Np=int(Np))
+    assert inv.is_contiguous() and tiles.is_contiguous() and inv.numel() == N and inv.is_cuda and tiles.is_cuda
+    _chk(load().fbl_adapter_bwd_dw_rows(*lead, N, H, int(A), Ap, *outs, _p(inv), _p(tiles), tiles.numel(), int(Np), _stream()),
+         "fbl_adapter_bwd_dw_rows")
 
 
 def embed_gather(ids, E, vproj, T, out_t):
@@ -796,11 +820,17 @@
 def ln_bwd_rows(dout, inv, t, stats, gamma, *, rowmask=None, p_drop=0.0, seed=0, out_dt=None, out_dy_bf16=None, out_dy_pad,
                 dgamma=None, dbeta=None, dysum=None, ws=None):
     N, H = t.shape
-    _req(inv, torch.int32, "inv"); _req(out_dy_pad, torch.bfloat16, "out_dy_pad")
-    assert dout.is_contiguous() and t.is_contiguous() and inv.is_contiguous() and inv.numel() == N
-    assert out_dy_pad.is_contiguous() and tuple(out_dy_pad.shape) == (N, H) and dout.shape[1] == H
+    _req(inv, torch.int32, "inv")
+    assert dout.is_contiguous() and t.is_contiguous() and inv.is_contiguous() and inv.numel() == N and dout.shape[1] == H
     assert out_dt is None or (out_dt.is_contiguous() and out_dt.shape == dout.shape)
     ld_dyb = _rows2d(out_dy_bf16, "out_dy_bf16") if out_dy_bf16 is not None else 0
+    if out_dy_pad is None:
+        _chk(load().fbl_ln_bwd_rows_nopad(_p(dout), _p(inv), _p(rowmask), _p(t), _p(stats), _p(gamma), float(p_drop), int(seed),
+                                          _seed_dev(), _p(out_dt), _p(out_dy_bf16), ld_dyb, _p(dgamma), _p(dbeta), _p(dysum), _p(ws),
+                                          N, H, _stream()), "fbl_ln_bwd_rows_nopad")
+        return
+    _req(out_dy_pad, torch.bfloat16, "out_dy_pad")
+    assert out_dy_pad.is_contiguous() and tuple(out_dy_pad.shape) == (N, H)
     _chk(load().fbl_ln_bwd_rows(_p(dout), _p(inv), _p(rowmask), _p(t), _p(stats), _p(gamma), float(p_drop), int(seed), _seed_dev(),
                                 _p(out_dt), _p(out_dy_bf16), ld_dyb, _p(out_dy_pad), _p(dgamma), _p(dbeta), _p(dysum), _p(ws), N, H,
                                 _stream()), "fbl_ln_bwd_rows")
diff --git a/include/fbl_adw_rows.h b/include/fbl_adw_rows.h
--- /dev/null
+++ b/include/fbl_adw_rows.h
@@ -0,0 +1,22 @@
+#ifndef FBL_ADW_ROWS_H
+#define FBL_ADW_ROWS_H
+#include "fbl_rows.h"
+#ifdef __cplusplus
+extern "C" {
+#endif
+
+int fbl_adapter_bwd_dw_rows(int n_adapters, const int32_t* seg_first, const void* const* dy_bf16, const void* const* z_bf16,
+                            const void* const* dz_bf16, const void* const* x_bf16, const int64_t* ld_dy, const int64_t* ld_z,
+                            const int64_t* ld_dz, const int64_t* ld_x, int N_pad, int H, int A, int Ap, float* const* dWu,
+                            float* const* dWd, float* const* dbd, const int32_t* inv, const int32_t* tiles, int n_tiles, int Np,
+                            void* stream);
+
+int fbl_ln_bwd_rows_nopad(const float* dout, const int32_t* inv, const int32_t* rowmask, const float* t, const float* stats,
+                          const float* gamma, float p_drop, uint64_t seed, const uint64_t* seed_dev, float* out_dt,
+                          void* out_dy_bf16, int64_t ld_dy_bf16, float* dgamma, float* dbeta, float* dysum, float* ws, int N_pad,
+                          int H, void* stream);
+
+#ifdef __cplusplus
+}
+#endif
+#endif
```
